# littlepure2333/GFlow

Measured on AMD Instinct MI355X. Metric: GFlow fit_video frames/sec (fwd+bwd+step) @60k Gaussians 480p, higher is better.
Workload: dtype f32

## Files before the change

gflow_amd/_lib.py:

```python
import ctypes
import os
import subprocess
import threading

import torch

_HERE = os.path.dirname(os.path.abspath(__file__))
_CSRC = os.path.join(_HERE, "csrc")
LIB_PATH = os.environ.get("GFLOW_HIP_LIB") or os.path.join(_HERE, "libgflow_hip.so")

_lock = threading.Lock()
_lib = None

c_void_p, c_int, c_float, c_size_t, c_int64 = ctypes.c_void_p, ctypes.c_int, ctypes.c_float, ctypes.c_size_t, ctypes.c_int64

MIN_VERSION = 312

_P = c_void_p
SIGNATURES = {
    "gfl_version": (c_int, []),
    "gfl_constants": (c_int, [_P]),
    "gfl_constants_n": (c_int, [_P, c_int]),
    "gfl_ewa_on_mfma": (c_int, []),
    "gfl_status_string": (ctypes.c_char_p, [c_int]),
    "gfl_last_hip_error": (c_int, []),
    "gfl_reduce_workspace_bytes": (c_size_t, [c_int]),
    "gfl_reduce_cam_workspace_bytes": (c_size_t, [c_int]),
    "gfl_project_point_fwd": (c_int, [_P, _P, _P, c_int, c_int, c_int, c_float, c_float, _P, _P, _P]),
    "gfl_project_point_bwd": (c_int, [_P, _P, _P, _P, _P, _P, c_int, _P, _P, _P, c_size_t, _P]),
    "gfl_project_point_bwd_cam": (c_int, [_P, _P, _P, _P, _P, _P, c_int, _P, _P, _P, _P, c_size_t, _P]),
    "gfl_cov3d_fwd": (c_int, [_P, _P, _P, c_int, _P, _P]),
    "gfl_cov3d_bwd": (c_int, [_P, _P, _P, _P, c_int, _P, _P, _P]),
    "gfl_ewa_fwd": (c_int, [_P, _P, _P, _P, _P, _P, c_int, c_int, c_int, _P, _P, _P, _P]),
    "gfl_ewa_bwd": (c_int, [_P, _P, _P, _P, _P, _P, c_int, c_int, c_int, _P, _P, _P, _P, c_size_t, _P]),
    "gfl_ewa_bwd_cam": (c_int, [_P, _P, _P, _P, _P, _P, c_int, c_int, c_int, _P, _P, _P, _P, _P, c_size_t, _P]),
    "gfl_bin_workspace_bytes": (c_size_t, [c_int, c_int, c_int, c_int]),
    "gfl_bin_count": (c_int, [_P, _P, _P, c_int, c_int, c_int, _P, _P]),
    "gfl_bin_sort": (c_int, [_P, _P, _P, _P, c_int, c_int, c_int, _P, c_int, _P, _P, _P, _P, c_size_t, _P]),
    "gfl_blend_fwd": (c_int, [_P, _P, _P, _P, c_int, c_int, c_int, _P, _P, c_float, c_int, c_int, _P, _P, _P, _P]),
    "gfl_blend_bwd": (c_int, [_P, _P, _P, _P, c_int, c_int, c_int, _P, _P, c_float, c_int, c_int, _P, _P, _P, c_int,
                              _P, _P, _P, _P, c_int, _P]),
    "gfl_sh_fwd": (c_int, [_P, _P, _P, c_int, c_int, _P, _P]),
    "gfl_sh_bwd": (c_int, [_P, _P, _P, _P, c_int, c_int, _P, _P, _P]),
    "gfl_colormap_nonzero": (c_int, [_P, c_int, _P, _P, _P, c_size_t, _P]),
    "gfl_loss_workspace_bytes": (c_size_t, [c_int, c_int]),
    "gfl_loss_fwd_bwd": (c_int, [_P, _P, _P, _P, _P, c_float, c_float, c_int, c_int, _P, _P, _P, _P, c_size_t, _P]),
    "gfl_loss_fwd_bwd_partials": (c_int, [_P, _P, _P, _P, _P, c_float, c_float, c_int, c_int, _P, _P, _P, c_size_t, _P, _P, _P, _P, _P]),
    "gfl_loss_prepare_gt": (c_int, [_P, _P, c_int, c_int, _P, _P]),
    "gfl_loss_fwd_bwd_partials_cached": (c_int, [_P, _P, _P, _P, _P, c_float, c_float, c_int, c_int, _P, _P, _P, c_size_t, _P, _P, _P, _P, _P, _P]),
    "gfl_adam_step": (c_int, [_P, _P, _P, _P, c_int64, c_int, _P, c_float, c_float, c_float, c_float, _P, c_float, c_int, _P]),
    "gfl_step_increment": (c_int, [_P, _P]),
    "gfl_tile_sort_only": (c_int, [_P, c_int, c_int, _P, _P, _P, _P]),
    "gfl_tile_sort_ordered": (c_int, [_P, c_int, c_int, c_int, _P, _P, _P, _P]),
    "gfl_tile_sort_reserved": (c_int, [_P, _P, _P, _P, c_int, c_int, c_int, _P, _P, _P, _P]),
    "gfl_fit_workspace_bytes": (c_size_t, [c_int, c_int, c_int, c_int]),
    "gfl_fit_workspace_layout": (c_int, [c_int, c_int, c_int, c_int, _P, _P, _P, c_int]),
    "gfl_fit_forward": (c_int, [_P, _P, _P]),
    "gfl_fit_backward_step": (c_int, [_P, _P, _P]),
    "gfl_fit_iteration": (c_int, [_P, _P, _P]),
    "gfl_fit_iterations": (c_int, [_P, _P, c_int, c_int, _P]),
    "gfl_fit_reserved_supported": (c_int, [_P, _P]),
    "gfl_fit_snapshot_stage": (c_int, [_P, _P, _P]),
    "gfl_fit_snapshot_workspace_bytes": (c_size_t, [c_int, c_int, c_int]),
    "gfl_fit_snapshot": (c_int, [_P, _P, _P, _P, _P, c_size_t, _P]),
    "gfl_fit_iteration_snapshot": (c_int, [_P, _P, _P, _P, _P]),
    "gfl_render_fwd": (c_int, [_P, _P, _P]),
    "gfl_render_bwd": (c_int, [_P, _P, _P, _P, _P, _P, _P, _P]),
    "gfl_render_bwd_cam": (c_int, [_P, _P, _P, _P, _P, _P, _P, _P, _P]),
    "gfl_render_batch_workspace_bytes": (c_size_t, [c_int, c_int, c_int, c_int, c_int]),
    "gfl_render_batch": (c_int, [_P, c_int, _P, _P, c_int, c_int, c_int, c_int, c_int, _P, _P, _P, _P, _P, c_size_t, _P]),
    "gfl_fit_prepare_targets": (c_int, [_P, _P]),
    "gfl_fit_schedule_info": (c_int, [_P, _P, _P, _P, _P]),
    "gfl_fit_schedule_info_fwd": (c_int, [_P, _P, _P, _P, _P]),
    "gfl_selftest_reduce10": (c_int, [_P, _P, _P, _P]),
    "gfl_selftest_cov2d": (c_int, [_P, _P, c_int, _P, _P, _P]),
    "gfl_selftest_block_mask": (c_int, [_P, c_int, c_int, c_int, c_int, _P, _P, _P]),
    "gfl_concave_hull": (c_int, [_P, c_int, ctypes.c_double, ctypes.c_double, _P, c_int]),
    "gfl_scan_f64_workspace_bytes": (c_size_t, [c_int]),
    "gfl_scan_f64": (c_int, [_P, c_int, _P, _P, c_size_t, _P]),
    "gfl_track_anchor_workspace_bytes": (c_size_t, [c_int, c_int]),
    "gfl_track_anchor": (c_int, [_P, c_int, c_int, _P, c_int, _P, _P, _P, c_size_t, _P]),
    "gfl_track_frame": (c_int, [_P, c_int, _P, c_int, c_int, _P, c_int, c_int, _P, _P, c_int, c_int, c_int, c_float, _P, _P,
                                _P]),
    "gfl_track_history": (c_int, [_P, c_int, _P, c_int, c_int, _P, c_int, c_int, c_float, _P, _P, _P]),
    "gfl_track_backward_workspace_bytes": (c_size_t, [c_int, c_int]),
    "gfl_track_backward": (c_int, [_P, _P, _P, c_int, _P, _P, c_int, _P, _P, _P, _P, c_size_t, _P]),
    "gfl_seg_score": (c_int, [_P, _P, _P, c_int, c_int, c_int, c_int, _P, _P]),
    "gfl_recon_workspace_bytes": (c_size_t, [c_int, c_int]),
    "gfl_recon_frame": (c_int, [_P, _P, c_int, c_int, c_int, c_int, _P, _P, c_size_t, _P]),
    "gfl_flow_workspace_bytes": (c_size_t, [c_int, c_int]),
    "gfl_flow_pair": (c_int, [_P, c_int, _P, _P, _P, c_int, _P, c_int, c_int, _P, _P, c_int, c_int, c_float, c_int, c_int, _P,
                              _P, _P, _P, c_size_t, _P]),
    "gfl_epi_workspace_bytes": (c_size_t, [c_int, c_int, c_int]),
    "gfl_epi_fundamental": (c_int, [_P, c_int, c_int, _P, c_int, _P, _P, _P, _P, _P, c_size_t, _P]),
    "gfl_epi_mask": (c_int, [_P, c_int, c_int, _P, ctypes.c_double, _P, _P, _P, _P, _P, _P, c_size_t, _P]),
    "gfl_flow_occlusion": (c_int, [_P, _P, c_int, c_int, c_int, c_float, c_float, _P, _P, _P, _P, _P]),
    "gfl_abi_sizes": (c_int, [_P, _P]),
    "gfl_profile_enable": (c_int, [ctypes.c_uint]),
    "gfl_profile_read": (c_int, [_P, _P, c_int]),
}


def build(force=False, quiet=True):
    if force:
        subprocess.run(["make", "-C", _CSRC, "clean"], check=True, capture_output=quiet)
    res = subprocess.run(["make", "-C", _CSRC, "-j8"], capture_output=True, text=True)
    if res.returncode != 0:
        raise RuntimeError("building libgflow_hip.so failed:\n" + res.stdout + res.stderr)
    return LIB_PATH


def load():
    global _lib
    with _lock:
        if _lib is not None:
            return _lib
        if not os.path.exists(LIB_PATH):
            raise RuntimeError(
                f"{LIB_PATH} is missing: run `python -c 'import __graft_entry__ as g; g.build()'` "
                "(or `make -C gflow_amd/csrc`).  gflow_amd has no CPU fallback.")
        lib = ctypes.CDLL(LIB_PATH)
        for name, (res, args) in SIGNATURES.items():
            try:
                fn = getattr(lib, name)
            except AttributeError:
                raise RuntimeError(f"{LIB_PATH} has no {name}: it was built from older sources, rebuild the library "
                                   "(make -C gflow_amd/csrc)") from None
            fn.restype = res
            fn.argtypes = args
        if lib.gfl_version() < MIN_VERSION:
            raise RuntimeError(f"{LIB_PATH} is version {lib.gfl_version()}, this binding needs >= {MIN_VERSION}: rebuild it "
                               "(make -C gflow_amd/csrc)")
        _lib = lib
        return lib


def check(rc, what=""):
    if rc != 0:
        lib = load()
        msg = lib.gfl_status_string(rc).decode()
        extra = f" (hipError {lib.gfl_last_hip_error()})" if rc == -3 else ""
        raise RuntimeError(f"libgflow_hip: {what}: {msg}{extra}")


def ptr(t):
    return None if t is None else ctypes.c_void_p(t.data_ptr())


def stream():
    return ctypes.c_void_p(torch.cuda.current_stream().cuda_stream)


def need_device(*tensors):
    for t in tensors:
        if t is not None and not t.is_cuda:
            raise RuntimeError("gflow_amd: tensors must be on a HIP (cuda) device; there is no CPU fallback")


def scratch(nbytes, device):
    return torch.empty(max(int(nbytes), 16), dtype=torch.uint8, device=device)


def scan_f64(x):
    need_device(x)
    x = x.reshape(-1).double().contiguous()
    out = torch.empty_like(x)
    n = x.numel()
    if n:
        lib = load()
        ws = scratch(lib.gfl_scan_f64_workspace_bytes(n), x.device)
        check(lib.gfl_scan_f64(ptr(x), n, ptr(out), ptr(ws), ws.numel(), stream()), "scan_f64")
    return out


def resolve_deterministic(deterministic):
    return torch.are_deterministic_algorithms_enabled() if deterministic is None else bool(deterministic)


_hip = None


def _hip_runtime():
    global _hip
    if _hip is None:
        _hip = ctypes.CDLL("libamdhip64.so")
        _hip.hipExtStreamCreateWithCUMask.restype = ctypes.c_int
        _hip.hipExtStreamCreateWithCUMask.argtypes = [ctypes.POINTER(ctypes.c_void_p), ctypes.c_uint32,
                                                      ctypes.POINTER(ctypes.c_uint32)]
    return _hip


def cu_partition(parts, device=None, cus=None):
    if cus is None:
        cus = torch.cuda.get_device_properties(device if device is not None else torch.cuda.current_device()).multi_processor_count
    xcds = 8
    per_xcd = cus // xcds
    n = per_xcd // int(parts)
    if n < 1:
        raise ValueError(f"cu_partition: {parts} shares of {per_xcd} CUs per XCD")
    out = []
    for p in range(int(parts)):
        words = [0] * ((cus + 31) // 32)
        for cu in range(p * n, (p + 1) * n):
            for x in range(xcds):
                i = cu * xcds + x
                words[i // 32] |= 1 << (i % 32)
        out.append((words, n * xcds))
    return out


def masked_stream(words, device=None):
    dev = torch.device("cuda", torch.cuda.current_device()) if device is None else torch.device(device)
    with torch.cuda.device(dev):
        arr = (ctypes.c_uint32 * len(words))(*words)
        h = ctypes.c_void_p()
        rc = _hip_runtime().hipExtStreamCreateWithCUMask(ctypes.byref(h), len(words), arr)
        if rc != 0:
            raise RuntimeError(f"hipExtStreamCreateWithCUMask failed: hipError {rc}")
    return torch.cuda.ExternalStream(h.value, device=dev)
```

gflow_amd/csrc/gfl_fit.hip:

```cpp
#include "gfl_fit.hpp"

using namespace gfl;

extern "C" {

size_t gfl_loss_workspace_bytes(int W, int H);

static inline int fit_nblk(int N) { return (N + BIN_BLOCK - 1) / BIN_BLOCK; }

static bool ewa_on_mfma() {
    static const bool on = [] { const char* e = getenv("GFL_EWA_MFMA"); return e && e[0] == '1'; }();
    return on;
}

int gfl_ewa_on_mfma(void) { return ewa_on_mfma() ? 1 : 0; }

static int fwd_split_min() {
    static const int v = [] { const char* e = getenv("GFL_FWD_SPLIT_MIN"); return e ? atoi(e) : FWD_SPLIT_MIN; }();
    return v;
}

static bool reserved_enabled() {
    static const bool on = [] { const char* e = getenv("GFL_RESERVED"); return !(e && e[0] == '0'); }();
    return on;
}

static int device_cus() {
    static const int cus = [] {
        int dev = 0, n = 0;
        const bool ok = hipGetDevice(&dev) == hipSuccess &&
                        hipDeviceGetAttribute(&n, hipDeviceAttributeMultiprocessorCount, dev) == hipSuccess && n > 0;
        return ok ? n : 256;
    }();
    return cus;
}
static int blend_queues(const gfl_fit_state* st) {
    int cus = (st && st->cu_count > 0) ? (st->cu_count / 8) * 8 : device_cus();
    if (cus <= 0) cus = 8;
    if (st && st->cu_count > 0) return cus < SCHED_MAX_QUEUES ? cus : SCHED_MAX_QUEUES;
    return cus < 64 ? 64 : (cus < SCHED_MAX_QUEUES ? cus : SCHED_MAX_QUEUES);
}

static int blend_grid(const gfl_fit_state* st, int T, int max_per_cu = BLEND_WG_PER_CU) {
    const int nq = blend_queues(st);
    int per = (T + nq - 1) / nq + 1;
    if (per > max_per_cu) per = max_per_cu;
    return nq * per;
}

struct FitCounters {
    int32_t pool_counter;   int32_t pad0[15];
    int32_t sched_valid;    int32_t pad1[15];
    int32_t regions_valid;  int32_t pad2[7];
    int32_t extent;         int32_t pad3[7];
    int32_t extent_next;    int32_t pad4[7];
    int32_t stamp;          int32_t pad5;
    int32_t snap_mm[2];     int32_t pad6[4];
};
static_assert(sizeof(FitCounters) == 256, "the counter block is one 256-byte region");
static_assert(offsetof(FitCounters, pool_counter) == 0 * 4 && offsetof(FitCounters, sched_valid) == 16 * 4 &&
              offsetof(FitCounters, regions_valid) == 32 * 4 && offsetof(FitCounters, extent) == 40 * 4 &&
              offsetof(FitCounters, extent_next) == 48 * 4 && offsetof(FitCounters, stamp) == 56 * 4 &&
              offsetof(FitCounters, snap_mm) == 58 * 4, "word offsets of the counters");

static size_t fit_regions(Arena& a, int cap_arg, int K_cap, int W, int H, FitWs& w) {
    const size_t T = tile_grid(W, H).tiles();
    const int cap = cap_arg > 0 ? cap_arg : 1;
    const size_t queue_items = (size_t)SCHED_MAX_QUEUES * sched_queue_capacity((int)T, 64);
    const size_t order_words = T * 4 + SORT_ORDER_TRAILER;
    w.hist = a.take<int32_t>("hist", (size_t)fit_nblk(cap) * T);
    w.keys = a.take<unsigned long long>("keys", (size_t)K_cap);
    w.partial = a.take<float>("partial", (size_t)reduce_rows(cap) * 12);
    w.tile_counts = a.take<int32_t>("tile_counts", T);
    w.pair_grad = a.take<float>("pair_grad", ((size_t)cap * SLOT_MAX + (size_t)K_cap) * PG);
    w.wide_base = (long long)cap * SLOT_MAX;
    w.wide_off = a.take<int32_t>("wide_off", (size_t)cap);
    if (FitCounters* c = a.take<FitCounters>("counters", 1)) {
        w.pool_counter = &c->pool_counter; w.sched_valid = &c->sched_valid; w.regions_valid = &c->regions_valid;
        w.extent = &c->extent; w.extent_next = &c->extent_next; w.stamp = &c->stamp; w.snap_mm = (unsigned*)c->snap_mm;
    }
    w.sched.work = a.take<int32_t>("sched_work", 4 * T);
    w.sched.list = a.take<int32_t>("sched_list", queue_items);
    w.sched.count = a.take<int32_t>("sched_count", 2 * SCHED_MAX_QUEUES);
    w.sched.counters = a.take<int32_t>("sched_counters", 2 * SCHED_MAX_QUEUES);
    w.ckpt = a.take<float>("ckpt", (size_t)SCHED_MAX_QUEUES * (HEAVY_PARTS - 1) * 5 * 256);
    w.sched_fwd.work = a.take<int32_t>("sched_fwd_work", 4 * T);
    w.sched_fwd.list = a.take<int32_t>("sched_fwd_list", queue_items);
    w.sched_fwd.count = a.take<int32_t>("sched_fwd_count", 2 * SCHED_MAX_QUEUES);
    w.sched_fwd.counters = w.sched.counters;
    w.sched_fwd.first_slot = nullptr;
    w.sched.first_slot = a.take<int32_t>("first_slot", T);
    w.loss_ws_bytes = up256(gfl_loss_workspace_bytes(W, H));
    w.loss_ws = a.take<char>("loss_ws", w.loss_ws_bytes);
    a.take<char>("loss_pad", 256);
    w.gt_stats = a.take<float>("gt_stats", (size_t)6 * W * H);
    w.scale_cnt = a.take<int32_t>("scale_cnt", (size_t)2 * fit_nblk(cap));
    w.sort_order = (int4*)a.take<int32_t>("sort_order", order_words);
    w.sort_order_next = (int4*)a.take<int32_t>("sort_order_next", order_words);
    w.region = a.take<int4>("region", T);
    w.fill = a.take<int32_t>("fill", T);
    w.partial_cam = a.take<float>("partial_cam", (size_t)reduce_rows(cap) * 4);
    w.d_rec_cam = a.take<float>("d_rec_cam", (size_t)cap * REC);
    return queue_items;
}

static int fit_layout(Arena& a, int cap, int K_cap, int W, int H) {
    if (cap < 0 || K_cap < 0 || W <= 0 || H <= 0) return GFL_ERR_INVALID;
    FitWs w;
    fit_regions(a, cap, K_cap, W, H, w);
    return a.n;
}

size_t gfl_fit_workspace_bytes(int cap, int K_cap, int W, int H) {
    Arena a;
    return fit_layout(a, cap, K_cap, W, H) < 0 ? 0 : a.off;
}

int gfl_fit_workspace_layout(int cap, int K_cap, int W, int H, const char** names, size_t* offsets, size_t* bytes, int max) {
    if (max < 0 || (max > 0 && (!names || !offsets || !bytes))) return GFL_ERR_INVALID;
    Arena a{nullptr, 0, names, offsets, bytes, max};
    return fit_layout(a, cap, K_cap, W, H);
}

static bool fit_ws_fits(const gfl_fit_state* st) {
    return st->workspace_bytes >= gfl_fit_workspace_bytes(st->cap, st->K_cap, st->W, st->H);
}

static FitWs carve(const gfl_fit_state* st) {
    Arena a{(char*)st->workspace};
    FitWs w;
    const size_t queue_items = fit_regions(a, st->cap, st->K_cap, st->W, st->H, w);
    for (Sched* s : {&w.sched, &w.sched_fwd}) {
        s->nq = blend_queues(st);
        s->cap_q = (int)(queue_items / s->nq);
        s->xcd = 1;
        s->det = (st->flags & GFL_FIT_DETERMINISTIC) ? 1 : 0;
    }
    w.sched.split_min = 0;
    w.sched_fwd.split_min = fwd_split_min();
    return w;
}

static bool next_sched_ok(const FitWs& w, int T) {
    return w.sched.xcd && T <= SCHED_PLAN_TILES && w.sched.nq % 8 == 0 && w.sched.nq / 8 <= 64 && w.sched.nq <= REDUCE_BLOCK;
}
static int next_sched_blocks(const FitWs& w, int T) { return next_sched_ok(w, T) ? 2 : 0; }
static size_t next_sched_lds(const FitWs& w, int T) { return next_sched_ok(w, T) ? sched_dyn_lds(T) : 0; }
static NextSched next_sched(const FitWs& w, int rows, int T) {
    NextSched ns;
    ns.rows = rows;
    ns.T = T;
    ns.tile_counts = w.tile_counts;
    ns.bwd = w.sched;
    ns.fwd = w.sched_fwd;
    ns.valid = w.sched_valid;
    ns.reserve = 0;
    ns.order_next = nullptr; ns.ro = ReserveOut{}; ns.regions_valid = nullptr; ns.pool_counter = nullptr;
    ns.pull_counters = nullptr; ns.n_pull = 0;
    return ns;
}

static bool fit_reserved_ok(const FitWs& w, int T) {
    return reserved_enabled() && next_sched_ok(w, T) && T <= 4096 && (2 * (size_t)T + 64) * sizeof(int32_t) <= 57 * 1024;
}
static NextSched next_sched_reserving(const gfl_fit_state* st, const FitWs& w, int rows, int T) {
    NextSched ns = next_sched(w, rows, T);
    if (!fit_reserved_ok(w, T)) return ns;
    ns.reserve = 1;
    ns.order_next = w.sort_order_next;
    ns.ro.region = w.region; ns.ro.fill = w.fill; ns.ro.extent_next = w.extent_next; ns.ro.total = st->tile_offsets + T;
    ns.ro.K_cap = st->K_cap;
    ns.regions_valid = w.regions_valid;
    ns.pool_counter = w.pool_counter;
    ns.pull_counters = w.sched.counters; ns.n_pull = 2 * w.sched.nq;
    return ns;
}

static int fit_check(const gfl_fit_state* st, const gfl_fit_hyper* hp) {
    if (!st || !hp) return GFL_ERR_INVALID;
    if (st->N < 0 || st->N > st->cap || st->W <= 0 || st->H <= 0 || st->K_cap < 0) return GFL_ERR_INVALID;
    if (st->flags & ~GFL_FIT_DETERMINISTIC) return GFL_ERR_INVALID;
    if (!st->params || !st->rec || !st->pose || !st->intr || !st->extr || !st->render || !st->final_T ||
        !st->n_contrib || !st->tile_offsets || !st->ids || !st->tile_range || !st->overflow || !st->workspace)
        return GFL_ERR_INVALID;
    if (!fit_ws_fits(st)) return GFL_ERR_WORKSPACE;
    return GFL_OK;
}


static PreArgs pre_args(const gfl_fit_state* st, const gfl_fit_hyper* hp, const FitWs& w, int gx, int gy, int op_mode) {
    PreArgs a;
    a.intr = st->intr; a.pose = st->pose;
    a.N = st->N; a.W = st->W; a.H = st->H;
    a.nearest = hp->nearest; a.extent = hp->extent;
    a.gx = gx; a.gy = gy;
    a.rec = st->rec; a.wide_off = w.wide_off; a.hist_g = w.hist; a.extr_out = st->extr; a.overflow = st->overflow;
    a.pool_counter = w.pool_counter; a.pool_cap = st->K_cap;
    a.op_mode = op_mode;
    a.scale_rows_mode = (!op_mode && hp->lambda_scale != 0.f) ? (hp->freeze_all_splats ? 2 : 1) : 0;
    a.scale_cnt = w.scale_cnt;
    return a;
}

static int fit_forward_impl(const gfl_fit_state* st, const gfl_fit_hyper* hp, gfl_stream_t stream, int op_mode, int reserved = 0,
                            const float* snap_lut = nullptr, uint8_t* snap_u8 = nullptr) {
    int rc = fit_check(st, hp);
    if (rc) return rc;
    hipStream_t s = (hipStream_t)stream;
    const auto [gx, gy, T] = tile_grid(st->W, st->H);
    const FitWs w = carve(st);
    const int nblk = fit_nblk(st->N > 0 ? st->N : 1);
    if ((size_t)T * sizeof(int32_t) > 57 * 1024) return GFL_ERR_INVALID;
    const PreArgs pa = pre_args(st, hp, w, gx, gy, op_mode);
    if (reserved) {
        if (op_mode || !fit_reserved_ok(w, T)) return GFL_ERR_INVALID;
        {
            StageScope p(ST_PREPROCESS, s);
            BinArgs b;
            b.region = w.region; b.fill = w.fill; b.keys = w.keys; b.K_cap = st->K_cap;
            b.regions_valid = w.regions_valid; b.extent_next = w.extent_next; b.extent = w.extent;
            b.pull_counters = w.sched.counters; b.n_pull = 2 * w.sched.nq;
            launch_preprocess_bin(st->params, pa, st->row_flags, b, nblk, ewa_on_mfma(), s);
        }
        {
            StageScope p(ST_TILE_SORT, s);
            rc = gfl_tile_sort_reserved((const int32_t*)w.sort_order_next, w.fill, w.tile_counts, st->overflow + 2, st->W, st->H,
                                        st->K_cap, w.keys, st->ids, st->tile_range, stream);
        }
        if (rc) return rc;
    } else {
        {
            StageScope p(ST_PREPROCESS, s);
            launch_preprocess_fwd(st->params, pa, st->row_flags, nblk, ewa_on_mfma(), s);
        }
        {
            StageScope p(ST_COLSCAN, s);
            launch_colscan(w, nblk, T, st->overflow, s);
        }
        const bool ordered = T <= 8 * BIN_BLOCK;
        {
            StageScope p(ST_SCATTER, s);
            launch_scatter(st, w, nblk, gx, gy, ordered, s);
        }
        {
            StageScope p(ST_TILE_SORT, s);
            if (ordered)
                rc = gfl_tile_sort_ordered((const int32_t*)w.sort_order, st->W, st->H, st->K_cap, w.keys, st->ids, st->tile_range,
                                           stream);
            else
                rc = gfl_tile_sort_only(st->tile_offsets, gx * gy, st->K_cap, w.keys, st->ids, st->tile_range, stream);
        }
        if (rc) return rc;
    }
    {
        StageScope p(ST_BLEND_FWD, s);
        const TileQueue q = {w.sched_fwd.list, w.sched_fwd.count, w.sched.counters, w.sched.nq, w.sched.cap_q};
        if (snap_u8) {
            rc = check(hipMemsetAsync(w.snap_mm, 0, 2 * sizeof(unsigned), s));
            if (rc) return rc;
            if (st->N > 0) launch_rec_depth_range(st->rec, st->N, w.snap_mm, s);
            launch_blend_fwd(st, hp->bg, gx, blend_grid(st, T, FWD_WG_PER_CU), st->render, st->final_T, st->n_contrib, q, w, 2,
                             w.snap_mm, snap_lut, fwd_split_min(), s, snap_u8);
            launch_center_blend(st, hp->bg, gx, T, nullptr, snap_u8 + (size_t)2 * st->W * st->H * 3, s);
        }
        const bool foot = st->foot_flags && !(hp->bg > 0.f) && st->N > 0;
        if (foot && !st->keep) return GFL_ERR_INVALID;
        const bool foot_inside = foot && !snap_u8;
        if (!snap_u8)
            launch_blend_fwd(st, hp->bg, gx, blend_grid(st, T, FWD_WG_PER_CU), st->render, st->final_T, st->n_contrib, q, w,
                             foot_inside ? 3 : 0, nullptr, nullptr, fwd_split_min(), s);
        if (st->foot_flags) {
            if (!st->keep) return GFL_ERR_INVALID;
            if (foot && !foot_inside) launch_footprint(st, gx, T, s);
        }
    }
    return check_launch();
}

int gfl_fit_forward(const gfl_fit_state* st, const gfl_fit_hyper* hp, gfl_stream_t stream) {
    return fit_forward_impl(st, hp, stream, 0);
}

struct SnapWs { unsigned* mm; int32_t* pull; size_t head_bytes; float *img_dc, *img_c, *fT; int32_t* nc; size_t bytes; };
static SnapWs snap_ws(void* base, int W, int H) {
    Arena a{(char*)base};
    const size_t P = (size_t)W * H;
    return {a.take<unsigned>("mm", 2), a.take<int32_t>("pull", 2 * SCHED_MAX_QUEUES), a.off,
            a.take<float>("img_dc", 4 * P), a.take<float>("img_c", 4 * P), a.take<float>("final_T", P),
            a.take<int32_t>("n_contrib", P), a.off};
}

size_t gfl_fit_snapshot_workspace_bytes(int N, int W, int H) {
    return (N < 0 || W <= 0 || H <= 0) ? 0 : snap_ws(nullptr, W, H).bytes;
}

int gfl_fit_snapshot(const gfl_fit_state* st, const gfl_fit_hyper* hp, const float* lut, uint8_t* out_u8, void* workspace,
                     size_t workspace_bytes, gfl_stream_t stream) {
    int rc = fit_check(st, hp);
    if (rc) return rc;
    if (!lut || !out_u8 || !workspace) return GFL_ERR_INVALID;
    if (workspace_bytes < gfl_fit_snapshot_workspace_bytes(st->N, st->W, st->H)) return GFL_ERR_WORKSPACE;
    hipStream_t s = (hipStream_t)stream;
    const auto [gx, gy, T] = tile_grid(st->W, st->H);
    const FitWs w = carve(st);
    const SnapWs sw = snap_ws(workspace, st->W, st->H);
    rc = check(hipMemsetAsync(workspace, 0, sw.head_bytes, s));
    if (rc) return rc;
    if (st->N > 0) launch_rec_depth_range(st->rec, st->N, sw.mm, s);
    launch_center_blend(st, hp->bg, gx, T, sw.img_c, nullptr, s);
    {
        const TileQueue q = {w.sched_fwd.list, w.sched_fwd.count, sw.pull, w.sched.nq, w.sched.cap_q};
        launch_blend_fwd(st, hp->bg, gx, blend_grid(st, T, FWD_WG_PER_CU), sw.img_dc, sw.fT, sw.nc, q, w, 1, sw.mm, lut, fwd_split_min(), s);
    }
    launch_snapshot_u8(st->render, sw.img_dc, sw.img_c, st->W * st->H, out_u8, s);
    return check_launch();
}

int gfl_fit_snapshot_stage(const gfl_fit_state* src, const gfl_fit_state* dst, gfl_stream_t stream) {
    if (!src || !dst || !src->workspace || !dst->workspace || !src->rec || !dst->rec || !src->ids || !dst->ids ||
        !src->tile_range || !dst->tile_range || !src->render || !dst->render || !src->tile_offsets)
        return GFL_ERR_INVALID;
    if (src->W != dst->W || src->H != dst->H || src->N != dst->N || dst->N > dst->cap || src->N > src->cap)
        return GFL_ERR_INVALID;
    if (!fit_ws_fits(src) || !fit_ws_fits(dst)) return GFL_ERR_WORKSPACE;
    const int T = tile_grid(src->W, src->H).T;
    const size_t P = (size_t)src->W * src->H;
    const FitWs a = carve(src), b = carve(dst);
    if (a.sched_fwd.nq != b.sched_fwd.nq || a.sched_fwd.cap_q != b.sched_fwd.cap_q) return GFL_ERR_INVALID;
    StageCopy c;
    c.k_ptr = a.extent;
    c.ids_cap = (unsigned)min(src->K_cap, dst->K_cap);
    c.seg[0] = {(const uint32_t*)src->ids, (uint32_t*)dst->ids, 0u};
    c.seg[1] = {(const uint32_t*)src->rec, (uint32_t*)dst->rec, (unsigned)((size_t)src->N * REC)};
    c.seg[2] = {(const uint32_t*)src->tile_range, (uint32_t*)dst->tile_range, (unsigned)(2 * T)};
    c.seg[3] = {(const uint32_t*)src->render, (uint32_t*)dst->render, (unsigned)(3 * P)};
    c.seg[4] = {(const uint32_t*)a.sched_fwd.list, (uint32_t*)b.sched_fwd.list,
                (unsigned)((size_t)a.sched_fwd.nq * a.sched_fwd.cap_q)};
    c.seg[5] = {(const uint32_t*)a.sched_fwd.count, (uint32_t*)b.sched_fwd.count, (unsigned)a.sched_fwd.nq};
    c.seg[6] = {(const uint32_t*)a.sched.first_slot, (uint32_t*)b.sched.first_slot, (unsigned)T};
    launch_snapshot_stage(c, (hipStream_t)stream);
    return check_launch();
}

int gfl_render_fwd(const gfl_fit_state* st, const gfl_fit_hyper* hp, gfl_stream_t stream) {
    if (st && st->foot_flags) return GFL_ERR_INVALID;
    if (st && (st->flags & GFL_FIT_DETERMINISTIC)) {
        const int rc = fit_check(st, hp);
        if (rc) return rc;
        const int T = tile_grid(st->W, st->H).T;
        const FitWs w = carve(st);
        hipStream_t s = (hipStream_t)stream;
        if (check(hipMemsetAsync(w.sched.work, 0, 4 * (size_t)T * sizeof(int32_t), s)) ||
            check(hipMemsetAsync(w.sched_fwd.work, 0, 4 * (size_t)T * sizeof(int32_t), s)) ||
            check(hipMemsetAsync(w.sched_valid, 0, sizeof(int32_t), s)))
            return GFL_ERR_HIP;
    }
    return fit_forward_impl(st, hp, stream, 1);
}

static int render_bwd_impl(const gfl_fit_state* st, const gfl_fit_hyper* hp, const float* d_render, const float* d_uv,
                           const float* d_depth, float* d_params, float* d_extr, float* d_intr, gfl_stream_t stream) {
    hipStream_t s = (hipStream_t)stream;
    const auto [gx, gy, T] = tile_grid(st->W, st->H);
    const FitWs w = carve(st);
    {
        StageScope p(ST_BLEND_BWD, s);
        const TileQueue q = {w.sched.list, w.sched.count, w.sched.counters + w.sched.nq, w.sched.nq, w.sched.cap_q};
        launch_blend_bwd(st, hp->bg, gx, gy, blend_grid(st, T), 10, d_render, q, w, LossTail{}, s);
    }
    {
        StageScope p(ST_PRE_BWD_ADAM, s);
        const NextSched ns = next_sched(w, reduce_rows(st->N > 0 ? st->N : 1), T);
        if (d_intr)
            launch_splat_bwd_op_cam(st, w, gx, gy, ns, next_sched_blocks(w, T), next_sched_lds(w, T), d_uv, d_depth, d_params, d_extr,
                                    d_intr, s);
        else
            launch_splat_bwd_op(st, w, gx, gy, ns, next_sched_blocks(w, T), next_sched_lds(w, T), d_uv, d_depth, d_params, d_extr, s);
    }
    return check_launch();
}

int gfl_render_bwd(const gfl_fit_state* st, const gfl_fit_hyper* hp, const float* d_render, const float* d_uv,
                   const float* d_depth, float* d_params, float* d_extr, gfl_stream_t stream) {
    int rc = fit_check(st, hp);
    if (rc) return rc;
    if (!d_render || !d_params || !d_extr) return GFL_ERR_INVALID;
    return render_bwd_impl(st, hp, d_render, d_uv, d_depth, d_params, d_extr, nullptr, stream);
}

int gfl_render_bwd_cam(const gfl_fit_state* st, const gfl_fit_hyper* hp, const float* d_render, const float* d_uv,
                       const float* d_depth, float* d_params, float* d_extr, float* d_intr, gfl_stream_t stream) {
    if (!d_extr || !d_intr) return GFL_ERR_INVALID;
    int rc = fit_check(st, hp);
    if (rc) return rc;
    if (!d_render || !d_params) return GFL_ERR_INVALID;
    return render_bwd_impl(st, hp, d_render, d_uv, d_depth, d_params, d_extr, d_intr, stream);
}

int gfl_fit_backward_step(const gfl_fit_state* st, const gfl_fit_hyper* hp, gfl_stream_t stream) {
    int rc = fit_check(st, hp);
    if (rc) return rc;
    if (!st->adam_m || !st->adam_v || !st->pose_m || !st->pose_v || !st->depth_ab || !st->depth_ab_m ||
        !st->depth_ab_v || !st->step || !st->gt_rgb || !st->d_render || !st->err_px || !st->sums || !st->d_extr)
        return GFL_ERR_INVALID;
    hipStream_t s = (hipStream_t)stream;
    const auto [gx, gy, T] = tile_grid(st->W, st->H);
    const FitWs w = carve(st);
    const float *p_ssim = nullptr, *p_grad = nullptr;
    int n_ssim = 0, n_grad = 0;
    {
        StageScope p(ST_LOSS, s);
        const float* gt_stats = (st->gt_cached && !st->foot_flags) ? w.gt_stats : nullptr;
        rc = gfl_loss_fwd_bwd_partials_cached(st->render, st->gt_rgb, st->gt_depth, st->keep, st->depth_ab,
                                              hp->lambda_rgb, hp->lambda_depth, st->W, st->H, st->d_render,
                                              st->err_px, w.loss_ws, w.loss_ws_bytes, gt_stats, &p_ssim, &n_ssim,
                                              &p_grad, &n_grad, stream);
    }
    if (rc) return rc;
    AdamCfg ac = {hp->lr, hp->beta1, hp->beta2, hp->eps, hp->lr_end_factor, hp->total_iters};
    AdamCfg ac_cam = ac;
    ac_cam.lr = hp->lr_camera;
    const bool frozen = hp->step_camera != 2 && (hp->step_camera == 0 || hp->lr_camera == 0.f);
    LossTail lt = {};
    if (frozen) {
        lt.enabled = 1;
        lt.p_ssim = p_ssim; lt.n_ssim = n_ssim; lt.p_grad = p_grad; lt.n_grad = n_grad;
        lt.depth_ab = st->depth_ab; lt.ab_m = st->depth_ab_m; lt.ab_v = st->depth_ab_v;
        lt.sums = st->sums; lt.ac_ab = ac; lt.step_affine = hp->step_camera != 0;
        lt.d_step = st->step; lt.d_extr_out = st->d_extr; lt.overflow = st->overflow;
    }
    {
        StageScope p(ST_BLEND_BWD, s);
        const TileQueue q = {w.sched.list, w.sched.count, w.sched.counters + w.sched.nq, w.sched.nq, w.sched.cap_q};
        const int sums = hp->freeze_all_splats ? 6 : (hp->freeze_rgb ? 7 : 10);
        launch_blend_bwd(st, hp->bg, gx, gy, blend_grid(st, T), sums, st->d_render, q, w, lt, s);
    }
    const int rows = reduce_rows(st->N > 0 ? st->N : 1);
    RegCfg rcfg;
    rcfg.lambda_scale = hp->lambda_scale;
    rcfg.scale_blocks = 2 * fit_nblk(st->N > 0 ? st->N : 1);
    rcfg.lambda_var = st->N > 0 ? hp->lambda_var / (float)st->N : 0.f;
    rcfg.lambda_flow = hp->lambda_flow;
    rcfg.lambda_still = hp->lambda_still;
    rcfg.freeze_rgb = hp->freeze_rgb;
    rcfg.freeze_all = hp->freeze_all_splats;
    rcfg.no_pose_grad = frozen ? 1 : 0;
    {
        StageScope p(ST_PRE_BWD_ADAM, s);
        const NextSched ns = next_sched_reserving(st, w, rows, T);
        launch_splat_bwd_adam(st, w, gx, gy, rcfg, ac, ns, next_sched_blocks(w, T) + ns.reserve, next_sched_lds(w, T), s);
    }
    if (!frozen) {
        StageScope p(ST_CAMERA, s);
        launch_camera_adam(st, w, rows, p_ssim, n_ssim, p_grad, n_grad, ac_cam, ac, hp->step_camera != 0, s);
    }
    return check_launch();
}

int gfl_fit_iterations(const gfl_fit_state* st, const gfl_fit_hyper* hp, int count, int flags, gfl_stream_t stream) {
    if (count < 1 || (flags & ~GFL_ITER_RESERVED)) return GFL_ERR_INVALID;
    int rc = fit_check(st, hp);
    if (rc) return rc;
    const int T = tile_grid(st->W, st->H).T;
    const FitWs w = carve(st);
    const bool res_ok = fit_reserved_ok(w, T) && st->N > 0;
    if ((flags & GFL_ITER_RESERVED) && !res_ok) return GFL_ERR_INVALID;
    for (int j = 0; j < count; ++j) {
        const int reserved = res_ok && (j > 0 || (flags & GFL_ITER_RESERVED)) ? 1 : 0;
        rc = fit_forward_impl(st, hp, stream, 0, reserved);
        if (rc) return rc;
        rc = gfl_fit_backward_step(st, hp, stream);
        if (rc) return rc;
    }
    return GFL_OK;
}

int gfl_fit_iteration_snapshot(const gfl_fit_state* st, const gfl_fit_hyper* hp, const float* lut, uint8_t* out_u8,
                               gfl_stream_t stream) {
    if (!lut || !out_u8) return GFL_ERR_INVALID;
    int rc = fit_forward_impl(st, hp, stream, 0, 0, lut, out_u8);
    if (rc) return rc;
    return gfl_fit_backward_step(st, hp, stream);
}

int gfl_fit_reserved_supported(const gfl_fit_state* st, const gfl_fit_hyper* hp) {
    if (fit_check(st, hp) || st->N <= 0) return 0;
    const int T = tile_grid(st->W, st->H).T;
    return fit_reserved_ok(carve(st), T) ? 1 : 0;
}

int gfl_fit_prepare_targets(const gfl_fit_state* st, gfl_stream_t stream) {
    if (!st || st->W <= 0 || st->H <= 0 || !st->gt_rgb || !st->workspace) return GFL_ERR_INVALID;
    if (!fit_ws_fits(st)) return GFL_ERR_WORKSPACE;
    const FitWs w = carve(st);
    return gfl_loss_prepare_gt(st->gt_rgb, st->keep, st->W, st->H, w.gt_stats, stream);
}

static int schedule_info(const gfl_fit_state* st, bool fwd, int* n_queues, int* queue_capacity, const int32_t** d_lists,
                         const int32_t** d_counts) {
    if (!st || !n_queues || !queue_capacity || !d_lists || !d_counts || !st->workspace) return GFL_ERR_INVALID;
    if (!fit_ws_fits(st)) return GFL_ERR_WORKSPACE;
    const FitWs w = carve(st);
    const Sched& sc = fwd ? w.sched_fwd : w.sched;
    *n_queues = sc.nq;
    *queue_capacity = sc.cap_q;
    *d_lists = sc.list;
    *d_counts = sc.count;
    return GFL_OK;
}

int gfl_fit_schedule_info(const gfl_fit_state* st, int* n_queues, int* queue_capacity, const int32_t** d_lists,
                          const int32_t** d_counts) {
    return schedule_info(st, false, n_queues, queue_capacity, d_lists, d_counts);
}

int gfl_fit_schedule_info_fwd(const gfl_fit_state* st, int* n_queues, int* queue_capacity, const int32_t** d_lists,
                              const int32_t** d_counts) {
    return schedule_info(st, true, n_queues, queue_capacity, d_lists, d_counts);
}

int gfl_fit_iteration(const gfl_fit_state* st, const gfl_fit_hyper* hp, gfl_stream_t stream) {
    int rc = gfl_fit_forward(st, hp, stream);
    if (rc) return rc;
    return gfl_fit_backward_step(st, hp, stream);
}

#ifdef GFL_TRACE
int gfl_debug_read_fwd_trace(long long* out, int n_tiles) { return read_fwd_trace(out, n_tiles); }
int gfl_debug_read_fwd_trace2(long long* out, int n_values) { return read_fwd_trace2(out, n_values); }
int gfl_debug_read_phase_trace(long long* out, int n_values) {
    const int rc = read_phase_trace_bin(out, n_values);
    return rc ? rc : read_phase_trace_splat(out, n_values);
}
int gfl_debug_read_bwd_trace(long long* out, int n_tiles) { return read_bwd_trace(out, n_tiles); }
#endif

}
```

gflow_amd/csrc/gfl_fit_snap.hip:

```cpp
#include "gfl_fit.hpp"

namespace gfl {

__global__ void __launch_bounds__(256) center_blend_kernel(const float* __restrict__ rec, const int32_t* __restrict__ ids,
                                                           const int32_t* __restrict__ tile_range, float bg, int W, int H, int gx,
                                                           float* __restrict__ out, uint8_t* __restrict__ out_u8) {
    __shared__ RecLDS recs[FB + 1];
    __shared__ unsigned char s_mask[FB];
    if (threadIdx.x == 0) {
        const float4 z = make_float4(0.f, 0.f, 0.f, 0.f);
        recs[FB].p0 = z; recs[FB].p1 = z; recs[FB].p2 = z;
    }
    const int tile = blockIdx.x;
    const int tx = tile % gx, ty = tile / gx;
    const int tid = threadIdx.x, wave = tid >> 6, lane = tid & 63;
    const int px = tx * GFL_TILE + (wave & 1) * 8 + (lane & 7);
    const int py = ty * GFL_TILE + (wave >> 1) * 8 + (lane >> 3);
    const bool inside = px < W && py < H;
    const float fx = pixf(px), fy = pixf(py);
    const int start = tile_range[2 * tile], end = tile_range[2 * tile + 1];
    const float blob_cutoff = alpha_cutoff(1.f, 1.f);
    float T = 1.f, Tw = inside ? 1.f : 0.f, a0 = 0.f, a1 = 0.f, a2 = 0.f;
    for (int base = start; base < end; base += FB) {
        if (__syncthreads_and(Tw == 0.f)) break;
        const int idx = base + tid;
        unsigned char m = 0;
        if (idx < end) {
            const int g = ids[idx];
            const float4* r4 = reinterpret_cast<const float4*>(rec + (size_t)g * REC);
            float4 p0 = r4[0], p1 = r4[1], p2 = r4[2];
            p0.z = 1.f; p0.w = 0.f; p1.x = 1.f; p1.y = 1.f;
            p2.z = p2.z < 0.f ? p2.z : blob_cutoff;
            recs[tid].p0 = p0; recs[tid].p1 = p1; recs[tid].p2 = p2;
            m = (unsigned char)block_mask(p0, p1, p2.z, tx * GFL_TILE, ty * GFL_TILE);
        }
        s_mask[tid] = m;
        __syncthreads();
        const int cnt = min(FB, end - base);
        for (int c0 = 0; c0 < cnt && !__all(Tw == 0.f); c0 += 64) {
            const int slot = c0 + lane;
            unsigned long long bits = __ballot(slot < cnt && ((s_mask[slot] >> wave) & 1));
            while (bits) {
                int j[4];
#pragma unroll
                for (int u = 0; u < 4; ++u) {
                    j[u] = bits ? c0 + (int)__builtin_ctzll(bits) : FB;
                    bits &= bits - 1;
                }
                float4 q0[4], q1[4];
                float cb[4], al[4];
                bool val[4];
#pragma unroll
                for (int u = 0; u < 4; ++u) { q0[u] = recs[j[u]].p0; q1[u] = recs[j[u]].p1; cb[u] = recs[j[u]].p2.x; }
#pragma unroll
                for (int u = 0; u < 4; ++u) {
                    float G;
                    val[u] = splat_alpha2(q0[u], q1[u], fx, fy, al[u], G);
                }
#pragma unroll
                for (int u = 0; u < 4; ++u) {
                    const float a = val[u] ? al[u] : 0.f;
                    const float test_T = Tw * (1.f - a);
                    const bool stop = test_T < GFL_T_MIN;
                    const float w = stop ? 0.f : a * Tw;
                    a0 = fmaf(q1[u].z, w, a0); a1 = fmaf(q1[u].w, w, a1); a2 = fmaf(cb[u], w, a2);
                    T = stop ? T : test_T;
                    Tw = stop ? 0.f : test_T;
                }
                if (__all(Tw == 0.f)) break;
            }
        }
    }
    if (inside) {
        const size_t pix = (size_t)py * W + px, plane = (size_t)H * W;
        const float o0 = fmaf(T, bg, a0), o1 = fmaf(T, bg, a1), o2 = fmaf(T, bg, a2);
        if (out_u8) {
            uint8_t* u = out_u8 + pix * 3;
            u[0] = img_u8(o0); u[1] = img_u8(o1); u[2] = img_u8(o2);
        } else {
            out[pix] = o0; out[plane + pix] = o1; out[2 * plane + pix] = o2;
        }
    }
}

__global__ void __launch_bounds__(256) rec_depth_range_kernel(const float* __restrict__ rec, int N, unsigned* __restrict__ mm) {
    unsigned lo = 0xffffffffu, hi = 0u;
    for (int i = blockIdx.x * blockDim.x + threadIdx.x; i < N; i += gridDim.x * blockDim.x) {
        const float x = rec[(size_t)i * REC + 9];
        const unsigned b = __float_as_uint(x);
        const unsigned k = (b & 0x80000000u) ? ~b : (b | 0x80000000u);
        if (x != 0.f) lo = min(lo, k);
        hi = max(hi, k);
    }
#pragma unroll
    for (int off = 32; off >= 1; off >>= 1) {
        lo = min(lo, (unsigned)__shfl_xor((int)lo, off));
        hi = max(hi, (unsigned)__shfl_xor((int)hi, off));
    }
    if ((threadIdx.x & 63) == 0) {
        atomicMax(&mm[0], ~lo);
        atomicMax(&mm[1], hi);
    }
}

__global__ void __launch_bounds__(256) snapshot_u8_kernel(const float* __restrict__ a, const float* __restrict__ b,
                                                          const float* __restrict__ c, int P, uint8_t* __restrict__ out) {
    const int i = blockIdx.x * blockDim.x + threadIdx.x;
    if (i >= P) return;
    const float* src[3] = {a, b, c};
#pragma unroll
    for (int k = 0; k < 3; ++k) {
#pragma unroll
        for (int ch = 0; ch < 3; ++ch) {
            out[((size_t)k * P + i) * 3 + ch] = img_u8(src[k][(size_t)ch * P + i]);
        }
    }
}

__global__ void __launch_bounds__(256) snapshot_stage_kernel(StageCopy c) {
    const unsigned tid = blockIdx.x * blockDim.x + threadIdx.x, stride = gridDim.x * blockDim.x;
#pragma unroll
    for (int sgi = 0; sgi < 7; ++sgi) {
        const StageSeg sg = c.seg[sgi];
        unsigned n = sg.n;
        if (sgi == 0) n = min((unsigned)max(*c.k_ptr, 0), c.ids_cap);
        const unsigned n4 = n >> 2;
        const uint4* s4 = reinterpret_cast<const uint4*>(sg.src);
        uint4* d4 = reinterpret_cast<uint4*>(sg.dst);
        for (unsigned i = tid; i < n4; i += stride) d4[i] = s4[i];
        for (unsigned i = (n4 << 2) + tid; i < n; i += stride) sg.dst[i] = sg.src[i];
    }
}

void launch_center_blend(const gfl_fit_state* st, float bg, int gx, int T, float* out, uint8_t* out_u8, hipStream_t s) {
    center_blend_kernel<<<T, 256, 0, s>>>(st->rec, st->ids, st->tile_range, bg, st->W, st->H, gx, out, out_u8);
}

void launch_rec_depth_range(const float* rec, int N, unsigned* mm, hipStream_t s) {
    rec_depth_range_kernel<<<min((N + 255) / 256, 32), 256, 0, s>>>(rec, N, mm);
}

void launch_snapshot_u8(const float* a, const float* b, const float* c, int P, uint8_t* out, hipStream_t s) {
    snapshot_u8_kernel<<<(P + 255) / 256, 256, 0, s>>>(a, b, c, P, out);
}

void launch_snapshot_stage(const StageCopy& c, hipStream_t s) { snapshot_stage_kernel<<<1024, 256, 0, s>>>(c); }

}
```

gflow_amd/fit_video.py:

```python
import argparse
import json
import math
import os
import sys
import time

import torch

from . import camera as CM
from . import flow as FL
from . import quality as QL
from . import segmentation as SG
from . import tracking as TK

SCRIPT_OVERRIDES = dict(num_points=50000, lr_after=4e-3, lr_camera_after=1e-3, densify_times_after=2,
                        densify_occ_percent=0.5, lambda_depth=0.1, lambda_var=50.0, lambda_still=0.0)
DEFAULTS = dict(num_points=60000, lr=4e-3, lr_camera=0.0, iterations_first=500, lr_after=1e-3, iterations_after=300,
                camera_first=True, lr_camera_after=5e-4, iterations_camera=150, densify_interval=150, densify_times=2,
                densify_interval_after=100, densify_times_after=1, densify_occ_percent=1.0, densify_err_thre=1e-2,
                densify_err_percent=1.0, lambda_rgb=1.0, lambda_depth=1e-4, lambda_var=10.0, lambda_still=10.0,
                lambda_flow=0.01, lambda_scale=0.0, background="black",
                traj_num=0, traj_offset=0)

METRIC_NAMES = ("psnr_sum", "frames", "iterations", "rasterisations", "clips", "splats_final")


def shard(n_items, rank, world, lengths=None):
    lengths = [1] * n_items if lengths is None else [int(v) for v in lengths]
    if len(lengths) != n_items:
        raise ValueError("shard: one length per clip")
    load = [0] * world
    mine = []
    for i in sorted(range(n_items), key=lambda j: (-lengths[j], j)):
        r = min(range(world), key=lambda q: (load[q], q))
        load[r] += lengths[i]
        if r == rank:
            mine.append(i)
    return sorted(mine)


def reduce_metrics(local, wall_seconds, dist=None, device="cpu", rank=0, world=1):
    own = [0.0] * world
    own[rank] = float(wall_seconds)
    vec = torch.tensor([float(local.get(k, 0.0)) for k in METRIC_NAMES] + own, dtype=torch.float64, device=device)
    wall = torch.tensor([float(wall_seconds)], dtype=torch.float64, device=device)
    if dist is not None and dist.is_initialized():
        dist.all_reduce(vec, op=dist.ReduceOp.SUM)
        dist.all_reduce(wall, op=dist.ReduceOp.MAX)
    vals = vec.tolist()
    out = {k: float(v) for k, v in zip(METRIC_NAMES, vals)}
    out["wall_s"] = float(wall.item())
    out["rank_wall_s"] = [float(v) for v in vals[len(METRIC_NAMES):]]
    return out


TAPVID_KEYS = ("occlusion_accuracy", "average_jaccard", "average_pts_within_thresh")
DAVIS_KEYS = ("J", "F", "J&F")
RECON_KEYS = ("PSNR", "SSIM")
CAMERA_KEYS = CM.SCORE_KEYS
FLOW_KEYS = FL.EVAL_KEYS


def _mean_over_clips(keys, scores, totals, dist=None, device="cpu", none=float("nan")):
    n = len(keys)
    sums, counts = [0.0] * n, [0.0] * n
    for m in scores:
        for j, k in enumerate(keys):
            if m[k] is not None and not math.isnan(m[k]):
                sums[j] += float(m[k])
                counts[j] += 1.0
    vec = torch.tensor(sums + counts + [float(t) for t in totals.values()], dtype=torch.float64, device=device)
    if dist is not None and dist.is_initialized():
        dist.all_reduce(vec, op=dist.ReduceOp.SUM)
    v = vec.tolist()
    out = {k: v[j] / v[n + j] if v[n + j] else none for j, k in enumerate(keys)}
    out.update(zip(totals, (int(t) for t in v[2 * n:])))
    return out


def reduce_tapvid(preds, gts, n_frames, dropped, dist=None, device="cpu"):
    ms = [TK.evaluate(p, *gts[ci][:4], n_frames[ci], *gts[ci][4:]) for ci, p in preds.items()]
    return _mean_over_clips(TAPVID_KEYS, ms, dict(clips=len(ms), queries_dropped=dropped), dist, device)


def reduce_davis(segs, dist=None, device="cpu"):
    ms = [SG.evaluate(seg) for seg in segs.values()]
    totals = dict(frames_scored=sum(m["frames_scored"] for m in ms), clips=sum(1 for m in ms if m["frames_scored"]))
    return _mean_over_clips(DAVIS_KEYS, ms, totals, dist, device)


def reduce_recon(recons, dist=None, device="cpu"):
    ms = [QL.evaluate(rec) for rec in recons.values()]
    totals = dict(frames=sum(m["frames"] for m in ms), clips=sum(1 for m in ms if m["frames"]))
    return _mean_over_clips(RECON_KEYS, ms, totals, dist, device)


def reduce_camera(cams, dist=None, device="cpu"):
    scored = [cam for cam in cams.values() if not any(cam[k] is None for k in CAMERA_KEYS)]
    totals = dict(clips=len(scored), clips_unscored=len(cams) - len(scored))
    return _mean_over_clips(CAMERA_KEYS, scored, totals, dist, device, none=None)


def reduce_flow(flows, dist=None, device="cpu"):
    ms = [FL.evaluate(fl) for fl in flows.values()]
    totals = dict(pairs=sum(m["pairs"] for m in ms), clips=sum(1 for m in ms if m["pairs"]))
    return _mean_over_clips(FLOW_KEYS, ms, totals, dist, device, none=None)


def csv_metrics(out):
    m = {}
    if "recon" in out:
        m.update({"PSNR": out["recon"]["PSNR"], "SSIM": out["recon"]["SSIM"]})
    if "tapvid" in out:
        m.update({"Occlusion_Accuracy": out["tapvid"]["occlusion_accuracy"], "Average_Jaccard": out["tapvid"]["average_jaccard"],
                  "Average_PTS_within_threshold": out["tapvid"]["average_pts_within_thresh"]})
    if "davis" in out:
        m.update({"J_zero": out["davis"]["J"], "F_zero": out["davis"]["F"], "J&F_zero": out["davis"]["J&F"]})
    if "camera" in out:
        m.update({k: out["camera"][k] for k in CAMERA_KEYS})
    return m


_FIT_STREAMS = {}


def upload_clip(frames, device):
    out = []
    for fr in frames:
        d = dict(fr)
        occ = fr.get("occ_mask")
        if occ is not None and "occ_count" not in d:
            m = torch.as_tensor(occ).squeeze()
            if m.dim() == 3:
                m = m[..., 0] if m.shape[-1] in (1, 3) else m[0]
            d["occ_count"] = int((m > 0).sum())
        for k, v in fr.items():
            if isinstance(v, torch.Tensor) and k != "extr":
                d[k] = v.to(device, non_blocking=True)
        out.append(d)
    return out


def select_traj_seeds(tr, traj_num, traj_offset):
    import numpy as np
    from scipy.ndimage import minimum_filter
    n = tr.current_pts_num()
    interval = max(int(n / traj_num), 1)
    plain = list(range(n))[traj_offset::interval]
    move_seg = getattr(tr, "move_seg", None)
    if move_seg is None:
        return plain, None
    H, W = tr.H, tr.W
    erode = lambda m: minimum_filter(m, size=10, mode="constant", cval=255)
    move_er = erode(np.asarray(move_seg, dtype=np.uint8))
    still_er = erode((255 - np.asarray(move_seg, dtype=np.int32)).astype(np.uint8))
    s_still, s_move = 50, 15
    grid = lambda lo_i, hi_i, lo_j, hi_j, s: [(j, i) for i in range(lo_i, hi_i, s) for j in range(lo_j, hi_j, s)]
    sparse = [(j, i) for (j, i) in grid(s_still, H, s_still, W, s_still) if still_er[i, j]]
    if len(sparse) == 0:
        sparse = grid(s_still, H, s_still, W, s_still)
    dense = [(j, i) for (j, i) in grid(s_move, H - s_move, s_move, W - s_move, s_move) if move_er[i, j]]
    if len(sparse) == 0:
        dense = grid(s_move, H - s_move, s_move, W - s_move, s_move)
    uv = tr.last_uv.detach().double()
    still = tr.still_mask.detach()

    def closest(points):
        q = torch.tensor(points, dtype=torch.float64, device=uv.device)
        out = []
        for a in range(0, q.shape[0], 256):
            d = ((uv[:, None, :] - q[None, a:a + 256, :]) ** 2).sum(-1)
            out.append(d.argmin(dim=0))
        return torch.cat(out)

    if len(sparse) == 0:
        return plain, None
    sp = closest(sparse)
    sp_still = sp[still[sp]]
    if len(dense):
        de = closest(dense)
        de_move = de[~still[de]]
        return torch.cat([sp_still, de_move]).tolist(), int(sp_still.shape[0])
    return sp_still.tolist(), None


def begin_frame(tr, frames, i, load_extr=True):
    fr = frames[i]
    tr.set_gt_image(fr["image"])
    tr.set_gt_depth(fr["depth"])
    tr.set_gt_flow(frames[i - 1]["flow"])
    if load_extr and fr.get("extr") is not None:
        tr.load_camera(extr=fr["extr"])


def stage_kwargs(c, frames, i, stage):
    fr = frames[i]
    if stage == "camera":
        return dict(iterations=c["iterations_camera"], lr_camera=c["lr_camera_after"], lambda_var=0.0, lambda_still=0.0,
                    lambda_flow=c["lambda_flow"], densify_interval=c["densify_interval"], densify_times=c["densify_times"],
                    camera_only=True, move_mask=fr["move_mask"])
    if stage == "joint":
        return dict(iterations=c["iterations_after"], lr=c["lr_after"], lr_camera=0.0, lambda_var=c["lambda_var"],
                    lambda_still=c["lambda_still"], lambda_flow=c["lambda_flow"], densify_interval=c["densify_interval_after"],
                    densify_times=c["densify_times_after"], mask=fr.get("occ_mask"), mask_count=fr.get("occ_count"),
                    move_mask=fr["move_mask"])
    raise ValueError(stage)


def fit_clip(frames, device, cfg=None, fused=True, deterministic=None, **options):
    if deterministic and not fused:
        raise ValueError("fit_clip(deterministic=True) needs fused=True: the operator path's alpha_blending backward has no "
                         "deterministic implementation")
    from .trainer import run_to_end
    dev_ = torch.device(device)
    g = fit_clip_steps(frames, device, cfg, fused=fused, deterministic=deterministic, chunk=None, cu_count=0, **options)

    drive = lambda: run_to_end(g)
    if dev_.type == "cuda" and torch.cuda.current_stream(dev_) == torch.cuda.default_stream(dev_):
        key = dev_.index
        if key not in _FIT_STREAMS:
            _FIT_STREAMS[key] = torch.cuda.Stream(device=dev_)
        fs = _FIT_STREAMS[key]
        fs.wait_stream(torch.cuda.current_stream(dev_))
        with torch.cuda.stream(fs):
            out = drive()
        torch.cuda.current_stream(dev_).wait_stream(fs)
        return out
    return drive()


def fit_clip_steps(frames, device, cfg=None, seed=0, snapshot_interval=0, fused=True, log=None, load_extr=True, chunk=None,
                   async_snapshots=True, keep=None, cu_count=0, deterministic=None, track_queries=None, segment=False,
                   recon=False, camera=False, flow=False, track_backward=False):
    if track_backward and track_queries is None:
        raise ValueError("fit_clip(track_backward=True) needs track_queries")
    from .trainer import SimpleGaussian
    c = dict(DEFAULTS)
    c.update(cfg or {})
    if any(isinstance(v, torch.Tensor) and not v.is_cuda for k, v in frames[0].items() if k != "extr"):
        frames = upload_clip(frames, device)
    f0 = frames[0]
    tracker = None
    if track_queries is not None:
        tracker = TK.Tracker(track_queries, len(frames), device, backward=bool(track_backward))
    cam_rec = None
    if camera:
        cam_gt = [fr["extr_gt"] if fr.get("extr_gt") is not None else fr.get("extr") for fr in frames]
        missing = [t for t, e in enumerate(cam_gt) if e is None]
        if missing:
            raise ValueError(f"fit_clip(camera=True): frames {missing} carry neither extr_gt nor extr")
        cam_rec = CM.CameraRecorder(len(frames))
    tr = SimpleGaussian(f0["image"], f0["depth"], num_points=c["num_points"], background=c["background"],
                        device=device, seed=seed, fused=fused, deterministic=deterministic)
    tr.async_snapshots = bool(async_snapshots)
    tr.cu_count = int(cu_count)
    if segment:
        tr.seg_recorder = SG.MoveSegRecorder(len(frames), tr.H, tr.W, tr.device)
    recon_rec = None
    if recon:
        recon_rec = QL.ReconRecorder(len(frames), tr.H, tr.W, tr.device)
    flow_rec = None
    if flow:
        flow_rec = FL.FlowRecorder(len(frames), tr.H, tr.W, tr.device, keep_maps=flow == "maps")
        if keep is not None and keep.get("record_flow_inputs"):
            flow_rec.inputs = keep.setdefault("flow_inputs", [])
    tr.load_camera(focal=f0["focal"], pp=f0["pp"])
    if load_extr and f0.get("extr") is not None:
        tr.load_camera(extr=f0["extr"])
    tr.init_gaussians_from_image(f0["image"], f0["depth"], num_points=c["num_points"])
    common = dict(lambda_rgb=c["lambda_rgb"], lambda_depth=c["lambda_depth"], lambda_scale=c["lambda_scale"],
                  densify_occ_percent=c["densify_occ_percent"], densify_err_thre=c["densify_err_thre"],
                  densify_err_percent=c["densify_err_percent"], snapshot_interval=snapshot_interval,
                  lazy_images=True,
                  chunk=chunk)
    traj = int(c["traj_num"]) > 0
    yield from tr.train_steps(iterations=c["iterations_first"], lr=c["lr"], lr_camera=c["lr_camera"],
                              lambda_var=c["lambda_var"], densify_interval=c["densify_interval"],
                              densify_times=c["densify_times"], move_mask=f0["move_mask"],
                              move_seg=traj,
                              **common)
    traj_rec = []
    final = []

    def final_forward():
        if not final:
            final.append(tr._aux_forward())
            final[0].watch_overflow()
            tr.rasterisations_done += 1
        return final[0]

    def record_trajectories():
        with torch.no_grad():
            xyz_now = tr.get_attribute("xyz")[traj_index_t].detach().float().clone()
            extr_now = tr.get_extr().detach().clone()
            if tr.engine_current:
                rgb_u8 = tr._render_scene_fused()[0].clone()
                final.append(tr._aux)
            else:
                from . import render as render_mod
                rgb_u8 = render_mod.render2img_device(render_mod.render_multiple(tr._input_group(detach=True), ["rgb"])["rgb"])
            tr.rasterisations_done += 1
        traj_rec.append((xyz_now, extr_now, rgb_u8))

    def record_tracks(i):
        with torch.no_grad():
            if tr.engine_current:
                from .fused import REC
                aux = final_forward()
                n = aux.N
                uv, uv_stride, depth, depth_stride, dm = aux.rec[:n, 0:2], REC, aux.rec[:n, 9], REC, aux.render[3]
            else:
                from . import render as render_mod
                o = render_mod.render_multiple(tr._input_group(detach=True), ["uv", "depth", "depth_map"])
                uv, depth = o["uv"].float().contiguous(), o["depth"].float().reshape(-1).contiguous()
                dm = o["depth_map"].float().reshape(tr.H, tr.W).contiguous()
                uv_stride, depth_stride = 2, 1
                tr.rasterisations_done += 1
            tracker.frame(i, uv, uv_stride, depth, depth_stride, dm)
            if keep is not None and keep.get("record_track_inputs"):
                keep.setdefault("track_inputs", []).append((uv.clone(), depth.clone(), dm.clone()))

    def record_flow(i):
        with torch.no_grad():
            if tr.engine_current:
                aux = final_forward()
                rec, n, ids, tile_range = aux.rec, aux.N, aux.ids, aux.tile_range
            else:
                rec, n, ids, tile_range = FL.operator_state(tr._input_group(detach=True))
                tr.rasterisations_done += 1
            prev = frames[i - 1] if i else None
            flow_rec.frame(i, rec, n, ids, tile_range, prev["flow"] if prev else None, prev["move_mask"] if prev else None)

    def record_scores(i):
        with torch.no_grad():
            if recon_rec is not None:
                recon_rec.frame(i, tr.last_render, tr.gt_image)
                if keep is not None and keep.get("record_recon_inputs"):
                    keep.setdefault("recon_inputs", []).append(tr.last_render[:3].clone())
            if cam_rec is not None:
                cam_rec.frame(i, tr.get_extr())

    def draw_trajectories():
        from . import msplat
        from . import render as render_mod
        imgs, uvs = [], []
        with torch.no_grad():
            for xyz_now, extr_now, rgb_u8 in traj_rec:
                overlay = tr.eval_trajectories(xyz_now, extr_now, line_scale=0.5, point_scale=2.0, alpha=0.8,
                                               split_interval=split_interval)
                img_traj = render_mod.render2img_device(overlay)
                upon = 1.0 - (1.0 - rgb_u8.double() / 255.0) * (1.0 - img_traj.double() / 255.0)
                imgs.append(torch.stack([img_traj, (upon * 255.0).to(torch.uint8)]))
                uvs.append(msplat.project_point(xyz_now, tr.intr, extr_now, tr.W, tr.H)[0])
                if keep is not None:
                    keep.setdefault("traj_groups", []).append([x.clone() if isinstance(x, torch.Tensor) else x
                                                               for x in tr.last_traj_group])
        return torch.stack(imgs), torch.stack(uvs)

    psnr_sum = None

    def end_of_frame(i):
        nonlocal psnr_sum
        final.clear()
        if traj:
            record_trajectories()
        if tracker is not None:
            record_tracks(i)
        if flow_rec is not None:
            record_flow(i)
        p = tr.psnr()
        psnr_sum = p.double() if psnr_sum is None else psnr_sum + p.double()
        if recon_rec is not None or cam_rec is not None:
            record_scores(i)
        if keep is not None:
            keep["psnr"].append(p)
        if log:
            log(f"frame {i}: psnr {float(p):.2f} dB, splats {tr.current_pts_num()}")

    if traj:
        traj_index, split_interval = select_traj_seeds(tr, int(c["traj_num"]), int(c["traj_offset"]))
        traj_index_t = torch.as_tensor(traj_index, device=tr.device).long()
    if keep is not None:
        keep["trainer"], keep["psnr"] = tr, []
    end_of_frame(0)
    for i in range(1, len(frames)):
        begin_frame(tr, frames, i, load_extr)
        if segment:
            tr.seg_recorder.frame = i
        if c["camera_first"]:
            yield from tr.train_steps(**stage_kwargs(c, frames, i, "camera"), **common)
        if c["iterations_after"] > 0:
            yield from tr.train_steps(**stage_kwargs(c, frames, i, "joint"), **common)
        end_of_frame(i)
    if tr.engine is not None:
        tr.engine.check_overflow()
    if traj:
        imgs_d, uvs_d = draw_trajectories()
        if imgs_d.is_cuda:
            from .pinned import PINNED
            block = PINNED.take(imgs_d.numel())
            imgs_h = block[0][:imgs_d.numel()].view(imgs_d.shape)
            imgs_h.copy_(imgs_d, non_blocking=True)
            uvs_h = uvs_d.cpu()
            traj_out = dict(images=PINNED.hand_out(block, [imgs_h])[0], uv=uvs_h.numpy(), index=list(traj_index),
                            split_interval=split_interval)
            PINNED.release(block)
        else:
            traj_out = dict(images=imgs_d.numpy(), uv=uvs_d.numpy(), index=list(traj_index), split_interval=split_interval)
        if keep is not None:
            keep["traj"] = traj_out
    out = dict(psnr_sum=float(psnr_sum), frames=len(frames), iterations=tr.iterations_done,
               rasterisations=tr.rasterisations_done, clips=1, splats_final=tr.current_pts_num(),
               void_iterations=tr.engine.regions_outgrown if tr.engine is not None else 0)
    if traj:
        out["traj"] = traj_out
    if tracker is not None:
        out["tracks"] = tracker.result()
    if segment:
        rec = tr.seg_recorder
        if keep is not None and keep.get("record_seg_inputs"):
            keep["seg_inputs"] = [None if x is None else (x[0].clone(), x[1].clone()) for x in rec.inputs]
        out["segmentation"] = rec.result([fr["move_mask"] for fr in frames])
    if recon_rec is not None:
        out["recon"] = recon_rec.result()
    if cam_rec is not None:
        import numpy as np
        extr = cam_rec.result()
        gt = np.stack([torch.as_tensor(e).detach().cpu().double().numpy().reshape(3, 4) for e in cam_gt])
        out["camera"] = dict(extr=extr, **CM.evaluate(extr, gt))
    if flow_rec is not None:
        out["flow"] = flow_rec.result()
    return out


NUMERIC_KEYS = ("psnr_sum", "frames", "iterations", "rasterisations", "clips", "splats_final", "void_iterations")


def fit_clips_concurrent(clips, device, cfg=None, seeds=None, chunk=32, partition=False, deterministic=None,
                         track_queries=None, track_backward=False, **options):
    n = len(clips)
    if track_queries is not None and len(track_queries) != n:
        raise ValueError("fit_clips_concurrent: track_queries needs one entry per clip")
    if track_backward and track_queries is None:
        raise ValueError("fit_clips_concurrent(track_backward=True) needs track_queries")
    seeds = list(range(n)) if seeds is None else seeds
    dev = torch.device(device)
    if dev.index is None:
        dev = torch.device("cuda", torch.cuda.current_device())
    cur = torch.cuda.current_stream(dev)
    shares = None
    if partition and n > 1:
        from . import _lib
        shares = _lib.cu_partition(n, dev)
        streams = [_lib.masked_stream(words, dev) for words, _ in shares]
    else:
        streams = [torch.cuda.Stream(device=dev) for _ in range(n)]
    for s in streams:
        s.wait_stream(cur)
    gens = [fit_clip_steps(clips[i], dev, cfg, seed=seeds[i], chunk=chunk, async_snapshots=n == 1,
                           cu_count=shares[i][1] if shares else 0, deterministic=deterministic,
                           track_queries=None if track_queries is None else track_queries[i],
                           track_backward=bool(track_backward) and track_queries[i] is not None, **options)
            for i in range(n)]
    results = [None] * n
    live = list(range(n))
    while live:
        for i in list(live):
            with torch.cuda.stream(streams[i]):
                try:
                    next(gens[i])
                except StopIteration as e:
                    results[i] = e.value
                    live.remove(i)
    for s in streams:
        cur.wait_stream(s)
    return results


def main(argv=None):
    ap = argparse.ArgumentParser(description="fit synthetic clips, one process per GPU")
    ap.add_argument("--clips", type=int, default=1)
    ap.add_argument("--frames", type=int, default=4)
    ap.add_argument("--height", type=int, default=480)
    ap.add_argument("--width", type=int, default=854)
    ap.add_argument("--num_points", type=int, default=60000)
    ap.add_argument("--iterations_first", type=int, default=500)
    ap.add_argument("--iterations_after", type=int, default=300)
    ap.add_argument("--iterations_camera", type=int, default=150)
    ap.add_argument("--frames-list", default=None, help="comma-separated frame counts, one per synthetic clip (clips of "
                                                        "unequal length: the shard balances them)")
    ap.add_argument("--clips-per-gpu", type=int, default=1,
                    help="clips a rank fits at the same time on its GPU (fit_clips_concurrent)")
    ap.add_argument("--verbose", action="store_true")
    ap.add_argument("--sequence", action="append", default=None,
                    help="path of a prepared sequence folder (images + the reference's sibling folders, "
                         "gflow_amd/io.py); may be given several times, one clip each; default: synthetic clips")
    ap.add_argument("--resize", type=int, default=None, help="shorter image side after loading a --sequence")
    ap.add_argument("--deterministic", action="store_true",
                    help="bit-identical results for identical inputs (the library's deterministic mode, INTEGRATION.md)")
    ap.add_argument("--track", action="store_true",
                    help="track the first-visible query points of each clip's tracking.pkl (synthetic clips: their "
                         "make_clip_tracks) through the fit and score them with TAP-Vid (a \"tapvid\" block in the line)")
    ap.add_argument("--track-backward", action="store_true",
                    help="with --track: also track every query through the frames before its own (the \"tapvid\" block "
                         "then carries \"backward\": true)")
    ap.add_argument("--track-queries", choices=("first", "strided"), default="first",
                    help="with --track: the query protocol -- each track's first visible frame, or TAP-Vid's strided one "
                         "(every fifth frame where the track is visible; wants --track-backward)")
    ap.add_argument("--track-out", default=None, help="with --track: write each clip's predicted tracks to DIR/clip_<i>.npz")
    ap.add_argument("--seg", action="store_true",
                    help="keep every frame's moving-region mask and score it against the frame's move_mask with DAVIS J, F "
                         "and J&F (a \"davis\" block in the line)")
    ap.add_argument("--seg-out", default=None,
                    help="with --seg: write each clip's masks to DIR/clip_<i>/move_mask_<frame>.png")
    ap.add_argument("--recon", action="store_true",
                    help="score every frame's render with PSNR and SSIM on the device (a \"recon\" block in the line)")
    ap.add_argument("--camera", action="store_true",
                    help="keep every frame's camera and score the path against the clip's own (extr_gt, else extr) with "
                         "ATE and RPE (a \"camera\" block in the line)")
    ap.add_argument("--flow", action="store_true",
                    help="the dense optical flow the fitted splats imply between consecutive frames, scored against the flow "
                         "the clip came with: end-point error, still / moving, accuracies, coverage (a \"flow\" block in the "
                         "line)")
    ap.add_argument("--flow-out", default=None,
                    help="with --flow: write each clip's flow maps to DIR/clip_<i>/flow_<frame>.flo (frame -> frame + 1 on "
                         "the frame's grid; pixels without a flow are 1e10, Middlebury's mark)")
    ap.add_argument("--no-load-extr", action="store_true",
                    help="do not load the frames' camera poses (extr): the camera-only stages estimate them, as the "
                         "reference's scripts/fit_video.sh runs")
    ap.add_argument("--make-move-masks", action="store_true",
                    help="with --sequence: compute every frame's move_mask from its forward flow on the device "
                         "(gflow_amd.move_seg, before the clock starts) instead of reading <seq>_epipolar")
    ap.add_argument("--make-occ-masks", action="store_true",
                    help="with --sequence: compute every frame's occ_mask from its forward and backward flows "
                         "(<seq>_flow_unimatch/*pred.flo, *pred_bwd.flo) on the device (gflow_amd.occlusion, before the clock "
                         "starts) instead of reading *occ_bwd.png")
    ap.add_argument("--metrics-csv", default=None,
                    help="rank 0 writes the blocks that were asked for as key,value lines under the reference's "
                         "metrics.csv keys")
    args = ap.parse_args(argv)
    if args.track_backward and not args.track:
        ap.error("--track-backward needs --track")
    if args.track and args.track_queries == "strided" and not args.track_backward:
        print("warning: --track-queries strided without --track-backward: every frame before a query is a miss",
              file=sys.stderr)
    det = True if args.deterministic else None
    from . import synthetic as S
    rank = int(os.environ.get("RANK", "0"))
    local_rank = int(os.environ.get("LOCAL_RANK", "0"))
    world = int(os.environ.get("WORLD_SIZE", "1"))
    n_dev = torch.cuda.device_count()
    if n_dev < 1:
        raise RuntimeError("gflow_amd.fit_video needs a HIP device (there is no CPU rasteriser)")
    shared = world > n_dev
    torch.cuda.set_device(local_rank % n_dev)
    dev = torch.device("cuda", local_rank % n_dev)
    dist = None
    if world > 1:
        import torch.distributed as dist
        if shared:
            dist.init_process_group(backend="gloo")
        else:
            dist.init_process_group(backend="nccl", device_id=dev)
    cfg = dict(num_points=args.num_points, iterations_first=args.iterations_first,
               iterations_after=args.iterations_after, iterations_camera=args.iterations_camera)
    local = {k: 0.0 for k in METRIC_NAMES}
    n_clips = len(args.sequence) if args.sequence else args.clips
    if args.sequence:
        from . import io as gio
        lengths = [len(gio.sequence_paths(p)["img"]) for p in args.sequence]
    elif args.frames_list:
        lengths = [int(v) for v in args.frames_list.split(",")]
        if len(lengths) != n_clips:
            raise SystemExit("--frames-list needs one length per clip")
    else:
        lengths = [args.frames] * n_clips
    mine = shard(n_clips, rank, world, lengths)
    t_load = time.perf_counter()
    clips = {}
    for ci in mine:
        if args.sequence:
            clips[ci] = gio.load_sequence(args.sequence[ci], resize=args.resize,
                                          move_masks="epipolar" if args.make_move_masks else "files",
                                          occ_masks="flow" if args.make_occ_masks else "files")
        else:
            clips[ci] = upload_clip(S.make_clip(lengths[ci], args.height, args.width, seed=ci, device=dev), dev)
    gts, queries, dropped = {}, {}, 0
    if args.track:
        for ci in mine:
            h, w = clips[ci][0]["image"].shape[:2]
            if args.sequence:
                pts, occ = TK.read_tapvid_pickle(os.path.join(args.sequence[ci], "tracking.pkl"))
            else:
                g = S.make_clip_tracks(lengths[ci], args.height, args.width, seed=ci)
                pts, occ = g["points"].astype("float32"), g["occluded"]
            if args.track_queries == "strided":
                q, src = TK.strided_queries(pts, occ, h, w)
                keep = q[:, 0] < len(clips[ci])
                gts[ci] = (pts, occ, h, w, q[keep], src[keep])
            else:
                q = TK.first_visible_queries(pts, occ, h, w)
                keep = q[:, 0] < len(clips[ci])
                gts[ci] = (pts[keep], occ[keep], h, w)
            dropped += int((~keep).sum())
            queries[ci] = q[keep]
    t_load = time.perf_counter() - t_load
    torch.cuda.synchronize()
    t0 = time.perf_counter()
    c = max(1, args.clips_per_gpu)
    order = sorted(clips, key=lambda j: (-lengths[j], j))
    options = dict(track_backward=args.track_backward, deterministic=det, segment=args.seg, recon=args.recon, camera=args.camera,
                   flow=("maps" if args.flow_out else True) if args.flow else False, load_extr=not args.no_load_extr)
    results = {}
    for g0 in range(0, len(order), c):
        group = order[g0:g0 + c]
        if len(group) == 1:
            ci = group[0]
            res = [fit_clip(clips[ci], dev, cfg, seed=ci, track_queries=queries.get(ci), **options,
                            log=(lambda s, ci=ci: print(f"[rank {rank} clip {ci}] {s}")) if args.verbose else None)]
        else:
            res = fit_clips_concurrent([clips[ci] for ci in group], dev, cfg, seeds=group,
                                       track_queries=[queries.get(ci) for ci in group] if args.track else None, **options)
        for ci, m in zip(group, res):
            for k in METRIC_NAMES:
                local[k] += m[k]
            results[ci] = m
    torch.cuda.synchronize()
    wall = time.perf_counter() - t0
    of = lambda key: {ci: m[key] for ci, m in results.items()}
    over_ranks = (dist, torch.device("cpu") if (world > 1 and shared) else dev)
    out = reduce_metrics(local, wall, *over_ranks, rank=rank, world=world)
    if args.track:
        preds = of("tracks")
        out["tapvid"] = reduce_tapvid(preds, gts, {ci: len(clips[ci]) for ci in clips}, dropped, *over_ranks)
        if args.track_backward:
            out["tapvid"]["backward"] = True
        if args.track_out:
            import numpy as np
            os.makedirs(args.track_out, exist_ok=True)
            for ci, p in preds.items():
                np.savez(os.path.join(args.track_out, f"clip_{ci}.npz"), queries=queries[ci], **p)
    if args.seg:
        out["davis"] = reduce_davis(of("segmentation"), *over_ranks)
        if args.seg_out:
            from PIL import Image
            for ci, seg in of("segmentation").items():
                d = os.path.join(args.seg_out, f"clip_{ci}")
                os.makedirs(d, exist_ok=True)
                for t in range(len(seg["masks"])):
                    if seg["valid"][t]:
                        Image.fromarray(seg["masks"][t]).save(os.path.join(d, f"move_mask_{t:05d}.png"))
    if args.recon:
        out["recon"] = reduce_recon(of("recon"), *over_ranks)
    if args.camera:
        out["camera"] = reduce_camera(of("camera"), *over_ranks)
    if args.flow:
        out["flow"] = reduce_flow(of("flow"), *over_ranks)
        if args.flow_out:
            for ci, fl in of("flow").items():
                FL.write_flo_maps(os.path.join(args.flow_out, f"clip_{ci}"), fl)
    if rank == 0 and args.metrics_csv:
        QL.write_metrics_csv(args.metrics_csv, csv_metrics(out))
    if rank == 0:
        out["frames_per_s"] = out["frames"] / out["wall_s"]
        out["iterations_per_s"] = out["iterations"] / out["wall_s"]
        out["psnr_mean_db"] = out["psnr_sum"] / max(out["frames"], 1.0)
        out["n_gpus"] = world
        out["clips_per_gpu"] = c
        out["load_s_rank0"] = t_load
        print(json.dumps(out))
    if dist is not None:
        dist.destroy_process_group()
    return out if rank == 0 else None


if __name__ == "__main__":
    main()
```

gflow_amd/fused.py:

```python
import ctypes

import torch

from . import _lib as L

ROW = 16
REC = 12
COLS = {"xyz": (0, 3), "scale": (3, 6), "rotate": (6, 10), "opacity": (10, 11), "rgb": (11, 14)}

_P = ctypes.c_void_p
_I = ctypes.c_int32


class FitState(ctypes.Structure):
    _fields_ = [("N", _I), ("cap", _I), ("W", _I), ("H", _I), ("K_cap", _I), ("gt_cached", _I),
                ("params", _P), ("adam_m", _P), ("adam_v", _P), ("rec", _P), ("d_rec", _P),
                ("flow_target", _P), ("flow_w", _P), ("still_target", _P), ("still_w", _P), ("row_flags", _P),
                ("pose", _P), ("pose_m", _P), ("pose_v", _P),
                ("depth_ab", _P), ("depth_ab_m", _P), ("depth_ab_v", _P),
                ("intr", _P), ("extr", _P), ("d_extr", _P), ("step", _P),
                ("gt_rgb", _P), ("gt_depth", _P), ("keep", _P), ("move_mask", _P), ("foot_flags", _P),
                ("render", _P), ("final_T", _P), ("n_contrib", _P),
                ("d_render", _P), ("err_px", _P), ("sums", _P),
                ("tile_offsets", _P), ("ids", _P), ("tile_range", _P), ("overflow", _P),
                ("workspace", _P), ("workspace_bytes", ctypes.c_size_t), ("cu_count", _I), ("flags", _I)]

GFL_FIT_DETERMINISTIC = 1


class FitHyper(ctypes.Structure):
    _fields_ = [("bg", ctypes.c_float), ("nearest", ctypes.c_float), ("extent", ctypes.c_float),
                ("lambda_rgb", ctypes.c_float), ("lambda_depth", ctypes.c_float), ("lambda_var", ctypes.c_float),
                ("lambda_flow", ctypes.c_float), ("lambda_still", ctypes.c_float), ("lambda_scale", ctypes.c_float),
                ("lr", ctypes.c_float), ("lr_camera", ctypes.c_float), ("beta1", ctypes.c_float),
                ("beta2", ctypes.c_float), ("eps", ctypes.c_float), ("lr_end_factor", ctypes.c_float),
                ("total_iters", _I), ("freeze_rgb", _I), ("freeze_all_splats", _I), ("step_camera", _I)]


def _declare(lib):
    if getattr(lib, "_fit_declared", False):
        return
    lib.gfl_fit_workspace_bytes.restype = ctypes.c_size_t
    lib.gfl_fit_workspace_bytes.argtypes = [ctypes.c_int] * 4
    for name in ("gfl_fit_forward", "gfl_fit_backward_step", "gfl_fit_iteration", "gfl_render_fwd"):
        fn = getattr(lib, name)
        fn.restype = ctypes.c_int
        fn.argtypes = [ctypes.POINTER(FitState), ctypes.POINTER(FitHyper), _P]
    lib.gfl_fit_iterations.restype = ctypes.c_int
    lib.gfl_fit_iterations.argtypes = [ctypes.POINTER(FitState), ctypes.POINTER(FitHyper), ctypes.c_int, ctypes.c_int, _P]
    lib.gfl_fit_snapshot.restype = ctypes.c_int
    lib.gfl_fit_snapshot.argtypes = [ctypes.POINTER(FitState), ctypes.POINTER(FitHyper), _P, _P, _P, ctypes.c_size_t, _P]
    lib.gfl_fit_iteration_snapshot.restype = ctypes.c_int
    lib.gfl_fit_iteration_snapshot.argtypes = [ctypes.POINTER(FitState), ctypes.POINTER(FitHyper), _P, _P, _P]
    lib.gfl_render_bwd.restype = ctypes.c_int
    lib.gfl_render_bwd.argtypes = [ctypes.POINTER(FitState), ctypes.POINTER(FitHyper), _P, _P, _P, _P, _P, _P]
    lib.gfl_render_bwd_cam.restype = ctypes.c_int
    lib.gfl_render_bwd_cam.argtypes = [ctypes.POINTER(FitState), ctypes.POINTER(FitHyper), _P, _P, _P, _P, _P, _P, _P]
    lib._fit_declared = True


PROFILE = {"mask": 0}

import gc as _gc
import threading as _threading

_GRAPH_LOCK = _threading.RLock()


def set_profile(mask):
    PROFILE["mask"] = int(mask)
    L.check(L.load().gfl_profile_enable(int(mask)), "profile")


class FitEngine:
    def __init__(self, W, H, capacity, device, K_cap=None, bg=0.0, cu_count=0, deterministic=False):
        self.lib = L.load()
        self.cu_count = int(cu_count)
        self._deterministic = bool(deterministic)
        _declare(self.lib)
        self.dev = torch.device(device)
        if self.dev.type != "cuda":
            raise RuntimeError("FitEngine needs a HIP device (there is no CPU path)")
        self.W, self.H = int(W), int(H)
        self.gx, self.gy = (self.W + 15) // 16, (self.H + 15) // 16
        self.T = self.gx * self.gy
        self.N = 0
        self.hp = FitHyper(bg=bg, nearest=0.2, extent=1.3, lambda_rgb=1.0, lambda_depth=0.0, lambda_var=0.0,
                           lambda_flow=0.0, lambda_still=0.0, lambda_scale=0.0, lr=1e-2, lr_camera=0.0, beta1=0.9, beta2=0.999,
                           eps=1e-8, lr_end_factor=0.1, total_iters=0, freeze_rgb=0, freeze_all_splats=0,
                           step_camera=1)
        f32 = dict(dtype=torch.float32, device=self.dev)
        i32 = dict(dtype=torch.int32, device=self.dev)
        H_, W_ = self.H, self.W
        self.pose = torch.zeros(7, **f32)
        self.pose[3:4].fill_(1.0)
        self.pose_m, self.pose_v = torch.zeros(7, **f32), torch.zeros(7, **f32)
        self.depth_ab = torch.zeros(2, **f32)
        self.depth_ab[0:1].fill_(1.0)
        self.ab_m, self.ab_v = torch.zeros(2, **f32), torch.zeros(2, **f32)
        self.intr = torch.zeros(4, **f32)
        self.extr = torch.zeros(12, **f32)
        self.d_extr = torch.zeros(12, **f32)
        self.step = torch.zeros(1, **i32)
        self.render = torch.zeros(4, H_, W_, **f32)
        self.final_T = torch.zeros(H_, W_, **f32)
        self.n_contrib = torch.zeros(H_, W_, **i32)
        self.d_render = torch.zeros(4, H_, W_, **f32)
        self.err_px = torch.zeros(H_, W_, **f32)
        self.sums = torch.zeros(8, **f32)
        self._offsets_and_flags = torch.zeros(self.T + 1 + 4, **i32)
        self.tile_offsets = self._offsets_and_flags[:self.T + 1]
        self.tile_range = torch.zeros(self.T, 2, **i32)
        self.overflow = self._offsets_and_flags[self.T + 1:]
        self.gt_rgb = self.gt_depth = self.keep = None
        self.move_mask = self.foot_flags = None
        self.flow_target = self.flow_w = self.still_target = self.still_w = self.row_flags = None
        self.cap = self.K_cap = 0
        self.K_cap_req = K_cap
        self._K_grown = False
        self.params = self.d_rec = self._state = None
        self.want_d_rec = False
        self._graphs, self._graph_key, self._graph_trash = {}, None, []
        self._reserved_sup = (None, 0)
        self.regions_outgrown = self.pairs_grown = 0
        self._pend_event = self._pend_host = self._ovf_event = self._ovf_host = None
        self._snap_ring = self._snap_ring_done = None
        self._snap_out = self._snap_ws = self._capture_stream = None
        self._launched = False
        self._reserved_N = -1
        self.busy = False
        self._alloc(int(capacity))

    def __del__(self):
        try:
            with _GRAPH_LOCK:
                self._graphs.clear()
                for gs in getattr(self, "_graph_trash", []):
                    gs.clear()
        except Exception:
            pass

    def _retire_graphs(self):
        if self._graphs:
            self._graph_trash.append(self._graphs)
            self._graphs = {}
        if len(self._graph_trash) > 256:
            self.reap_graphs()

    def reap_graphs(self):
        if self._graph_trash:
            with _GRAPH_LOCK:
                for gs in self._graph_trash:
                    gs.clear()
            self._graph_trash = []

    def _alloc(self, cap):
        f32 = dict(dtype=torch.float32, device=self.dev)
        old = self.params
        n = self.N
        self.cap = cap
        self.params = torch.zeros(cap, ROW, **f32)
        self.adam_m = torch.zeros(cap, ROW, **f32)
        self.adam_v = torch.zeros(cap, ROW, **f32)
        self.rec = torch.zeros(cap, REC, **f32)
        self.d_rec = torch.zeros(cap, REC, **f32) if self.want_d_rec else None
        if old is not None and n:
            self.params[:n] = old[:n]
        k_min = self.K_cap if self._K_grown else 0
        self._alloc_pairs(max(int(self.K_cap_req) if self.K_cap_req else max(4_000_000, 8 * cap), k_min))

    def _alloc_pairs(self, K_cap):
        self.K_cap = int(K_cap)
        self.ids = torch.zeros(self.K_cap, dtype=torch.int32, device=self.dev)
        nbytes = self.lib.gfl_fit_workspace_bytes(self.cap, self.K_cap, self.W, self.H)
        self.workspace = torch.zeros(nbytes, dtype=torch.uint8, device=self.dev)
        self._state = None
        self._reserved_N = -1

    def ensure_capacity(self, n):
        if n > self.cap:
            regs = (self.flow_target, self.flow_w, self.still_target, self.still_w, self.row_flags, self.foot_flags)
            m, v = self.adam_m, self.adam_v
            old_n = self.N
            self._alloc(max(n, 2 * self.cap))
            self.adam_m[:old_n], self.adam_v[:old_n] = m[:old_n], v[:old_n]
            grown = []
            for t in regs:
                if t is None:
                    grown.append(None)
                    continue
                g = torch.zeros((self.cap,) + tuple(t.shape[1:]), dtype=t.dtype, device=self.dev)
                g[:t.shape[0]] = t
                grown.append(g)
            self.flow_target, self.flow_w, self.still_target, self.still_w, self.row_flags, self.foot_flags = grown

    def set_count(self, n):
        if n > self.cap:
            raise RuntimeError("FitEngine.set_count beyond the capacity; call ensure_capacity first")
        self.N = int(n)
        if self._state is not None:
            self._state.N = self.N
        self._reserved_N = -1

    def invalidate_regions(self):
        self._reserved_N = -1

    def set_splats(self, attrs):
        n = attrs["xyz"].shape[0]
        self.ensure_capacity(n)
        self.N = n
        for k, (a, b) in COLS.items():
            self.params[:n, a:b] = attrs[k].detach().reshape(n, b - a).to(self.dev)
        self.params[:n, 14:] = 0
        self._state = None
        self._reserved_N = -1

    def views(self):
        return {k: self.params[:self.N, a:b] for k, (a, b) in COLS.items()}

    def reset_optimizer(self, splats=True, camera=True):
        if splats:
            self.adam_m.zero_()
            self.adam_v.zero_()
        if camera:
            self.pose_m.zero_(); self.pose_v.zero_(); self.ab_m.zero_(); self.ab_v.zero_()
        self.step.zero_()

    def set_targets(self, gt_image, gt_depth=None, keep=None):
        self.gt_rgb = gt_image.to(self.dev).float().contiguous()
        self.gt_depth = None if gt_depth is None else gt_depth.to(self.dev).float().reshape(self.H, self.W).contiguous()
        self.keep = None if keep is None else keep.to(self.dev).reshape(self.H, self.W).to(torch.uint8).contiguous()
        self.move_mask = self.foot_flags = None
        self._state = None

    def set_footprint_mask(self, move_mask, moving_rows):
        self.move_mask = move_mask.to(self.dev).reshape(self.H, self.W).to(torch.uint8).contiguous()
        flags = torch.zeros(self.cap, dtype=torch.uint8, device=self.dev)
        flags[:moving_rows.shape[0]] = moving_rows.to(self.dev).to(torch.uint8)
        self.foot_flags = flags
        if self.hp.bg > 0.0:
            self.keep = torch.zeros(self.H, self.W, dtype=torch.uint8, device=self.dev)
        else:
            self.keep = (self.move_mask == 0).to(torch.uint8).contiguous()
        self._state = None

    def set_regularisers(self, flow_target=None, flow_w=None, still_target=None, still_w=None, row_flags=None):
        def pad(t, width, dtype):
            if t is None:
                return None
            out = torch.zeros((self.cap, width) if width else (self.cap,), dtype=dtype, device=self.dev)
            out[:t.shape[0]] = t.to(self.dev).reshape((t.shape[0], width) if width else (t.shape[0],))
            return out
        self.flow_target, self.flow_w = pad(flow_target, 2, torch.float32), pad(flow_w, 0, torch.float32)
        self.still_target, self.still_w = pad(still_target, 3, torch.float32), pad(still_w, 0, torch.float32)
        self.row_flags = pad(row_flags, 0, torch.uint8)
        self._state = None

    def state(self):
        if self._state is None:
            s = FitState()
            s.N, s.cap, s.W, s.H, s.K_cap = self.N, self.cap, self.W, self.H, self.K_cap
            for name, ctype in FitState._fields_:
                if ctype is _P:
                    t = getattr(self, {"depth_ab_m": "ab_m", "depth_ab_v": "ab_v"}.get(name, name))
                    setattr(s, name, None if t is None else t.data_ptr())
            s.workspace_bytes = self.workspace.numel()
            s.cu_count = self.cu_count
            s.flags = GFL_FIT_DETERMINISTIC if self._deterministic else 0
            if self.gt_rgb is not None and self.foot_flags is None:
                L.check(self.lib.gfl_fit_prepare_targets(ctypes.byref(s), L.stream()), "fit prepare targets")
                s.gt_cached = 1
            self._state = s
        return self._state

    @property
    def deterministic(self):
        return self._deterministic

    @deterministic.setter
    def deterministic(self, on):
        self._deterministic = bool(on)
        if self._state is not None:
            self._state.flags = GFL_FIT_DETERMINISTIC if self._deterministic else 0

    def snapshot_ring(self, rows):
        ring = self._snap_ring
        if ring is None or ring.shape[0] < rows:
            ring = torch.empty(int(rows), 3, self.H, self.W, 3, dtype=torch.uint8, device=self.dev)
            self._snap_ring = ring
        if self._snap_ring_done is not None:
            torch.cuda.current_stream().wait_event(self._snap_ring_done)
        return ring[:rows]

    def snapshot_ring_copied(self):
        self._snap_ring_done = torch.cuda.Event()
        self._snap_ring_done.record()

    def forward(self):
        L.check(self.lib.gfl_fit_forward(ctypes.byref(self.state()), ctypes.byref(self.hp), L.stream()), "fit forward")

    def backward_step(self):
        L.check(self.lib.gfl_fit_backward_step(ctypes.byref(self.state()), ctypes.byref(self.hp), L.stream()),
                "fit backward/step")
        self._reserved_N = self.N

    GFL_ITER_RESERVED = 8

    def _reserved_flag(self):
        if self._reserved_N != self.N or self.N <= 0:
            return 0
        key = (self.W, self.H, self.K_cap)
        if self._reserved_sup[0] != key:
            self._reserved_sup = (key, int(self.lib.gfl_fit_reserved_supported(ctypes.byref(self.state()),
                                                                                ctypes.byref(self.hp))))
        return self.GFL_ITER_RESERVED if self._reserved_sup[1] else 0

    def iteration(self, use_graph=False, count=1, snapshot=False, flags=0, reserved=None):
        if snapshot:
            from .color import lut
            assert count == 1
            if self._snap_out is None:
                self._snap_out = torch.empty(3, self.H, self.W, 3, dtype=torch.uint8, device=self.dev)
            snap_args = (L.ptr(lut("turbo", self.dev)), L.ptr(self._snap_out))
        reserved = 0 if (flags or reserved is False or snapshot) else self._reserved_flag()
        gkey = ("snap", count, reserved) if snapshot else (count, reserved)
        if use_graph and not PROFILE["mask"] and self._launched and not flags:
            key = bytes(self.state()) + bytes(self.hp)
            if self._graph_key != key:
                self._retire_graphs()
                self._graph_key = key
            g = self._graphs.get(gkey)
            if g is None:
                if self._capture_stream is None:
                    self._capture_stream = torch.cuda.Stream(device=self.dev)
                side = self._capture_stream
                cur = torch.cuda.current_stream()
                st, hp = self.state(), self.hp
                with _GRAPH_LOCK:
                    gc_on = _gc.isenabled()
                    _gc.disable()
                    try:
                        g = torch.cuda.CUDAGraph()
                        side.wait_stream(cur)
                        with torch.cuda.stream(side):
                            g.capture_begin(capture_error_mode="thread_local")
                            try:
                                if snapshot:
                                    L.check(self.lib.gfl_fit_iteration_snapshot(ctypes.byref(st), ctypes.byref(hp), *snap_args,
                                                                                L.stream()), "snapshot iteration (capture)")
                                else:
                                    L.check(self.lib.gfl_fit_iterations(ctypes.byref(st), ctypes.byref(hp), count, reserved,
                                                                        L.stream()), "fit iterations (capture)")
                            finally:
                                g.capture_end()
                        cur.wait_stream(side)
                    finally:
                        if gc_on:
                            _gc.enable()
                self._graphs[gkey] = g
            g.replay()
            self._reserved_N = self.N
            return self._snap_out if snapshot else None
        if snapshot:
            L.check(self.lib.gfl_fit_iteration_snapshot(ctypes.byref(self.state()), ctypes.byref(self.hp), *snap_args, L.stream()),
                    "snapshot iteration")
        else:
            L.check(self.lib.gfl_fit_iterations(ctypes.byref(self.state()), ctypes.byref(self.hp), count, int(flags) | reserved,
                                                L.stream()), "fit iterations")
        self._reserved_N = self.N
        self._launched = True
        return self._snap_out if snapshot else None

    def snapshot(self, out=None):
        from .color import lut
        need = self.lib.gfl_fit_snapshot_workspace_bytes(self.N, self.W, self.H)
        if self._snap_ws is None or self._snap_ws.numel() < need:
            self._snap_ws = torch.empty(int(need * 1.5), dtype=torch.uint8, device=self.dev)
        if out is None:
            out = torch.empty(3, self.H, self.W, 3, dtype=torch.uint8, device=self.dev)
        L.check(self.lib.gfl_fit_snapshot(ctypes.byref(self.state()), ctypes.byref(self.hp), L.ptr(lut("turbo", self.dev)),
                                          L.ptr(out), L.ptr(self._snap_ws), self._snap_ws.numel(), L.stream()), "snapshot")
        return out

    _STATE_TENSORS = ("step", "pose", "pose_m", "pose_v", "depth_ab", "ab_m", "ab_v")

    def save_state(self):
        n = self.N
        out = {"N": n, "rows": [t[:n].clone() for t in (self.params, self.adam_m, self.adam_v)]}
        for k in self._STATE_TENSORS:
            out[k] = getattr(self, k).clone()
        return out

    def restore_state(self, saved):
        n = saved["N"]
        if n != self.N:
            raise RuntimeError("FitEngine.restore_state: the splat count has changed since save_state")
        self._reserved_N = -1
        for dst, src in zip((self.params, self.adam_m, self.adam_v), saved["rows"]):
            torch.bitwise_or(src.view(torch.int32), 0, out=dst[:n].view(torch.int32))
        for k in self._STATE_TENSORS:
            t = getattr(self, k)
            torch.bitwise_or(saved[k].view(torch.int32), 0, out=t.view(torch.int32))

    @property
    def uv(self):
        return self.rec[:self.N, 0:2]

    @property
    def depth(self):
        return self.rec[:self.N, 9:10]

    @property
    def K(self):
        return int(self.tile_offsets[self.T].item())

    def schedule(self, forward=False):
        nq, cap = ctypes.c_int(), ctypes.c_int()
        lists, counts = ctypes.c_void_p(), ctypes.c_void_p()
        fn = self.lib.gfl_fit_schedule_info_fwd if forward else self.lib.gfl_fit_schedule_info
        L.check(fn(ctypes.byref(self.state()), ctypes.byref(nq), ctypes.byref(cap),
                   ctypes.byref(lists), ctypes.byref(counts)), "fit schedule info")
        off_l = lists.value - self.workspace.data_ptr()
        off_c = counts.value - self.workspace.data_ptr()
        torch.cuda.synchronize(self.dev)
        lst = self.workspace[off_l:off_l + 4 * nq.value * cap.value].view(torch.int32).reshape(nq.value, cap.value).cpu()
        cnt = self.workspace[off_c:off_c + 4 * nq.value].view(torch.int32).cpu()
        return [(lst[c, :int(cnt[c])] & 0xffff).long() for c in range(nq.value)]

    def check_overflow(self):
        self._ovf_event = None
        code = int(self.overflow[0].item())
        self.reap_graphs()
        if code:
            self.overflow.zero_()
            raise RuntimeError(self._overflow_message(code))

    def settle_overflow(self):
        self._ovf_event = None
        self._pend_event = None
        code, skipped = (int(v) for v in self.overflow[:2].tolist())
        self.reap_graphs()
        if code == 0:
            if skipped > 0:
                self._count_void(skipped)
            return max(skipped, 0)
        if code != 1:
            self.overflow.zero_()
            raise RuntimeError(self._overflow_message(code))
        self._double_pairs()
        self.overflow.zero_()
        return max(skipped, 0)

    def _count_void(self, skipped):
        self.overflow[1:2].zero_()
        self.regions_outgrown += skipped

    def _double_pairs(self):
        self._K_grown = True
        self._alloc_pairs(2 * self.K_cap)
        with _GRAPH_LOCK:
            self._graphs.clear()
        self._graph_key = None
        self.pairs_grown += 1

    def grow_pairs(self):
        self._pend_event = None
        self._double_pairs()

    def _overflow_message(self, code):
        if code == 2:
            return ("FitEngine: an iteration was told that the previous one had run its preprocess / reserved its tile regions, "
                    "and it had not")
        return f"FitEngine: more than K_cap={self.K_cap} splat-tile pairs; raise K_cap"

    def watch_pending(self):
        if self._pend_host is None:
            self._pend_host = torch.zeros(8, dtype=torch.int32, pin_memory=True)
        self._pend_host[0:5].copy_(self._offsets_and_flags[self.T:self.T + 5], non_blocking=True)
        self._pend_event = torch.cuda.Event()
        self._pend_event.record()

    def pending_ready(self):
        return self._pend_event is None or self._pend_event.query()

    def read_pending(self):
        if self._pend_event is None:
            return None
        self._pend_event.synchronize()
        self._pend_event = None
        v = self._pend_host.tolist()
        return v[1], v[2], v[0]

    def drop_pending(self):
        self._pend_event = None

    def take_pending(self):
        got = self.read_pending()
        if got is None:
            return None
        code, skipped, pairs = got
        if code != 0 or 2 * pairs > self.K_cap:
            if code == 0:
                torch.cuda.current_stream().synchronize()
                self.grow_pairs()
            return -1
        if skipped > 0:
            self._count_void(skipped)
        return max(skipped, 0)

    def watch_overflow(self):
        self.poll_overflow()
        if self._ovf_host is None:
            self._ovf_host = torch.zeros(1, dtype=torch.int32, pin_memory=True)
        self._ovf_host.copy_(self.overflow[0:1], non_blocking=True)
        self._ovf_event = torch.cuda.Event()
        self._ovf_event.record()

    def poll_overflow(self):
        ev = self._ovf_event
        if ev is not None and ev.query():
            self._ovf_event = None
            if int(self._ovf_host[0]):
                self.overflow.zero_()
                raise RuntimeError(self._overflow_message(int(self._ovf_host[0])))

    def loss_terms(self):
        hw = float(self.H * self.W)
        return self.sums[0] / hw + (1.0 - self.sums[1] / (3.0 * hw)), self.sums[2] / hw
```

gflow_amd/stage.py:

```python
from types import SimpleNamespace

import torch

from . import geometry, losses
from . import render as render_mod
from .optim import LinearLR
from .pinned import PINNED, copy_stream


class StagePlan(SimpleNamespace):

    def snapshot(self, i):
        return bool(self.snapshot_interval) and i % self.snapshot_interval == 0

    def log(self, i):
        return bool(self.log_interval) and i % self.log_interval == 0

    def occ_densify(self, i):
        return bool(self.occlusion) and i == 0

    def err_densify(self, i):
        return bool(not self.camera_only and self.densify_interval and (i + 1) % self.densify_interval == 0
                    and (i + 1) // self.densify_interval <= self.densify_times)

    def plain(self, i):
        return not (self.snapshot(i) or self.log(i) or self.occ_densify(i) or self.err_densify(i))


class ListSink:
    copy_stream = snap_stream = None

    def __init__(self):
        self.lists = ([], [], [])

    def put(self, *images):
        for lst, img in zip(self.lists, images):
            lst.append(img)

    def flush(self, lazy=False):
        pass

    def images(self):
        return [[f for f in torch.stack(lst).cpu().numpy()] if lst else [] for lst in self.lists]


class RingSink(ListSink):

    def __init__(self, eng, plan, H, W, dev):
        super().__init__()
        self.eng, self.plan, self.H, self.W, self.dev = eng, plan, H, W, dev
        self.pin = self.pin_block = self.pin_hold = self.ring = None
        self.copy_stream = None
        self.snap_stream = None

    def slot(self, k):
        if self.pin is None or k >= self.pin.shape[0]:
            self._grow(k)
        self.put(*self.pin[k])
        return self.ring[k]

    def _grow(self, k):
        H, W, p = self.H, self.W, self.plan
        n_snaps = max((p.iterations + p.snapshot_interval - 1) // p.snapshot_interval, 2 * k, 1)
        block = PINNED.take(n_snaps * 3 * H * W * 3)
        pin = block[0][:n_snaps * 3 * H * W * 3].view(n_snaps, 3, H, W, 3)
        hold = PINNED.hold(block, self)
        PINNED.release(block)
        ring = self.eng.snapshot_ring(n_snaps)
        if self.pin is not None:
            if self.snap_stream is not None:
                torch.cuda.current_stream().wait_stream(self.snap_stream)
            ring[:k].copy_(self.ring[:k])
            self.lists = tuple([pin[j, c] for j in range(k)] for c in range(3))
            self.pin_hold()
        self.pin_block, self.pin, self.pin_hold, self.ring = block, pin, hold, ring
        self.copy_stream = copy_stream(self.dev)

    def copy_out(self, t):
        block = PINNED.take(t.numel())
        pin = block[0][:t.numel()].view(t.shape)
        cs = copy_stream(self.dev)
        cs.wait_stream(torch.cuda.current_stream())
        with torch.cuda.stream(cs):
            pin.copy_(t, non_blocking=True)
        PINNED.copied(block, cs)
        t.record_stream(cs)
        if self.copy_stream is None:
            self.copy_stream = cs
        return block, pin

    def flush(self, lazy=False):
        k = len(self.lists[0])
        if self.pin is not None and k:
            self.copy_stream.wait_stream(torch.cuda.current_stream())
            if self.snap_stream is not None:
                self.copy_stream.wait_stream(self.snap_stream)
            with torch.cuda.stream(self.copy_stream):
                self.pin[:k].copy_(self.ring[:k], non_blocking=True)
                self.eng.snapshot_ring_copied()
            PINNED.copied(self.pin_block, self.copy_stream)
            self.ring.record_stream(self.copy_stream)
        if self.copy_stream is not None and not lazy:
            self.copy_stream.synchronize()

    def images(self):
        out = [PINNED.hand_out(self.pin_block, lst) if lst else [] for lst in self.lists]
        if self.pin_hold is not None:
            self.lists, self.pin = ([], [], []), None
            self.pin_hold()
        return out


class _Stage:

    def __init__(self, tr, p, sink):
        self.tr, self.plan, self.sink = tr, p, sink
        self.log = []
        self.iteration = 0
        self.move_mask, self.camera_only = p.move_mask, p.camera_only
        self.uv = self.depth = self.last_render = None
        self.yielding = False

    @property
    def frames(self):
        return self.sink.lists[0]

    def __call__(self):
        self.one_iteration()

    def run(self, n):
        for _ in range(n):
            self.one_iteration()


class OperatorStage(_Stage):

    def __init__(self, tr, p):
        super().__init__(tr, p, ListSink())
        tr.add_optimizer(p.lr, p.lr_camera, depth_invariant=True)
        tr.scheduler = LinearLR(tr.optimizer, start_factor=1.0, end_factor=0.1, total_iters=p.iterations)
        self.later_frame = tr.later_frame

    def one_iteration(self):
        tr, p, iteration, camera_only = self.tr, self.plan, self.iteration, self.camera_only
        snap = p.snapshot(iteration)
        uv, depth, render4, extras = tr._render_rgbd(want_extras=snap)
        within = geometry.within(uv.detach(), tr.W, tr.H)
        tr.within_index = within
        mm = p.move_mask
        if tr.still_mask_tentative is not None and camera_only:
            with torch.no_grad():
                grp = tr._input_group(sel=~tr.still_mask_tentative, detach=True)
                mrgb = render_mod.render_multiple(grp, ["rgb"])["rgb"]
                tr.rasterisations_done += 1
                grey = 0.299 * mrgb[0] + 0.587 * mrgb[1] + 0.114 * mrgb[2]
                mm = (grey > 0.0) | self.move_mask
            self.move_mask = mm
        loss, loss_rgb_pixel, l_rgb, l_depth = losses.image_loss(
            render4, tr.gt_image, tr.gt_depth if p.lambda_depth > 0 else None, tr.depth_ab,
            p.lambda_rgb if p.lambda_rgb > 0 else 0.0, p.lambda_depth if p.lambda_depth > 0 else 0.0,
            mm if camera_only else None)
        terms = {"rgb": l_rgb, "depth": l_depth}

        valid = tr._stage_rows(within, camera_only)
        if p.lambda_var:
            l_var = losses.var_loss(tr.get_attribute("scale"))
            loss = loss + p.lambda_var * l_var
            terms["var"] = l_var
        if p.lambda_scale:
            l_scale = losses.scale_loss(tr.get_attribute("scale"), valid, depth[valid])
            loss = loss + p.lambda_scale * l_scale
            terms["scale"] = l_scale
        still = tr._still_selection(p.lambda_still)
        if still is not None:
            m, last_xyz = still
            diff = torch.norm(tr.get_attribute("xyz")[:m.shape[0]] - last_xyz, dim=1)
            l_still = (diff * m).sum() / m.sum().clamp(min=1)
            loss = loss + p.lambda_still * l_still
            terms["still"] = l_still
        flow = tr._flow_selection(p.lambda_flow, camera_only)
        if flow is not None:
            and_mask, gt_f = flow
            d = (uv[:tr.last_num] - tr.last_uv - gt_f) ** 2
            l_flow = (d * and_mask.unsqueeze(1)).sum() / (2.0 * and_mask.sum().clamp(min=1))
            loss = loss + p.lambda_flow * l_flow
            terms["flow"] = l_flow

        tr.optimizer.zero_grad()
        loss.backward()
        if self.later_frame and tr._attributes["rgb"].grad is not None:
            tr._attributes["rgb"].grad.zero_()
        if tr.has_still and tr._attributes["xyz"].grad is not None:
            tr._attributes["xyz"].grad[:tr.still_mask.shape[0]] *= (~tr.still_mask).unsqueeze(1)
        if camera_only:
            for q in tr._attributes.values():
                if q.grad is not None:
                    q.grad.zero_()
        tr.optimizer.step()
        tr.scheduler.step()
        tr.iterations_done += 1
        if p.log(iteration):
            self.log.append({k: float(v.detach()) for k, v in terms.items()}
                            | {"total": float(loss.detach()), "it": iteration})

        if p.occ_densify(iteration):
            if p.mask.sum() > 0:
                tr.densify_by_pixels(torch.ones_like(loss_rgb_pixel), error_threshold=0.0,
                                     percent=p.densify_occ_percent, mask=p.mask)
        if p.err_densify(iteration):
            tr.densify_by_pixels(loss_rgb_pixel, error_threshold=p.densify_err_thre, percent=p.densify_err_percent,
                                 mask=None)
        if snap:
            self.sink.put(render_mod.render2img_device(render4[:3]), render_mod.render2img_device(extras[0]),
                          render_mod.render2img_device(extras[1]))
        self.uv, self.depth, self.last_render = uv.detach(), depth.detach(), render4.detach()
        self.iteration += 1


class FusedStage(_Stage):

    def __init__(self, tr, p):
        tr.lr, tr.lr_camera = p.lr, p.lr_camera
        eng = self.eng = tr._pack_to_engine()
        super().__init__(tr, p, RingSink(eng, p, tr.H, tr.W, tr.device))
        eng.drop_pending()
        eng.pose.copy_(tr.pose.detach())
        eng.invalidate_regions()
        tr.pose = eng.pose
        eng.depth_ab.zero_()
        eng.depth_ab[0:1].fill_(1.0)
        tr.depth_ab = eng.depth_ab
        eng.intr.copy_(tr.intr)
        eng.reset_optimizer()
        hp = eng.hp
        hp.bg = tr.bg
        hp.lambda_rgb = p.lambda_rgb if p.lambda_rgb > 0 else 0.0
        hp.lambda_depth = p.lambda_depth if p.lambda_depth > 0 else 0.0
        hp.lambda_var, hp.lr, hp.lr_camera = p.lambda_var, p.lr, p.lr_camera
        hp.lambda_scale = float(p.lambda_scale or 0.0)
        hp.lr_end_factor, hp.total_iters = 0.1, p.iterations
        hp.freeze_rgb = 1 if tr.later_frame else 0
        hp.freeze_all_splats = 1 if p.camera_only else 0
        hp.step_camera = 1
        hp.lambda_flow = hp.lambda_still = 0.0
        self._set_regularisers()
        move_mask, camera_only = p.move_mask, p.camera_only
        eng.set_targets(tr.gt_image, tr.gt_depth if p.lambda_depth > 0 else None,
                        (~move_mask) if (camera_only and move_mask is not None) else None)
        self.tentative = tr.still_mask_tentative is not None and camera_only
        if self.tentative:
            eng.set_footprint_mask(move_mask if move_mask is not None else torch.zeros(tr.H, tr.W, dtype=torch.bool),
                                   ~tr.still_mask_tentative)
        self.unchecked = 0

    def _set_regularisers(self):
        tr, p, eng, dev = self.tr, self.plan, self.eng, self.tr.device
        n, hp = eng.N, eng.hp
        flow_target = flow_w = still_target = still_w = row_flags = None
        if tr.has_still:
            row_flags = torch.zeros(n, dtype=torch.uint8, device=dev)
            row_flags[:tr.still_mask.shape[0]] = tr.still_mask.to(torch.uint8) | 2
        still = tr._still_selection(p.lambda_still)
        if still is not None:
            m, last_xyz = still
            still_target = torch.zeros(n, 3, device=dev)
            still_target[:m.shape[0]] = last_xyz
            still_w = torch.zeros(n, device=dev)
            still_w[:m.shape[0]] = m.float() / m.sum().clamp(min=1)
            hp.lambda_still = p.lambda_still
        flow = tr._flow_selection(p.lambda_flow, p.camera_only)
        if flow is not None:
            and_mask, gt_f = flow
            flow_target = torch.zeros(n, 2, device=dev)
            flow_target[:tr.last_num] = tr.last_uv + gt_f
            flow_w = torch.zeros(n, device=dev)
            flow_w[:tr.last_num] = and_mask.float() / (2.0 * and_mask.sum().clamp(min=1))
            hp.lambda_flow = p.lambda_flow
        eng.set_regularisers(flow_target, flow_w, still_target, still_w, row_flags)

    def note_forward(self, n_rendered, rec=None):
        rec = self.eng.rec if rec is None else rec
        self.uv, self.depth, self.last_render = rec[:n_rendered, 0:2], rec[:n_rendered, 9:10], self.eng.render

    def settle(self, last=None):
        while True:
            k = self.eng.settle_overflow()
            if not k:
                return
            for _ in range(k - 1 if last else k):
                self.eng.iteration(use_graph=False)
            if last:
                last()

    def account(self):
        k = self.eng.take_pending()
        if k is None:
            if self.unchecked:
                self.settle()
        elif k < 0:
            self.settle()
        else:
            for _ in range(k):
                self.eng.iteration(use_graph=False, reserved=False)

    def _launch(self, dst, n_rendered, looked_at):
        tr, eng = self.tr, self.eng
        if dst is not None and not tr.async_snapshots:
            imgs = eng.iteration(use_graph=tr.use_graph, snapshot=True, reserved=False)
            torch.bitwise_or(imgs, 0, out=dst)
        else:
            eng.iteration(use_graph=tr.use_graph, reserved=None if not looked_at else False)
            if dst is not None:
                tr._snapshot_async(dst, n_rendered)
                self.sink.snap_stream = tr._snap_stream

    def one_iteration(self):
        tr, eng, p, iteration = self.tr, self.eng, self.plan, self.iteration
        n_rendered = eng.N
        looked_at = not p.plain(iteration)
        if looked_at and tr.exact_snapshots:
            self.account()
        if self.tentative:
            tr.rasterisations_done += 1
        dst = None
        if p.snapshot(iteration):
            dst = self.sink.slot(len(self.frames))
        launch = lambda: self._launch(dst, n_rendered, looked_at)
        launch()
        if looked_at and tr.exact_snapshots == "blocking":
            self.settle(last=launch)
        self.unchecked = 0 if looked_at else self.unchecked + 1
        tr.rasterisations_done += 1
        tr.iterations_done += 1
        rec_now = eng.rec
        if p.log(iteration):
            self.log.append(self._log_entry(iteration))
        densified = self._densify(iteration, launch)
        self.note_forward(n_rendered, rec_now)
        if densified:
            self.uv, self.depth = self.uv.clone(), self.depth.clone()
            eng.reset_optimizer(splats=True, camera=False)
            eng.hp.total_iters = 0
            eng.hp.step_camera = 0
        self.iteration += 1

    def _log_entry(self, iteration):
        eng, hp, lambda_var = self.eng, self.eng.hp, self.plan.lambda_var
        l_rgb, l_depth = eng.loss_terms()
        total = hp.lambda_rgb * l_rgb + hp.lambda_depth * l_depth
        entry = {"rgb": float(l_rgb), "depth": float(l_depth), "it": iteration}
        if lambda_var:
            entry["var"] = float(losses.var_loss(torch.abs(eng.views()["scale"])))
            total = total + lambda_var * entry["var"]
        entry["total"] = float(total)
        return entry

    def _densify(self, iteration, launch):
        tr, eng, p = self.tr, self.eng, self.plan
        densified = False
        if not tr.exact_snapshots and p.err_densify(iteration):
            self.settle(last=launch)
        if p.occ_densify(iteration):
            b, n = tr.densify_by_pixels(torch.ones_like(eng.err_px), error_threshold=0.0,
                                        percent=p.densify_occ_percent, mask=p.mask, n_masked=p.mask_count)
            densified |= n > b
        if p.err_densify(iteration):
            b, n = tr.densify_by_pixels(eng.err_px, error_threshold=p.densify_err_thre,
                                        percent=p.densify_err_percent, mask=None)
            densified |= n > b
        return densified

    def _plain(self, b, **how):
        n_rendered = self.eng.N
        self.eng.iteration(count=b, **how)
        self.note_forward(n_rendered)
        self.tr.rasterisations_done += (2 * b) if self.tentative else b
        self.tr.iterations_done += b
        self.iteration += b

    def run(self, n):
        tr, eng, plain, iterations = self.tr, self.eng, self.plan.plain, self.plan.iterations
        end = self.iteration + n
        while self.iteration < end:
            i = self.iteration
            if self.yielding and not plain(i) and tr.exact_snapshots and not eng.pending_ready():
                return
            if plain(i) and not plain(i + 1) and i + 1 < iterations and tr.exact_snapshots:
                if self.unchecked:
                    eng.watch_pending()
                    self.unchecked = 0
                self._plain(1, use_graph=tr.use_graph, reserved=False)
                continue
            k = 0
            while (k < 4 and i + k < end and plain(i + k)
                   and (plain(i + k + 1) or i + k + 1 >= iterations or not tr.exact_snapshots)):
                k += 1
            if k < 2 or not tr.use_graph:
                self.one_iteration()
                continue
            self._plain(4 if k == 4 else 2, use_graph=True)
            self.unchecked += 4 if k == 4 else 2
```

gflow_amd/trainer.py:

```python
import math
import os

import numpy as np
import torch
import torch.nn as nn
import torch.nn.functional as F

from . import _lib as L
from . import geometry, msplat
from . import render as render_mod
from .geometry import device_constant, pose_to_extr, rotmat_to_unitquat_xyzw
from .optim import Adam
from .pinned import PINNED
from .sampling import complex_texture_sampling
from .stage import FusedStage, OperatorStage, StagePlan


def run_to_end(g):
    try:
        while True:
            next(g)
    except StopIteration as e:
        return e.value


class SimpleGaussian:
    def __init__(self, gt_image, gt_depth=None, gt_flow=None, num_points=100000, background="black",
                 device=None, log_dir=None, seed=None, fused=True, deterministic=None):
        self.fused = bool(fused)
        self.deterministic = L.resolve_deterministic(deterministic)
        if self.deterministic and not self.fused and deterministic is not None:
            raise ValueError("SimpleGaussian(deterministic=True) needs fused=True: the operator path's alpha_blending "
                             "backward has no deterministic implementation")
        self.async_snapshots = True
        self.exact_snapshots = True
        self.cu_count = 0
        self.use_graph = True
        self.engine = None
        self.device = torch.device(device if device is not None else "cuda")
        if self.device.type != "cuda":
            raise RuntimeError("gflow_amd.trainer needs a HIP device (there is no CPU rasteriser)")
        self.gt_image = gt_image.to(self.device)
        self.gt_depth = gt_depth.to(self.device) if gt_depth is not None else None
        self.gt_flow = gt_flow.to(self.device) if gt_flow is not None else None
        self.num_points = num_points
        H, W, _ = gt_image.shape
        self.H, self.W = H, W
        self.bg = {"black": 0.0, "white": 1.0, "cyan": 0.33}.get(background, 0.0)
        fov = math.pi / 2.0
        fx = 0.5 * float(W) / math.tan(0.5 * fov)
        fy = 0.5 * float(H) / math.tan(0.5 * fov)
        self.intr = device_constant([fx, fy, W / 2.0, H / 2.0], self.device)
        self.pose = device_constant([0.0, 0.0, 0.0, 1.0, 0.0, 0.0, 0.0], self.device)
        self.rng = np.random.default_rng(seed)
        self.gen = torch.Generator(device=self.device)
        self.gen.manual_seed(0 if seed is None else int(seed))
        N = int(num_points)
        self._activations = {
            "scale": torch.abs,
            "rotate": F.normalize,
            "opacity": lambda x: torch.sigmoid(x * 10.0),
            "rgb": torch.sigmoid,
        }
        self._activations_inv = {
            "scale": torch.abs,
            "rotate": F.normalize,
            "opacity": lambda x: torch.logit(x) / 10.0,
            "rgb": torch.logit,
        }
        rand = lambda *s: torch.rand(*s, device=self.device, generator=self.gen)
        self._attributes = {
            "xyz": rand(N, 3) * 2 - 1,
            "scale": rand(N, 3),
            "rotate": F.normalize(rand(N, 4)),
            "opacity": self._activations_inv["opacity"](0.99 * torch.ones(N, 1, device=self.device)),
            "rgb": rand(N, 3),
        }
        self.dir = log_dir
        if log_dir is not None:
            os.makedirs(log_dir, exist_ok=True)
        self.move_seg = None
        self.seg_recorder = None
        self.iterations_done = 0
        self.rasterisations_done = 0
        self.lr = self.lr_camera = None
        self.train_log = self.last_render = None
        self.still_mask = self.still_mask_tentative = self.last_still_mask = self.last_uv = self.last_depth = None
        self.last_xyz = self.last_num = self.move_seg_erode = self.mask_prompt_pts = self.propagate_seg = None
        self.traj_xyz = self.traj_scale = self.traj_rotate = self.traj_opacity = self.traj_rgb = self.last_traj_group = None
        self._engine_live = False
        self._aux = self._snap_aux = self._snap_stream = self._snap_done = None

    @property
    def later_frame(self):
        return self.last_xyz is not None

    @property
    def has_still(self):
        return self.still_mask is not None

    @property
    def engine_current(self):
        return self.fused and self.engine is not None and self.engine.N == self.current_pts_num()

    @property
    def engine_live(self):
        return (self.engine_current and self._engine_live
                and self._attributes["xyz"].data_ptr() == self.engine.params.data_ptr())

    def set_gt_image(self, gt_image):
        self.gt_image = gt_image.to(self.device)

    def set_gt_depth(self, gt_depth):
        self.gt_depth = gt_depth.to(self.device)

    def set_gt_flow(self, gt_flow):
        self.gt_flow = gt_flow.to(self.device)

    def get_extr(self):
        return pose_to_extr(self.pose)

    def load_camera(self, focal=None, pp=None, extr=None, scale=None, show=False):
        if focal is not None:
            self.intr[:2].fill_(float(focal))
        if pp is not None:
            self.intr[2:3].fill_(float(pp[0]))
            self.intr[3:4].fill_(float(pp[1]))
        if extr is not None:
            extr = torch.as_tensor(extr, dtype=torch.float32, device=self.device)
            T = extr[:3, 3] * (scale if scale is not None else 1.0)
            pose = self.pose.detach().clone()
            pose[0:4] = rotmat_to_unitquat_xyzw(extr[:3, :3])
            pose[4:7] = T
            self.pose = pose
        if show:
            print("[camera] intr:", self.intr, "\n[camera] extr:\n", self.get_extr())

    def current_pts_num(self):
        return self._attributes["xyz"].shape[0]

    def get_attribute(self, name):
        if name not in self._attributes:
            raise ValueError(f"Attribute or activation for {name} is not VALID!")
        act = self._activations.get(name)
        return act(self._attributes[name]) if act is not None else self._attributes[name]

    def init_gaussians_from_image(self, gt_image, gt_depth=None, num_points=None, mask=None, drop_to=None):
        num_points = self.num_points if num_points is None else num_points
        self._engine_live = False
        if mask is None and drop_to is None:
            from .sampling import complex_texture_sampling_device
            img = gt_image.to(self.device)
            self.gt_depth = gt_depth.float().to(self.device)
            xys, depths, scales, rgbs = complex_texture_sampling_device(img, self.gt_depth, num_points, generator=self.gen,
                                                                        deterministic=self.deterministic)
            n = xys.shape[0]
            xys, depths = xys.float(), depths.float()
            scales = (scales * (depths / depths.min()).squeeze(1).double()).float()
            rgbs = rgbs.float()
        else:
            xys, depths, scales, rgbs, gt_depth = complex_texture_sampling(
                gt_image, gt_depth.cpu(), num_points=num_points, mask=mask, drop_to=drop_to, rng=self.rng)
            n = xys.shape[0]
            xys = torch.from_numpy(xys).float().to(self.device)
            depths = depths.float().to(self.device)
            self.gt_depth = gt_depth.float().to(self.device)
            scales = torch.from_numpy(scales * (depths / depths.min()).squeeze().cpu().numpy()).float().to(self.device)
            rgbs = torch.from_numpy(rgbs).float().contiguous().to(self.device)
        self._attributes["xyz"] = geometry.pix2world(xys, depths, self.intr, self.get_extr().detach())
        scales = scales.unsqueeze(1).repeat(1, 3)
        self._attributes["scale"] = self._activations_inv["scale"](torch.clamp(scales, max=1e-3))
        rgbs = torch.clamp(rgbs.contiguous(), 1e-15, 1 - 1e-15)
        self._attributes["rgb"] = self._activations_inv["rgb"](rgbs)
        self._attributes["opacity"] = self._activations_inv["opacity"](0.99 * torch.ones(n, 1, device=self.device))
        self._attributes["rotate"] = F.normalize(torch.rand(n, 4, device=self.device, generator=self.gen))

    def add_optimizer(self, lr=1e-2, lr_camera=0.0, depth_invariant=True):
        self.lr, self.lr_camera = lr, lr_camera
        self._engine_live = False
        for k in self._attributes:
            self._attributes[k] = nn.Parameter(self._attributes[k].detach().contiguous()).requires_grad_(True)
        self.pose = nn.Parameter(self.pose.detach().clone()).requires_grad_(True)
        self.depth_ab = nn.Parameter(device_constant([1.0, 0.0], self.device)).requires_grad_(depth_invariant)
        groups = [{"params": list(self._attributes.values()), "lr": lr, "name": "attributes"},
                  {"params": [self.pose], "lr": lr_camera, "name": "extr"}]
        if depth_invariant:
            groups.append({"params": [self.depth_ab], "lr": lr, "name": "depth_ab"})
        self.optimizer = Adam(groups)

    def _input_group(self, sel=None, detach=False):
        g = []
        for k in ("xyz", "scale", "rotate", "opacity", "rgb"):
            a = self.get_attribute(k)
            if detach:
                a = a.detach()
            if sel is not None:
                a = a[:sel.shape[0]][sel]
            g.append(a)
        return g + [self.intr, self.get_extr(), self.bg, self.W, self.H]

    def _render_rgbd(self, want_extras):
        xyz, scale, rotate, opacity, rgb, intr, extr, bg, W, H = self._input_group()
        uv, depth = msplat.project_point(xyz, intr, extr, W, H)
        visible = depth != 0
        cov3d = msplat.compute_cov3d(scale, rotate, visible)
        conic, radius, tiles = msplat.ewa_project(xyz, cov3d, intr, extr, uv, W, H, visible)
        ids, tile_range = msplat.sort_gaussian(uv, depth, W, H, radius, tiles)
        self.last_K = ids.numel()
        render4 = msplat.alpha_blending(uv, conic, opacity, torch.cat([rgb, depth], dim=1), ids, tile_range, bg, W, H)
        extras = None
        if want_extras:
            with torch.no_grad():
                dc = render_mod.apply_float_colormap(depth.detach(), "turbo", non_zero=True)
                depth_color = msplat.alpha_blending(uv.detach(), conic.detach(), opacity.detach(), dc, ids,
                                                    tile_range, bg, W, H)
                unit = device_constant([1.0, 0.0, 1.0], self.device)
                center = msplat.alpha_blending(uv.detach(), torch.ones_like(conic) * unit,
                                               torch.ones_like(opacity.detach()), rgb.detach(), ids, tile_range, bg,
                                               W, H)
            extras = (depth_color, center)
        self.rasterisations_done += 1
        return uv, depth, render4, extras

    def init_mask_prompt_pts(self, mask_prompt, ckpt_name=None):
        with torch.no_grad():
            uv = render_mod.render_multiple(self._input_group(detach=True), ["uv", "center"])["uv"].detach()
        self.rasterisations_done += 1
        mask_prompt = torch.as_tensor(mask_prompt).to(self.device)
        within = geometry.within(uv, self.W, self.H)
        yx = uv.long()
        under = mask_prompt[yx[:, 1].clamp(0, self.H - 1), yx[:, 0].clamp(0, self.W - 1)].bool()
        self.mask_prompt_pts = within & under
        if self.dir is not None and ckpt_name is not None:
            from PIL import Image
            os.makedirs(os.path.join(self.dir, "images_seg"), exist_ok=True)
            Image.fromarray((mask_prompt.detach().cpu().numpy() * 255).astype(np.uint8)).save(
                os.path.join(self.dir, "images_seg", f"propagate_mask_{ckpt_name}.png"))
        return self.mask_prompt_pts

    def make_stepper(self, iterations=500, lr=1e-2, lr_camera=0.0, lambda_rgb=1.0, lambda_depth=0.0,
                     lambda_flow=0.0, lambda_var=0.0, lambda_still=0.0, lambda_scale=0.0, move_mask=None,
                     densify_interval=500, densify_times=1, mask=None, camera_only=False, densify_occ_percent=0.1,
                     densify_err_thre=1e-2, densify_err_percent=0.2, snapshot_interval=10, log_interval=0,
                     mask_count=None):
        if move_mask is not None:
            move_mask = move_mask.to(self.device).bool()
        if not camera_only and self.has_still:
            self._warp_moving()
        plan = StagePlan(iterations=iterations, lr=lr, lr_camera=lr_camera, lambda_rgb=lambda_rgb, lambda_depth=lambda_depth,
                         lambda_flow=lambda_flow, lambda_var=lambda_var, lambda_still=lambda_still, lambda_scale=lambda_scale,
                         move_mask=move_mask, densify_interval=densify_interval, densify_times=densify_times, mask=mask,
                         camera_only=camera_only, densify_occ_percent=densify_occ_percent, densify_err_thre=densify_err_thre,
                         densify_err_percent=densify_err_percent, snapshot_interval=snapshot_interval,
                         log_interval=log_interval, mask_count=mask_count,
                         occlusion=not camera_only and self.later_frame and mask is not None)
        return (FusedStage if self.fused else OperatorStage)(self, plan)

    def _warp_moving(self):
        W, H = self.W, self.H
        n_last = self.last_still_mask.shape[0]
        moving = ~self.last_still_mask
        uv_last = self.last_uv[:n_last]
        inside = geometry.within(uv_last, W, H) & moving
        yx = uv_last.long()
        flow_at = self.gt_flow[yx[:, 1].clamp(0, H - 1), yx[:, 0].clamp(0, W - 1)]
        uv_new = uv_last + flow_at
        yn = uv_new[:, 1].long().clamp(0, H - 1)
        xn = uv_new[:, 0].long().clamp(0, W - 1)
        depth_new = self.gt_depth[yn, xn]
        xyz_new = geometry.pix2world(uv_new, depth_new.reshape(-1, 1), self.intr, self.get_extr().detach())
        xyz = self._attributes["xyz"].detach().clone()
        xyz[:n_last] = torch.where(inside.unsqueeze(1), xyz_new, xyz[:n_last])
        self._attributes["xyz"] = xyz

    def _stage_rows(self, inside, camera_only):
        if not self.has_still:
            return inside
        n = self.still_mask.shape[0]
        out = inside.clone()
        out[:n] = (self.still_mask if camera_only else ~self.still_mask) & out[:n]
        return out

    def _still_selection(self, lambda_still):
        if not (lambda_still and self.has_still):
            return None
        m = self.last_still_mask
        return m, self.last_xyz[:m.shape[0]]

    def _flow_selection(self, lambda_flow, camera_only):
        if not (lambda_flow and self.gt_flow is not None and self.last_uv is not None):
            return None
        W, H = self.W, self.H
        and_mask = self._stage_rows(geometry.within(self.last_uv, W, H), camera_only)
        yx = self.last_uv.long()
        return and_mask, self.gt_flow[yx[:, 1].clamp(0, H - 1), yx[:, 0].clamp(0, W - 1)]

    def _new_engine(self, capacity, K_cap=None):
        from .fused import FitEngine
        return FitEngine(self.W, self.H, capacity, self.device, K_cap=K_cap, bg=self.bg, cu_count=self.cu_count,
                         deterministic=self.deterministic)

    def _engine_for(self, n):
        if self.engine is None:
            self.engine = self._new_engine(max(8 * int(self.num_points), 2 * n, 65536))
        self.engine.ensure_capacity(n)
        return self.engine

    def _pack_to_engine(self):
        eng = self._engine_for(self.current_pts_num())
        if not self.engine_live:
            eng.set_splats(self._attributes)
        self._attributes = eng.views()
        self._engine_live = True
        return eng

    def train(self, *a, **kw):
        return run_to_end(self.train_steps(*a, **kw))

    def train_steps(self, iterations=500, save_ckpt=False, ckpt_name="ckpt", snapshot_interval=10, render_parts=True,
                    lazy_images=False, chunk=None, move_seg=False, **kw):
        st = self.make_stepper(iterations=iterations, snapshot_interval=snapshot_interval, **kw)
        if chunk:
            st.yielding = True
            while st.iteration < iterations:
                st.run(min(int(chunk), iterations - st.iteration))
                yield
        else:
            st.run(iterations)
        self.train_log = st.log
        if self.fused and self.engine is not None:
            st.settle()
            if st.sink.snap_stream is not None:
                with torch.cuda.stream(st.sink.snap_stream):
                    self._snap_aux.watch_overflow()
        move_mask = kw.get("move_mask")
        if move_mask is not None:
            move_mask = move_mask.to(self.device).bool()

        self._project_appended(st)
        uv_d, depth_d = st.uv.clone(), st.depth.clone()
        if not st.camera_only:
            self._relabel_after_stage(uv_d, depth_d, move_mask, move_seg)
        parts, parts_block = (None, None, None, None), None
        if self.has_still and render_parts:
            parts, parts_block = self._render_parts(st.sink)
            self.rasterisations_done += 2
        self.last_render = st.last_render.clone()
        if save_ckpt:
            self.save_checkpoint(ckpt_name=ckpt_name)
        st.sink.flush(lazy_images)
        if parts_block is not None:
            parts = PINNED.hand_out(parts_block, [parts[0, 0], parts[0, 2], parts[1, 0], parts[1, 2]])
            PINNED.release(parts_block)
        frames, frames_depth, frames_center = st.sink.images()
        return (frames, frames_center, frames_depth, *parts, self.move_seg)

    def _project_appended(self, st):
        if st.uv.shape[0] == self.current_pts_num():
            return
        with torch.no_grad():
            if self.fused and self.engine is not None:
                self.engine.forward()
                st.uv, st.depth, st.last_render = self.engine.uv, self.engine.depth, self.engine.render
            else:
                st.uv, st.depth, st.last_render, _ = self._render_rgbd(want_extras=False)
            self.rasterisations_done += 1

    def _relabel_after_stage(self, uv_d, depth_d, move_mask, move_seg):
        W, H, dev = self.W, self.H, self.device
        within = geometry.within(uv_d, W, H)
        yx = uv_d.long()
        labels = ~move_mask[yx[:, 1].clamp(0, H - 1), yx[:, 0].clamp(0, W - 1)]
        n_now = self.current_pts_num()
        still = torch.ones(n_now, dtype=torch.bool, device=dev)
        still[:uv_d.shape[0]] = torch.where(within, labels, still[:uv_d.shape[0]])
        self.still_mask = still
        self.still_mask_tentative = still.clone()
        if self.last_still_mask is not None:
            self.still_mask[:self.last_still_mask.shape[0]] = self.last_still_mask
        if move_seg:
            from .hull import FastConcaveHull2D
            from scipy.ndimage import minimum_filter
            sel = within & ~self.still_mask[:uv_d.shape[0]]
            pts = uv_d[sel].cpu().numpy()
            if pts.shape[0] > 5:
                self.move_seg = (FastConcaveHull2D(pts).mask(W, H) * 255).astype(np.uint8)
                self.move_seg_erode = minimum_filter(self.move_seg, size=20, mode="constant", cval=255)
        if self.seg_recorder is not None:
            self.seg_recorder.record(uv_d, within & ~self.still_mask[:uv_d.shape[0]])
        if self.mask_prompt_pts is not None:
            from .hull import FastConcaveHull2D
            m = self.mask_prompt_pts
            p_uv = uv_d[:m.shape[0]][m]
            p_uv = p_uv[geometry.within(p_uv, W, H)]
            if p_uv.shape[0] > 4:
                self.propagate_seg = (FastConcaveHull2D(p_uv.cpu().numpy()).mask(W, H) * 255).astype(np.uint8)
        self.last_still_mask = self.still_mask.detach()
        self.last_uv = uv_d
        self.last_depth = depth_d
        self.last_xyz = self.get_attribute("xyz").detach()
        self.last_num = self.last_xyz.shape[0]

    def _render_parts(self, sink):
        if self.fused and self.engine is not None and self.engine.N == self.still_mask.shape[0]:
            block, pin = sink.copy_out(self._render_parts_fused())
            return pin, block
        with torch.no_grad():
            o = render_mod.render_multiple(self._input_group(sel=self.still_mask, detach=True), ["rgb", "center"])
            still_rgb, still_center = render_mod.render2img(o["rgb"]), render_mod.render2img(o["center"])
            o = render_mod.render_multiple(self._input_group(sel=~self.still_mask, detach=True), ["rgb", "center"])
            move_rgb, move_center = render_mod.render2img(o["rgb"]), render_mod.render2img(o["center"])
        return (still_rgb, still_center, move_rgb, move_center), None

    def _snapshot_async(self, out, n):
        import ctypes
        eng = self.engine
        cur = torch.cuda.current_stream()
        if not self._fits(self._snap_aux, n, eng.K_cap):
            if self._snap_aux is not None:
                self._snap_stream.synchronize()
            else:
                self._snap_stream = torch.cuda.Stream(device=self.device)
            self._snap_aux = self._new_engine(max(eng.cap, n), eng.K_cap)
            self._snap_done = None
        aux, side = self._snap_aux, self._snap_stream
        if self._snap_done is not None:
            cur.wait_event(self._snap_done)
        aux.set_count(n)
        aux.hp.bg, aux.hp.nearest, aux.hp.extent = eng.hp.bg, eng.hp.nearest, eng.hp.extent
        L.check(eng.lib.gfl_fit_snapshot_stage(ctypes.byref(eng.state()), ctypes.byref(aux.state()), L.stream()),
                "snapshot stage")
        ready = torch.cuda.Event()
        ready.record(cur)
        with torch.cuda.stream(side):
            side.wait_event(ready)
            aux.snapshot(out=out)
            self._snap_done = torch.cuda.Event()
            self._snap_done.record(side)

    @staticmethod
    def _fits(aux, n, K_cap=None):
        return aux is not None and aux.cap >= n and (K_cap is None or aux.K_cap >= K_cap)

    def _aux_engine(self):
        eng = self.engine
        if not self._fits(self._aux, eng.N):
            self._aux = self._new_engine(max(eng.cap, eng.N))
        aux = self._aux
        aux.set_count(eng.N)
        aux.pose.copy_(eng.pose)
        aux.intr.copy_(eng.intr)
        aux.hp.bg = self.bg
        return aux

    def _render_scene_fused(self):
        aux = self._aux_forward()
        out = aux.snapshot()
        aux.watch_overflow()
        return out

    def _aux_forward(self):
        aux, n = self._aux_engine(), self.engine.N
        aux.params[:n].copy_(self.engine.params[:n])
        aux.forward()
        return aux

    def _render_parts_fused(self):
        eng, aux, n = self.engine, self._aux_engine(), self.engine.N
        out = []
        hidden = torch.full((), -1000.0, device=self.device)
        for sel in (self.still_mask, ~self.still_mask):
            aux.params[:n].copy_(eng.params[:n])
            aux.params[:n, 10] = torch.where(sel, eng.params[:n, 10], hidden)
            aux.forward()
            out.append(aux.snapshot())
        aux.watch_overflow()
        return torch.stack(out)

    def densify_weights(self, error_map, error_threshold=1e-3, mask=None):
        dev = self.device
        err = error_map.detach().float()
        inf = torch.full_like(err, float("inf"))
        pos_min = torch.where(err > 0, err, inf).min()
        err = err + torch.where(torch.isinf(pos_min), torch.ones_like(pos_min), pos_min)
        if mask is None:
            m = err > error_threshold
        else:
            m = mask.detach().to(dev).squeeze()
            if m.dim() == 3:
                m = m[..., 0] if m.shape[-1] in (1, 3) else m[0]
            m = m > 0
        m = m[:, :err.shape[1]]
        return err * m, m

    def new_splats_at(self, ys, xs):
        dev = self.device
        k = ys.shape[0]
        xys = torch.stack([xs, ys], dim=1).float()
        depths = self.gt_depth[ys, xs].reshape(-1, 1).float()
        scales = (depths / depths.min()).squeeze(1) * (1.0 / self.num_points)
        new_xyz = geometry.pix2world(xys, depths, self.intr, self.get_extr().detach())
        new_scale = torch.abs(scales.unsqueeze(1).repeat(1, 3))
        new_rgb = torch.logit(torch.clamp(self.gt_image[ys, xs].contiguous(), 1e-15, 1 - 1e-15))
        new_rot = torch.zeros(k, 4, device=dev)
        new_rot[:, 0] = 1.0
        new_op = torch.logit(0.99 * torch.ones(k, 1, device=dev)) / 10.0
        return new_xyz, new_scale, new_rot, new_op, new_rgb

    def densify_by_pixels(self, error_map, error_threshold=1e-3, percent=0.1, mask=None, n_masked=None):
        W = self.W
        if n_masked == 0:
            return self.current_pts_num(), self.current_pts_num()
        err, m = self.densify_weights(error_map, error_threshold, mask)
        if n_masked is None:
            n_masked = int(m.sum())
            if self.fused and self.engine is not None:
                self.engine.reap_graphs()
        densify_num = int(self.num_points * (n_masked / m.numel()) * percent)
        num_before = self.current_pts_num()
        if densify_num > 0:
            idx = self.sample_pixels(err, densify_num)
            self.last_densify_idx = idx
            self.densification_postfix(*self.new_splats_at(idx // W, idx % W))
        return num_before, self.current_pts_num()

    def sample_pixels(self, weights, count):
        from .sampling import cdf_device
        cdf = cdf_device(weights, self.deterministic)
        u = torch.rand(count, generator=self.gen, device=self.device, dtype=torch.float64) * cdf[-1]
        return torch.searchsorted(cdf, u, right=True).clamp_(max=cdf.numel() - 1)

    def densification_postfix(self, new_xyz, new_scale, new_rotate, new_opacity, new_rgb):
        new = {"xyz": new_xyz, "scale": new_scale, "rotate": new_rotate, "opacity": new_opacity, "rgb": new_rgb}
        eng = self.engine
        if self.engine_live:
            from .fused import COLS
            n0, k = eng.N, new_xyz.shape[0]
            eng.ensure_capacity(n0 + k)
            rows = eng.params[n0:n0 + k]
            for name, (a, b) in COLS.items():
                rows[:, a:b] = new[name].detach().reshape(k, b - a)
            rows[:, 14:] = 0
            eng.set_count(n0 + k)
            self._attributes = eng.views()
            return
        for k in self._attributes:
            cat = torch.cat((self._attributes[k].detach(), new[k]), dim=0).contiguous()
            self._attributes[k] = nn.Parameter(cat).requires_grad_(True)
        self.optimizer = Adam(list(self._attributes.values()), lr=self.lr)

    def save_checkpoint(self, ckpt_name=None):
        if self.dir is None:
            raise RuntimeError("save_checkpoint: this trainer was built without log_dir")
        ckpt = {
            "attributes": {k: v.detach().clone().contiguous() for k, v in self._attributes.items()},
            "intr": self.intr,
            "extr": self.get_extr().detach().clone(),
            "still_mask": self.still_mask,
            "move_seg": self.move_seg,
            "last_uv": self.last_uv,
            "width": self.W,
            "height": self.H,
        }
        os.makedirs(os.path.join(self.dir, "ckpt"), exist_ok=True)
        self.checkpoint_path = os.path.join(self.dir, "ckpt", f"{ckpt_name or 'ckpt'}.tar")
        torch.save(ckpt, self.checkpoint_path)

    def load_checkpoint(self, checkpoint_path):
        ckpt = torch.load(checkpoint_path, map_location=self.device, weights_only=False)
        self._engine_live = False
        self._attributes = {k: v.to(self.device) for k, v in ckpt["attributes"].items()}
        self.intr = ckpt["intr"].to(self.device)
        self.load_camera(extr=ckpt["extr"])
        for k in ("still_mask", "move_seg", "last_uv"):
            if ckpt.get(k) is not None:
                setattr(self, k, ckpt[k])

    def eval(self, traj_index=None, line_scale=0.1, point_scale=0.3, alpha=0.5, split_interval=None):
        traj_index = torch.as_tensor(traj_index, device=self.device).long()
        current_xyz = self.get_attribute("xyz")[traj_index].detach().float()
        with torch.no_grad():
            out_traj = self.eval_trajectories(current_xyz, self.get_extr().detach(), line_scale, point_scale, alpha, split_interval)
            out = render_mod.render_multiple(self._input_group(detach=True), ["rgb", "center", "depth_map_color"])
            self.rasterisations_done += 1
        out_img = render_mod.render2img(out["rgb"])
        out_img_center = render_mod.render2img(out["center"])
        out_img_depth = render_mod.render2img(out["depth_map_color"])
        out_img_traj = render_mod.render2img(out_traj)
        result = 1 - (1 - np.array(out_img) / 255.0) * (1 - np.array(out_img_traj) / 255.0)
        return out_img, out_img_center, out_img_depth, out_img_traj, (result * 255).astype(np.uint8)

    def eval_trajectories(self, current_xyz, extr, line_scale=0.1, point_scale=0.3, alpha=0.5, split_interval=None):
        from .color import apply_float_colormap
        from .trajectory import gen_line_set
        dev = self.device
        num_traj = current_xyz.shape[0]
        op_inv = self._activations_inv["opacity"]
        if self.traj_xyz is None:
            self.traj_xyz = current_xyz
            self.traj_scale = torch.ones((num_traj, 3), device=dev)
            self.traj_rotate = torch.tensor([1.0, 0.0, 0.0, 0.0], device=dev).repeat(num_traj, 1)
            self.traj_opacity = op_inv(0.99 * torch.ones((num_traj, 1), device=dev))
            if split_interval is None or num_traj == split_interval:
                traj_rgb = torch.arange(0, 1, 1 / num_traj, device=dev).float().unsqueeze(1)
            else:
                still = torch.arange(0, 1, 1 / split_interval, device=dev).float().unsqueeze(1)
                move = torch.arange(0, 1, 1 / (num_traj - split_interval), device=dev).float().unsqueeze(1)
                traj_rgb = torch.cat([still, move], dim=0)
            traj_rgb = apply_float_colormap(traj_rgb, colormap="gist_rainbow")
            self.traj_rgb = torch.nan_to_num(self._activations_inv["rgb"](traj_rgb), posinf=1e6, neginf=-1e6)
            self.last_traj_xyz = self.traj_xyz
            self.last_traj_rgb = self.traj_rgb
        else:
            line_xyz, line_rgb = gen_line_set(self.last_traj_xyz, current_xyz, self.last_traj_rgb, device=dev)
            num_in_line = line_xyz.shape[0]
            self.traj_xyz = torch.cat([self.traj_xyz, line_xyz], dim=0)
            num_total = self.traj_xyz.shape[0]
            self.traj_scale = torch.ones((num_total, 3), device=dev) * 1e-6
            self.traj_rotate = torch.tensor([1.0, 0.0, 0.0, 0.0], device=dev).repeat(num_total, 1)
            self.traj_opacity = torch.cat([self.traj_opacity * alpha,
                                           op_inv(0.99 * torch.ones((num_in_line, 1), device=dev))], dim=0)
            self.traj_rgb = torch.cat([self.traj_rgb, line_rgb], dim=0)
            self.last_traj_xyz = current_xyz
        traj_group = [self.traj_xyz, self.traj_scale, self.traj_rotate, self.traj_opacity, self.traj_rgb, self.intr, extr,
                      self.bg, self.W, self.H]
        self.last_traj_group = traj_group
        self.rasterisations_done += 1
        return render_mod.render_traj(traj_group, num_traj, line_scale, point_scale)

    def project_points(self, points):
        return msplat.project_point(points, self.intr, self.get_extr(), self.W, self.H)

    def psnr(self):
        return self.psnr_of(self.last_render)

    def psnr_of(self, render4):
        img = torch.floor(torch.clamp(render4[:3].permute(1, 2, 0), 0.0, 1.0) * 255.0) / 255.0
        mse = ((img - self.gt_image) ** 2).mean()
        return -10.0 * torch.log10(mse)
```

include/gflow_hip.h:

```cpp
#ifndef GFLOW_HIP_H
#define GFLOW_HIP_H

#include <stddef.h>
#include <stdint.h>

#ifdef __cplusplus
extern "C" {
#endif

typedef void* gfl_stream_t;

typedef enum gfl_status {
    GFL_OK = 0,
    GFL_ERR_INVALID = -1,
    GFL_ERR_WORKSPACE = -2,
    GFL_ERR_HIP = -3
} gfl_status;

#define GFL_TILE 16
#ifndef GFL_NEAREST
#define GFL_NEAREST 0.2f
#endif
#ifndef GFL_EXTENT
#define GFL_EXTENT 1.3f
#endif
#ifndef GFL_FOV_CLAMP
#define GFL_FOV_CLAMP 1.3f
#endif
#ifndef GFL_LOWPASS
#define GFL_LOWPASS 0.3f
#endif
#ifndef GFL_EIG_FLOOR
#define GFL_EIG_FLOOR 0.1f
#endif
#ifndef GFL_RADIUS_SIGMA
#define GFL_RADIUS_SIGMA 3.0f
#endif
#ifndef GFL_ALPHA_MIN
#define GFL_ALPHA_MIN (1.0f / 255.0f)
#endif
#ifndef GFL_ALPHA_MAX
#define GFL_ALPHA_MAX 0.99f
#endif
#ifndef GFL_T_MIN
#define GFL_T_MIN 1e-4f
#endif
#ifndef GFL_PIXEL_CENTER
#define GFL_PIXEL_CENTER 0.0f
#endif
#define GFL_MAX_BLEND_CHANNELS 4

#define GFL_VERSION 312
int gfl_version(void);
int gfl_constants(float* out10);
#define GFL_N_CONSTANTS 11
int gfl_constants_n(float* out, int n);
int gfl_ewa_on_mfma(void);
const char* gfl_status_string(int status);
int gfl_last_hip_error(void);
size_t gfl_reduce_workspace_bytes(int N);
size_t gfl_reduce_cam_workspace_bytes(int N);

int gfl_project_point_fwd(const float* xyz, const float* intr, const float* extr, int N, int W, int H,
                          float nearest, float extent, float* uv, float* depth, gfl_stream_t stream);
int gfl_project_point_bwd(const float* xyz, const float* intr, const float* extr, const float* depth,
                          const float* d_uv, const float* d_depth, int N, float* d_xyz, float* d_extr,
                          void* workspace, size_t workspace_bytes, gfl_stream_t stream);
int gfl_project_point_bwd_cam(const float* xyz, const float* intr, const float* extr, const float* depth,
                              const float* d_uv, const float* d_depth, int N, float* d_xyz, float* d_extr,
                              float* d_intr, void* workspace, size_t workspace_bytes, gfl_stream_t stream);

int gfl_cov3d_fwd(const float* scale, const float* rotate, const uint8_t* visible, int N, float* cov3d,
                  gfl_stream_t stream);
int gfl_cov3d_bwd(const float* scale, const float* rotate, const uint8_t* visible, const float* d_cov3d,
                  int N, float* d_scale, float* d_rotate, gfl_stream_t stream);

int gfl_ewa_fwd(const float* xyz, const float* cov3d, const float* intr, const float* extr, const float* uv,
                const uint8_t* visible, int N, int W, int H, float* conic, int32_t* radius,
                int32_t* tiles_touched, gfl_stream_t stream);
int gfl_ewa_bwd(const float* xyz, const float* cov3d, const float* intr, const float* extr,
                const int32_t* radius, const float* d_conic, int N, int W, int H, float* d_xyz,
                float* d_cov3d, float* d_extr, void* workspace, size_t workspace_bytes, gfl_stream_t stream);
int gfl_ewa_bwd_cam(const float* xyz, const float* cov3d, const float* intr, const float* extr,
                    const int32_t* radius, const float* d_conic, int N, int W, int H, float* d_xyz,
                    float* d_cov3d, float* d_extr, float* d_intr, void* workspace, size_t workspace_bytes,
                    gfl_stream_t stream);

size_t gfl_bin_workspace_bytes(int N, int K_cap, int W, int H);
int gfl_bin_count(const float* uv, const int32_t* radius, const float* cutoff, int N, int W, int H,
                  int32_t* tile_offsets, gfl_stream_t stream);
int gfl_bin_sort(const float* uv, const float* depth, const int32_t* radius, const float* cutoff, int N, int W,
                 int H, const int32_t* tile_offsets, int K_cap, int32_t* ids, int32_t* tile_range,
                 int32_t* overflow, void* workspace, size_t workspace_bytes, gfl_stream_t stream);

int gfl_blend_fwd(const float* uv, const float* conic, const float* opacity, const float* feature,
                  int C_total, int c0, int C, const int32_t* ids, const int32_t* tile_range, float bg, int W,
                  int H, float* out, float* final_T, int32_t* n_contrib, gfl_stream_t stream);
int gfl_blend_bwd(const float* uv, const float* conic, const float* opacity, const float* feature,
                  int C_total, int c0, int C, const int32_t* ids, const int32_t* tile_range, float bg, int W,
                  int H, const float* final_T, const int32_t* n_contrib, const float* d_out, int N,
                  float* d_uv, float* d_conic, float* d_opacity, float* d_feature, int zero_first,
                  gfl_stream_t stream);

int gfl_sh_fwd(const float* shs, const float* dirs, const uint8_t* visible, int N, int K, float* out,
               gfl_stream_t stream);
int gfl_sh_bwd(const float* shs, const float* dirs, const uint8_t* visible, const float* d_out, int N, int K,
               float* d_shs, float* d_dirs, gfl_stream_t stream);

int gfl_colormap_nonzero(const float* value, int N, const float* lut, float* out, void* workspace,
                         size_t workspace_bytes, gfl_stream_t stream);

size_t gfl_loss_workspace_bytes(int W, int H);
int gfl_loss_fwd_bwd_partials(const float* render, const float* gt_rgb, const float* gt_depth, const uint8_t* keep,
                              const float* depth_ab, float lambda_rgb, float lambda_depth, int W, int H,
                              float* d_render, float* err_px, void* workspace, size_t workspace_bytes,
                              const float** p_ssim, int* n_ssim, const float** p_grad, int* n_grad,
                              gfl_stream_t stream);
int gfl_loss_prepare_gt(const float* gt_rgb, const uint8_t* keep, int W, int H, float* gt_stats, gfl_stream_t stream);
int gfl_loss_fwd_bwd_partials_cached(const float* render, const float* gt_rgb, const float* gt_depth,
                                     const uint8_t* keep, const float* depth_ab, float lambda_rgb, float lambda_depth,
                                     int W, int H, float* d_render, float* err_px, void* workspace,
                                     size_t workspace_bytes, const float* gt_stats, const float** p_ssim, int* n_ssim,
                                     const float** p_grad, int* n_grad, gfl_stream_t stream);
int gfl_loss_fwd_bwd(const float* render, const float* gt_rgb, const float* gt_depth, const uint8_t* keep,
                     const float* depth_ab, float lambda_rgb, float lambda_depth, int W, int H,
                     float* d_render, float* err_px, float* sums, void* workspace, size_t workspace_bytes,
                     gfl_stream_t stream);

int gfl_adam_step(float* param, const float* grad, float* m, float* v, int64_t n, int row_len,
                  const uint8_t* row_zero_grad, float lr, float beta1, float beta2, float eps,
                  const int32_t* d_step, float lr_end_factor, int total_iters, gfl_stream_t stream);
int gfl_step_increment(int32_t* d_step, gfl_stream_t stream);

typedef struct gfl_fit_state {
    int32_t N, cap, W, H, K_cap;
    int32_t gt_cached;
    float *params, *adam_m, *adam_v;
    float *rec, *d_rec;
    const float *flow_target, *flow_w, *still_target, *still_w;
    const uint8_t* row_flags;
    float *pose, *pose_m, *pose_v;
    float *depth_ab, *depth_ab_m, *depth_ab_v;
    const float* intr;
    float* extr;
    float* d_extr;
    int32_t* step;
    const float* gt_rgb;
    const float* gt_depth;
    uint8_t* keep;
    const uint8_t* move_mask;
    const uint8_t* foot_flags;
    float *render, *final_T;
    int32_t* n_contrib;
    float *d_render, *err_px, *sums;
    int32_t *tile_offsets, *ids, *tile_range, *overflow;
    void* workspace;
    size_t workspace_bytes;
    int32_t cu_count;
    int32_t flags;
} gfl_fit_state;

#define GFL_FIT_DETERMINISTIC 1

typedef struct gfl_fit_hyper {
    float bg, nearest, extent;
    float lambda_rgb, lambda_depth, lambda_var, lambda_flow, lambda_still;
    float lambda_scale;
    float lr, lr_camera, beta1, beta2, eps, lr_end_factor;
    int32_t total_iters;
    int32_t freeze_rgb;
    int32_t freeze_all_splats;
    int32_t step_camera;
} gfl_fit_hyper;

size_t gfl_fit_workspace_bytes(int cap, int K_cap, int W, int H);
int gfl_fit_workspace_layout(int cap, int K_cap, int W, int H,
                             const char** names, size_t* offsets, size_t* bytes, int max);
int gfl_fit_forward(const gfl_fit_state* st, const gfl_fit_hyper* hp, gfl_stream_t stream);
int gfl_fit_backward_step(const gfl_fit_state* st, const gfl_fit_hyper* hp, gfl_stream_t stream);
int gfl_fit_iteration(const gfl_fit_state* st, const gfl_fit_hyper* hp, gfl_stream_t stream);
#define GFL_ITER_RESERVED 8
int gfl_fit_iterations(const gfl_fit_state* st, const gfl_fit_hyper* hp, int count, int flags, gfl_stream_t stream);
int gfl_fit_reserved_supported(const gfl_fit_state* st, const gfl_fit_hyper* hp);
int gfl_render_fwd(const gfl_fit_state* st, const gfl_fit_hyper* hp, gfl_stream_t stream);
int gfl_render_bwd(const gfl_fit_state* st, const gfl_fit_hyper* hp, const float* d_render, const float* d_uv,
                   const float* d_depth, float* d_params, float* d_extr, gfl_stream_t stream);
int gfl_render_bwd_cam(const gfl_fit_state* st, const gfl_fit_hyper* hp, const float* d_render, const float* d_uv,
                       const float* d_depth, float* d_params, float* d_extr, float* d_intr, gfl_stream_t stream);
size_t gfl_render_batch_workspace_bytes(int J, int rows_total, int K_cap, int W, int H);
int gfl_render_batch(const float* params, int R, const int32_t* job_rows, const float* job_cam, int J, int rows_total, int W,
                     int H, int K_cap, float* out_f32, uint8_t* out_u8, float* out_rec, int32_t* overflow, void* workspace,
                     size_t workspace_bytes, gfl_stream_t stream);
size_t gfl_fit_snapshot_workspace_bytes(int N, int W, int H);
int gfl_fit_snapshot(const gfl_fit_state* st, const gfl_fit_hyper* hp, const float* lut, uint8_t* out_u8, void* workspace,
                     size_t workspace_bytes, gfl_stream_t stream);
int gfl_fit_iteration_snapshot(const gfl_fit_state* st, const gfl_fit_hyper* hp, const float* lut, uint8_t* out_u8,
                               gfl_stream_t stream);
int gfl_fit_snapshot_stage(const gfl_fit_state* src, const gfl_fit_state* dst, gfl_stream_t stream);
int gfl_fit_prepare_targets(const gfl_fit_state* st, gfl_stream_t stream);
int gfl_fit_schedule_info(const gfl_fit_state* st, int* n_queues, int* queue_capacity, const int32_t** d_lists,
                          const int32_t** d_counts);
int gfl_fit_schedule_info_fwd(const gfl_fit_state* st, int* n_queues, int* queue_capacity, const int32_t** d_lists,
                              const int32_t** d_counts);
int gfl_tile_sort_only(const int32_t* tile_offsets, int T, int K_cap, void* keys, int32_t* ids,
                       int32_t* tile_range, gfl_stream_t stream);
#define GFL_SORT_MAX_SPLIT 64
#define GFL_SORT_ORDER_TRAILER (GFL_SORT_MAX_SPLIT + 4)
int gfl_tile_sort_ordered(const int32_t* order, int W, int H, int K_cap, void* keys, int32_t* ids, int32_t* tile_range,
                          gfl_stream_t stream);
int gfl_tile_sort_reserved(const int32_t* order, const int32_t* fill, int32_t* tile_counts, int32_t* void_words, int W, int H,
                           int K_cap, void* keys, int32_t* ids, int32_t* tile_range, gfl_stream_t stream);

int gfl_selftest_reduce10(const float* in, float* out_scatter, float* out_dpp, gfl_stream_t stream);
int gfl_selftest_cov2d(const float* m, const float* cov, int n, float* out_valu, float* out_mfma, gfl_stream_t stream);
int gfl_selftest_block_mask(const float* rec, int n, int x0, int y0, int box, int32_t* mask, int32_t* truth, gfl_stream_t stream);

int gfl_concave_hull(const double* points_xy, int n, double concavity, double length_threshold, double* ring_xy,
                     int cap_vertices);

#define GFL_SCAN_CHUNK 2048
size_t gfl_scan_f64_workspace_bytes(int n);
int gfl_scan_f64(const double* in, int n, double* out, void* workspace, size_t workspace_bytes, gfl_stream_t stream);

size_t gfl_track_anchor_workspace_bytes(int n_new, int N);
int gfl_track_anchor(const float* uv, int uv_stride, int N, const double* query_xy, int n_new, int32_t* anchor,
                     double* shift_xy, void* workspace, size_t workspace_bytes, gfl_stream_t stream);
int gfl_track_frame(const float* uv, int uv_stride, const float* depth, int depth_stride, int N, const float* depth_map,
                    int W, int H, const int32_t* anchor, const double* shift_xy, int n_anchored, int frame, int T,
                    float occ_threshold, float* tracks, uint8_t* occluded, gfl_stream_t stream);

int gfl_track_history(const float* uv, int uv_stride, const float* depth, int depth_stride, int N, const float* depth_map,
                      int W, int H, float occ_threshold, float* hist_uv, uint8_t* hist_occ, gfl_stream_t stream);
size_t gfl_track_backward_workspace_bytes(int Q, int T);
int gfl_track_backward(const float* hist_uv, const uint8_t* hist_occ, const int64_t* row_start, int T,
                       const double* query_xy, const int32_t* query_frame, int Q, float* tracks, uint8_t* occluded,
                       int32_t* back_anchor, void* workspace, size_t workspace_bytes, gfl_stream_t stream);

int gfl_seg_score(const uint8_t* pred, const uint8_t* gt, const uint8_t* valid, int T, int H, int W, int radius,
                  uint32_t* counts, gfl_stream_t stream);

size_t gfl_recon_workspace_bytes(int W, int H);
int gfl_recon_frame(const float* render, const float* gt_rgb, int W, int H, int frame, int T, double* sums, void* workspace,
                    size_t workspace_bytes, gfl_stream_t stream);

size_t gfl_flow_workspace_bytes(int W, int H);
int gfl_flow_pair(const float* rec_a, int n_a, const int32_t* ids, const int32_t* tile_range, const float* uv_b,
                  int uv_b_stride, const float* depth_b, int depth_b_stride, int n_b, const float* gt_flow,
                  const uint8_t* move_mask, int W, int H, float min_weight, int pair, int n_pairs, double* sums,
                  float* flow_out, uint8_t* valid_out, void* workspace, size_t workspace_bytes, gfl_stream_t stream);

size_t gfl_epi_workspace_bytes(int W, int H, int K);
int gfl_epi_fundamental(const float* flow, int W, int H, const int32_t* samples, int K, double* F_all, double* medians,
                        double* F_best, int32_t* best, void* workspace, size_t workspace_bytes, gfl_stream_t stream);
int gfl_epi_mask(const float* flow, int W, int H, const double* F, double threshold, float* err_norm, uint8_t* mask,
                 uint8_t* open, uint8_t* erode, uint8_t* dilate, void* workspace, size_t workspace_bytes, gfl_stream_t stream);

int gfl_flow_occlusion(const float* fwd, const float* bwd, int n_pairs, int W, int H, float alpha, float beta,
                       float* diff_fwd, float* diff_bwd, uint8_t* occ_fwd, uint8_t* occ_bwd, gfl_stream_t stream);

int gfl_abi_sizes(int* sizeof_fit_state, int* sizeof_fit_hyper);

#define GFL_PROFILE_STAGES 9
int gfl_profile_enable(unsigned stage_mask);
int gfl_profile_read(double* total_ms, int* counts, int n_stages);

#ifdef __cplusplus
}
#endif
#endif
```

Baseline: 10.26.

## Fuse stage begin/end bookkeeping and densify append into HIP kernels

Adds HIP kernels for the per-stage relabel step (stage_end), the stage-begin target and Adam-state reset (stage_begin), and densification row append. These replace chains of small PyTorch ops and host round-trips, with the fused engine writing new splats directly into its parameter and optimizer buffers. Snapshots can now render only the requested images (RGB, depth, center), so the parts render skips the depth blend and the final stack copy. This adds new code paths that must match the original PyTorch semantics exactly.

```diff
diff --git a/gflow_amd/_lib.py b/gflow_amd/_lib.py
--- a/gflow_amd/_lib.py
+++ b/gflow_amd/_lib.py
@@ -63,6 +63,7 @@
     "gfl_fit_snapshot_stage": (c_int, [_P, _P, _P]),
     "gfl_fit_snapshot_workspace_bytes": (c_size_t, [c_int, c_int, c_int]),
     "gfl_fit_snapshot": (c_int, [_P, _P, _P, _P, _P, c_size_t, _P]),
+    "gfl_fit_snapshot_images": (c_int, [_P, _P, _P, _P, _P, c_size_t, c_int, _P]),
     "gfl_fit_iteration_snapshot": (c_int, [_P, _P, _P, _P, _P]),
     "gfl_render_fwd": (c_int, [_P, _P, _P]),
     "gfl_render_bwd": (c_int, [_P, _P, _P, _P, _P, _P, _P, _P]),
@@ -95,6 +96,10 @@
     "gfl_epi_fundamental": (c_int, [_P, c_int, c_int, _P, c_int, _P, _P, _P, _P, _P, c_size_t, _P]),
     "gfl_epi_mask": (c_int, [_P, c_int, c_int, _P, ctypes.c_double, _P, _P, _P, _P, _P, _P, c_size_t, _P]),
     "gfl_flow_occlusion": (c_int, [_P, _P, c_int, c_int, c_int, c_float, c_float, _P, _P, _P, _P, _P]),
+    "gfl_stage_end": (c_int, [_P, c_int, _P, c_int, c_int, _P, c_int, c_int, _P, _P, _P, _P, _P, _P]),
+    "gfl_stage_begin_workspace_bytes": (c_size_t, []),
+    "gfl_stage_begin": (c_int, [_P, _P, c_int, _P, _P, c_int, _P, c_int, _P, c_int, c_int, _P, _P, c_size_t, _P]),
+    "gfl_densify_append": (c_int, [_P, _P, _P, c_int, c_int, _P, c_int, _P, _P, c_int, c_int, _P, _P, _P, c_float, _P, _P]),
     "gfl_abi_sizes": (c_int, [_P, _P]),
     "gfl_profile_enable": (c_int, [ctypes.c_uint]),
     "gfl_profile_read": (c_int, [_P, _P, c_int]),
@@ -173,6 +178,31 @@
     return out
 
 
+def mask_u8(t):
+    if t.dtype == torch.bool:
+        return t.contiguous().view(torch.uint8)
+    return (t != 0).contiguous().view(torch.uint8)
+
+
+def stage_end(rec, n_rendered, move_mask, last_still, n_now):
+    need_device(rec, move_mask, last_still)
+    if rec.dtype != torch.float32 or rec.dim() != 2 or rec.shape[1] != 12 or not rec.is_contiguous() or rec.shape[0] < n_rendered:
+        raise ValueError("stage_end: rec must be a contiguous (rows >= n_rendered, 12) float32 tensor")
+    H, W = move_mask.shape
+    dev = rec.device
+    mm = mask_u8(move_mask)
+    ls = None if last_still is None else mask_u8(last_still)
+    n_last = 0 if ls is None else ls.shape[0]
+    still = torch.empty(n_now, dtype=torch.bool, device=dev)
+    tentative = torch.empty(n_now, dtype=torch.bool, device=dev)
+    uv = torch.empty(n_rendered, 2, dtype=torch.float32, device=dev)
+    depth = torch.empty(n_rendered, 1, dtype=torch.float32, device=dev)
+    sel = torch.empty(n_rendered, dtype=torch.bool, device=dev)
+    check(load().gfl_stage_end(ptr(rec), int(n_rendered), ptr(mm), int(W), int(H), ptr(ls), int(n_last), int(n_now),
+                               ptr(still), ptr(tentative), ptr(uv), ptr(depth), ptr(sel), stream()), "stage end")
+    return still, tentative, uv, depth, sel
+
+
 def resolve_deterministic(deterministic):
     return torch.are_deterministic_algorithms_enabled() if deterministic is None else bool(deterministic)
 
diff --git a/gflow_amd/csrc/gfl_fit.hip b/gflow_amd/csrc/gfl_fit.hip
--- a/gflow_amd/csrc/gfl_fit.hip
+++ b/gflow_amd/csrc/gfl_fit.hip
@@ -296,23 +296,37 @@
 
 int gfl_fit_snapshot(const gfl_fit_state* st, const gfl_fit_hyper* hp, const float* lut, uint8_t* out_u8, void* workspace,
                      size_t workspace_bytes, gfl_stream_t stream) {
+    return gfl_fit_snapshot_images(st, hp, lut, out_u8, workspace, workspace_bytes, GFL_SNAP_ALL, stream);
+}
+
+int gfl_fit_snapshot_images(const gfl_fit_state* st, const gfl_fit_hyper* hp, const float* lut, uint8_t* out_u8, void* workspace,
+                            size_t workspace_bytes, int images, gfl_stream_t stream) {
     int rc = fit_check(st, hp);
     if (rc) return rc;
-    if (!lut || !out_u8 || !workspace) return GFL_ERR_INVALID;
-    if (workspace_bytes < gfl_fit_snapshot_workspace_bytes(st->N, st->W, st->H)) return GFL_ERR_WORKSPACE;
+    if (!out_u8 || (images & ~GFL_SNAP_ALL)) return GFL_ERR_INVALID;
+    const bool want_dc = images & GFL_SNAP_DEPTH, want_c = images & GFL_SNAP_CENTER;
+    if (want_dc && !lut) return GFL_ERR_INVALID;
+    if (want_dc || want_c) {
+        if (!workspace) return GFL_ERR_INVALID;
+        if (workspace_bytes < gfl_fit_snapshot_workspace_bytes(st->N, st->W, st->H)) return GFL_ERR_WORKSPACE;
+    }
+    if (!images) return GFL_OK;
     hipStream_t s = (hipStream_t)stream;
     const auto [gx, gy, T] = tile_grid(st->W, st->H);
     const FitWs w = carve(st);
     const SnapWs sw = snap_ws(workspace, st->W, st->H);
-    rc = check(hipMemsetAsync(workspace, 0, sw.head_bytes, s));
-    if (rc) return rc;
-    if (st->N > 0) launch_rec_depth_range(st->rec, st->N, sw.mm, s);
-    launch_center_blend(st, hp->bg, gx, T, sw.img_c, nullptr, s);
-    {
+    if (want_dc) {
+        rc = check(hipMemsetAsync(workspace, 0, sw.head_bytes, s));
+        if (rc) return rc;
+        if (st->N > 0) launch_rec_depth_range(st->rec, st->N, sw.mm, s);
+    }
+    if (want_c) launch_center_blend(st, hp->bg, gx, T, sw.img_c, nullptr, s);
+    if (want_dc) {
         const TileQueue q = {w.sched_fwd.list, w.sched_fwd.count, sw.pull, w.sched.nq, w.sched.cap_q};
         launch_blend_fwd(st, hp->bg, gx, blend_grid(st, T, FWD_WG_PER_CU), sw.img_dc, sw.fT, sw.nc, q, w, 1, sw.mm, lut, fwd_split_min(), s);
     }
-    launch_snapshot_u8(st->render, sw.img_dc, sw.img_c, st->W * st->H, out_u8, s);
+    launch_snapshot_u8((images & GFL_SNAP_RGB) ? st->render : nullptr, want_dc ? sw.img_dc : nullptr, want_c ? sw.img_c : nullptr,
+                       st->W * st->H, out_u8, s);
     return check_launch();
 }
 
diff --git a/gflow_amd/csrc/gfl_fit_snap.hip b/gflow_amd/csrc/gfl_fit_snap.hip
--- a/gflow_amd/csrc/gfl_fit_snap.hip
+++ b/gflow_amd/csrc/gfl_fit_snap.hip
@@ -110,6 +110,7 @@
     const float* src[3] = {a, b, c};
 #pragma unroll
     for (int k = 0; k < 3; ++k) {
+        if (!src[k]) continue;
 #pragma unroll
         for (int ch = 0; ch < 3; ++ch) {
             out[((size_t)k * P + i) * 3 + ch] = img_u8(src[k][(size_t)ch * P + i]);
diff --git a/gflow_amd/csrc/gfl_stage.hip b/gflow_amd/csrc/gfl_stage.hip
--- /dev/null
+++ b/gflow_amd/csrc/gfl_stage.hip
@@ -0,0 +1,307 @@
+#include "gfl_fit.hpp"
+
+namespace gfl {
+
+constexpr int STAGE_BLOCK = 256;
+constexpr int STAGE_COUNT_BLOCKS = 256;
+constexpr int MIN_BLOCK = 1024;
+
+__device__ __forceinline__ bool uv_within(float u, float v, int W, int H) {
+    return u > 0.f && u < (float)(W - 1) && v > 0.f && v < (float)(H - 1);
+}
+
+__device__ __forceinline__ int trunc_clamp(float x, int n) {
+    const float t = truncf(x);
+    if (!(t > 0.f)) return 0;
+    return t >= (float)(n - 1) ? n - 1 : (int)t;
+}
+
+__device__ __forceinline__ void pix2world(const Cam& c, float u, float v, float d, float (&out)[3]) {
+#pragma clang fp contract(off)
+    const float r0 = d * (u - c.cx) / c.fx, r1 = d * (v - c.cy) / c.fx, r2 = d;
+    const float b0 = -(c.r00 * c.t0 + c.r10 * c.t1 + c.r20 * c.t2);
+    const float b1 = -(c.r01 * c.t0 + c.r11 * c.t1 + c.r21 * c.t2);
+    const float b2 = -(c.r02 * c.t0 + c.r12 * c.t1 + c.r22 * c.t2);
+    out[0] = (r0 * c.r00 + r1 * c.r10 + r2 * c.r20) + b0;
+    out[1] = (r0 * c.r01 + r1 * c.r11 + r2 * c.r21) + b1;
+    out[2] = (r0 * c.r02 + r1 * c.r12 + r2 * c.r22) + b2;
+}
+
+__device__ __forceinline__ int block_sum_int(int v, int* s_part) {
+#pragma unroll
+    for (int off = 32; off >= 1; off >>= 1) v += __shfl_xor(v, off);
+    const int wave = threadIdx.x >> 6, nw = blockDim.x >> 6;
+    if ((threadIdx.x & 63) == 0) s_part[wave] = v;
+    __syncthreads();
+    int t = 0;
+    for (int w = 0; w < nw; ++w) t += s_part[w];
+    __syncthreads();
+    return t;
+}
+
+__global__ void __launch_bounds__(STAGE_BLOCK)
+    stage_end_kernel(const float* __restrict__ rec, int n_rendered, const uint8_t* __restrict__ move_mask, int W, int H,
+                     const uint8_t* __restrict__ last_still, int n_last, int n_now, uint8_t* __restrict__ still,
+                     uint8_t* __restrict__ tentative, float* __restrict__ uv_out, float* __restrict__ depth_out,
+                     uint8_t* __restrict__ sel_out) {
+    const int i = blockIdx.x * STAGE_BLOCK + threadIdx.x;
+    if (i >= n_now) return;
+    bool inside = false, label = true;
+    if (i < n_rendered) {
+        const float* r = rec + (size_t)i * REC;
+        const float u = r[0], v = r[1];
+        reinterpret_cast<float2*>(uv_out)[i] = make_float2(u, v);
+        depth_out[i] = r[9];
+        inside = uv_within(u, v, W, H);
+        if (inside) label = move_mask[(size_t)(int)v * W + (int)u] == 0;
+    }
+    const bool own = inside ? label : true;
+    const bool keep = i < n_last ? last_still[i] != 0 : own;
+    tentative[i] = own;
+    still[i] = keep;
+    if (i < n_rendered) sel_out[i] = inside && !keep;
+}
+
+struct BeginArgs {
+    const float* last_uv; int n_flow;
+    const float* gt_flow;
+    const uint8_t* still_mask; int n_lab;
+    const uint8_t* last_still; int n_still;
+    const float* last_xyz; int xyz_stride;
+    const float* warp_depth;
+    int camera_only, W, H, N, cap;
+    float *params, *adam_m, *adam_v;
+    const float *intr, *pose;
+    float *pose_m, *pose_v, *depth_ab, *depth_ab_m, *depth_ab_v;
+    int32_t* step;
+    float *flow_target, *flow_w, *still_target, *still_w;
+    uint8_t* row_flags;
+    int32_t* partial;
+    int count_blocks;
+};
+
+__device__ __forceinline__ bool flow_selected(const BeginArgs& a, int i, float u, float v) {
+    bool s = uv_within(u, v, a.W, a.H);
+    if (i < a.n_lab) s = s && ((a.still_mask[i] != 0) == (a.camera_only != 0));
+    return s;
+}
+
+__global__ void __launch_bounds__(STAGE_BLOCK) stage_count_warp_kernel(BeginArgs a) {
+    __shared__ int s_part[STAGE_BLOCK / 64];
+    const bool flow = a.flow_w != nullptr, still = a.still_w != nullptr, warp = a.warp_depth != nullptr;
+    const int n = max(a.n_flow, a.n_still);
+    Cam c{};
+    if (warp) c = cam_from_pose(a.intr, a.pose);
+    int c_flow = 0, c_still = 0;
+    for (int i = blockIdx.x * STAGE_BLOCK + threadIdx.x; i < n; i += gridDim.x * STAGE_BLOCK) {
+        float u = 0.f, v = 0.f;
+        if (i < a.n_flow) {
+            const float2 p = reinterpret_cast<const float2*>(a.last_uv)[i];
+            u = p.x; v = p.y;
+            if (flow && flow_selected(a, i, u, v)) ++c_flow;
+        }
+        if (i < a.n_still) {
+            const bool m = a.last_still[i] != 0;
+            if (still && m) ++c_still;
+            if (warp && !m && uv_within(u, v, a.W, a.H)) {
+                const float2 f = reinterpret_cast<const float2*>(a.gt_flow)[(size_t)trunc_clamp(v, a.H) * a.W + trunc_clamp(u, a.W)];
+                const float un = u + f.x, vn = v + f.y;
+                const float d = a.warp_depth[(size_t)trunc_clamp(vn, a.H) * a.W + trunc_clamp(un, a.W)];
+                float x[3];
+                pix2world(c, un, vn, d, x);
+                float* row = a.params + (size_t)i * ROW;
+                row[0] = x[0]; row[1] = x[1]; row[2] = x[2];
+            }
+        }
+    }
+    const int t_flow = block_sum_int(c_flow, s_part), t_still = block_sum_int(c_still, s_part);
+    if (threadIdx.x == 0) {
+        a.partial[blockIdx.x] = t_flow;
+        a.partial[STAGE_COUNT_BLOCKS + blockIdx.x] = t_still;
+    }
+}
+
+__global__ void __launch_bounds__(STAGE_BLOCK) stage_tables_kernel(BeginArgs a) {
+    __shared__ int s_part[STAGE_BLOCK / 64];
+    const bool flow = a.flow_w != nullptr, still = a.still_w != nullptr;
+    int n_sel_flow = 0, n_sel_still = 0;
+    if (flow || still) {
+        const int t = threadIdx.x;
+        n_sel_flow = block_sum_int(t < a.count_blocks ? a.partial[t] : 0, s_part);
+        n_sel_still = block_sum_int(t < a.count_blocks ? a.partial[STAGE_COUNT_BLOCKS + t] : 0, s_part);
+    }
+    const int i = blockIdx.x * STAGE_BLOCK + threadIdx.x;
+    if (i < a.cap) {
+        if (a.row_flags) a.row_flags[i] = i < a.n_lab ? (uint8_t)((a.still_mask[i] != 0 ? 1 : 0) | 2) : (uint8_t)0;
+        if (flow) {
+            float2 tgt = make_float2(0.f, 0.f);
+            float w = 0.f;
+            if (i < a.n_flow) {
+                const float2 p = reinterpret_cast<const float2*>(a.last_uv)[i];
+                const float2 f = reinterpret_cast<const float2*>(a.gt_flow)[(size_t)trunc_clamp(p.y, a.H) * a.W + trunc_clamp(p.x, a.W)];
+                tgt = make_float2(p.x + f.x, p.y + f.y);
+                w = (flow_selected(a, i, p.x, p.y) ? 1.f : 0.f) / (2.0f * (float)max(n_sel_flow, 1));
+            }
+            reinterpret_cast<float2*>(a.flow_target)[i] = tgt;
+            a.flow_w[i] = w;
+        }
+        if (still) {
+            float x = 0.f, y = 0.f, z = 0.f, w = 0.f;
+            if (i < a.n_still) {
+                const float* p = a.last_xyz + (size_t)i * a.xyz_stride;
+                x = p[0]; y = p[1]; z = p[2];
+                w = (a.last_still[i] != 0 ? 1.f : 0.f) / (float)max(n_sel_still, 1);
+            }
+            float* tg = a.still_target + (size_t)i * 3;
+            tg[0] = x; tg[1] = y; tg[2] = z;
+            a.still_w[i] = w;
+        }
+    }
+    const float4 z4 = make_float4(0.f, 0.f, 0.f, 0.f);
+    float4* m4 = reinterpret_cast<float4*>(a.adam_m);
+    float4* v4 = reinterpret_cast<float4*>(a.adam_v);
+    const size_t quads = (size_t)a.N * (ROW / 4), stride = (size_t)gridDim.x * STAGE_BLOCK;
+    for (size_t j = (size_t)i; j < quads; j += stride) { m4[j] = z4; v4[j] = z4; }
+    if (i < 7) { a.pose_m[i] = 0.f; a.pose_v[i] = 0.f; }
+    if (i < 2) { a.depth_ab_m[i] = 0.f; a.depth_ab_v[i] = 0.f; a.depth_ab[i] = i == 0 ? 1.f : 0.f; }
+    if (i == 0) *a.step = 0;
+}
+
+__global__ void __launch_bounds__(MIN_BLOCK)
+    densify_min_kernel(const int64_t* __restrict__ idx, int k, const float* __restrict__ gt_depth, int P, float* __restrict__ out) {
+    __shared__ float s_min[MIN_BLOCK / 64];
+    float m = INFINITY;
+    for (int j = threadIdx.x; j < k; j += MIN_BLOCK) {
+        const int64_t p = idx[j];
+        m = fminf(m, gt_depth[p < 0 ? 0 : (p >= P ? P - 1 : p)]);
+    }
+#pragma unroll
+    for (int off = 32; off >= 1; off >>= 1) m = fminf(m, __shfl_xor(m, off));
+    if ((threadIdx.x & 63) == 0) s_min[threadIdx.x >> 6] = m;
+    __syncthreads();
+    if (threadIdx.x == 0) {
+        for (int w = 1; w < MIN_BLOCK / 64; ++w) m = fminf(m, s_min[w]);
+        *out = m;
+    }
+}
+
+__global__ void __launch_bounds__(STAGE_BLOCK)
+    densify_rows_kernel(float* __restrict__ params, float* __restrict__ adam_m, float* __restrict__ adam_v, int N,
+                        const int64_t* __restrict__ idx, int k, const float* __restrict__ gt_depth,
+                        const float* __restrict__ gt_rgb, int W, int H, const float* __restrict__ intr,
+                        const float* __restrict__ pose, const float* __restrict__ opacity_raw, float inv_num_points,
+                        const float* __restrict__ depth_min) {
+#pragma clang fp contract(off)
+    const int j = blockIdx.x * STAGE_BLOCK + threadIdx.x;
+    if (j >= k) return;
+    const Cam c = cam_from_pose(intr, pose);
+    const int P = W * H;
+    const int64_t p64 = idx[j];
+    const int p = (int)(p64 < 0 ? 0 : (p64 >= P ? P - 1 : p64));
+    const int py = p / W, px = p - py * W;
+    const float d = gt_depth[p];
+    float x[3];
+    pix2world(c, (float)px, (float)py, d, x);
+    const float s = fabsf(d / *depth_min * inv_num_points);
+    float col[3];
+#pragma unroll
+    for (int ch = 0; ch < 3; ++ch) {
+        const float g = fminf(fmaxf(gt_rgb[(size_t)p * 3 + ch], 1e-15f), 1.0f);
+        col[ch] = logf(g / (1.0f - g));
+    }
+    const size_t r = (size_t)(N + j) * (ROW / 4);
+    float4* row = reinterpret_cast<float4*>(params) + r;
+    row[0] = make_float4(x[0], x[1], x[2], s);
+    row[1] = make_float4(s, s, 1.f, 0.f);
+    row[2] = make_float4(0.f, 0.f, *opacity_raw, col[0]);
+    row[3] = make_float4(col[1], col[2], 0.f, 0.f);
+    const float4 z4 = make_float4(0.f, 0.f, 0.f, 0.f);
+    float4* m4 = reinterpret_cast<float4*>(adam_m) + r;
+    float4* v4 = reinterpret_cast<float4*>(adam_v) + r;
+#pragma unroll
+    for (int q = 0; q < ROW / 4; ++q) { m4[q] = z4; v4[q] = z4; }
+}
+
+}
+
+using namespace gfl;
+
+extern "C" {
+
+int gfl_stage_end(const float* rec, int n_rendered, const uint8_t* move_mask, int W, int H, const uint8_t* last_still,
+                  int n_last, int n_now, uint8_t* still, uint8_t* tentative, float* uv_out, float* depth_out,
+                  uint8_t* sel_out, gfl_stream_t stream) {
+    if (W < 2 || H < 2 || (size_t)W * H > ((size_t)1 << 30)) return GFL_ERR_INVALID;
+    if (n_rendered < 0 || n_last < 0 || n_now < 0 || n_rendered > n_now || n_last > n_now) return GFL_ERR_INVALID;
+    if (n_last > 0 && !last_still) return GFL_ERR_INVALID;
+    if (n_now == 0) return GFL_OK;
+    if (!move_mask || !still || !tentative) return GFL_ERR_INVALID;
+    if (n_rendered > 0 && (!rec || !uv_out || !depth_out || !sel_out || ((uintptr_t)uv_out & 7))) return GFL_ERR_INVALID;
+    stage_end_kernel<<<(n_now + STAGE_BLOCK - 1) / STAGE_BLOCK, STAGE_BLOCK, 0, (hipStream_t)stream>>>(
+        rec, n_rendered, move_mask, W, H, last_still, n_last, n_now, still, tentative, uv_out, depth_out, sel_out);
+    return check_launch();
+}
+
+size_t gfl_stage_begin_workspace_bytes(void) { return (size_t)2 * STAGE_COUNT_BLOCKS * sizeof(int32_t); }
+
+int gfl_stage_begin(const gfl_fit_state* st, const float* last_uv, int n_flow, const float* gt_flow,
+                    const uint8_t* still_mask, int n_lab, const uint8_t* last_still, int n_still, const float* last_xyz,
+                    int xyz_stride, int camera_only, const float* warp_depth, void* workspace, size_t workspace_bytes,
+                    gfl_stream_t stream) {
+    if (!st || st->W < 2 || st->H < 2 || (size_t)st->W * st->H > ((size_t)1 << 30)) return GFL_ERR_INVALID;
+    if (st->N < 0 || st->cap <= 0 || st->N > st->cap) return GFL_ERR_INVALID;
+    if (!st->params || !st->adam_m || !st->adam_v || !st->pose || !st->intr || !st->pose_m || !st->pose_v || !st->depth_ab ||
+        !st->depth_ab_m || !st->depth_ab_v || !st->step)
+        return GFL_ERR_INVALID;
+    if (n_flow < 0 || n_lab < 0 || n_still < 0 || n_flow > st->N || n_lab > st->N || n_still > st->N) return GFL_ERR_INVALID;
+    const bool flow = st->flow_target || st->flow_w, still = st->still_target || st->still_w, warp = warp_depth != nullptr;
+    if (flow && (!st->flow_target || !st->flow_w || !gt_flow || (n_flow > 0 && !last_uv))) return GFL_ERR_INVALID;
+    if (still && (!st->still_target || !st->still_w || (n_still > 0 && (!last_still || !last_xyz || xyz_stride < 3))))
+        return GFL_ERR_INVALID;
+    if (warp && (!gt_flow || n_still > n_flow || (n_still > 0 && (!last_still || !last_uv)))) return GFL_ERR_INVALID;
+    if (n_lab > 0 && !still_mask) return GFL_ERR_INVALID;
+    if (((uintptr_t)last_uv & 7) || ((uintptr_t)gt_flow & 7) || ((uintptr_t)st->flow_target & 7)) return GFL_ERR_INVALID;
+    if (!flow) n_flow = warp ? n_flow : 0;
+    if (!still && !warp) n_still = 0;
+    const bool count = flow || still || warp;
+    if (count && (!workspace || workspace_bytes < gfl_stage_begin_workspace_bytes())) return GFL_ERR_WORKSPACE;
+    hipStream_t s = (hipStream_t)stream;
+    BeginArgs a;
+    a.last_uv = last_uv; a.n_flow = n_flow; a.gt_flow = gt_flow;
+    a.still_mask = still_mask; a.n_lab = n_lab;
+    a.last_still = last_still; a.n_still = n_still;
+    a.last_xyz = last_xyz; a.xyz_stride = xyz_stride;
+    a.warp_depth = warp_depth;
+    a.camera_only = camera_only; a.W = st->W; a.H = st->H; a.N = st->N; a.cap = st->cap;
+    a.params = st->params; a.adam_m = st->adam_m; a.adam_v = st->adam_v;
+    a.intr = st->intr; a.pose = st->pose;
+    a.pose_m = st->pose_m; a.pose_v = st->pose_v;
+    a.depth_ab = st->depth_ab; a.depth_ab_m = st->depth_ab_m; a.depth_ab_v = st->depth_ab_v;
+    a.step = st->step;
+    a.flow_target = const_cast<float*>(st->flow_target); a.flow_w = const_cast<float*>(st->flow_w);
+    a.still_target = const_cast<float*>(st->still_target); a.still_w = const_cast<float*>(st->still_w);
+    a.row_flags = const_cast<uint8_t*>(st->row_flags);
+    a.partial = (int32_t*)workspace;
+    const int rows = max(n_flow, n_still);
+    a.count_blocks = min(max((rows + STAGE_BLOCK - 1) / STAGE_BLOCK, 1), STAGE_COUNT_BLOCKS);
+    if (count) stage_count_warp_kernel<<<a.count_blocks, STAGE_BLOCK, 0, s>>>(a);
+    stage_tables_kernel<<<(st->cap + STAGE_BLOCK - 1) / STAGE_BLOCK, STAGE_BLOCK, 0, s>>>(a);
+    return check_launch();
+}
+
+int gfl_densify_append(float* params, float* adam_m, float* adam_v, int N, int cap, const int64_t* idx, int k,
+                       const float* gt_depth, const float* gt_rgb, int W, int H, const float* intr, const float* pose,
+                       const float* opacity_raw, float inv_num_points, float* depth_min, gfl_stream_t stream) {
+    if (W < 2 || H < 2 || (size_t)W * H > ((size_t)1 << 30)) return GFL_ERR_INVALID;
+    if (N < 0 || k < 0 || cap <= 0 || (long long)N + k > cap) return GFL_ERR_INVALID;
+    if (k == 0) return GFL_OK;
+    if (!params || !adam_m || !adam_v || !idx || !gt_depth || !gt_rgb || !intr || !pose || !opacity_raw || !depth_min)
+        return GFL_ERR_INVALID;
+    hipStream_t s = (hipStream_t)stream;
+    densify_min_kernel<<<1, MIN_BLOCK, 0, s>>>(idx, k, gt_depth, W * H, depth_min);
+    densify_rows_kernel<<<(k + STAGE_BLOCK - 1) / STAGE_BLOCK, STAGE_BLOCK, 0, s>>>(
+        params, adam_m, adam_v, N, idx, k, gt_depth, gt_rgb, W, H, intr, pose, opacity_raw, inv_num_points, depth_min);
+    return check_launch();
+}
+
+}
diff --git a/gflow_amd/fit_video.py b/gflow_amd/fit_video.py
--- a/gflow_amd/fit_video.py
+++ b/gflow_amd/fit_video.py
@@ -294,7 +294,7 @@
             xyz_now = tr.get_attribute("xyz")[traj_index_t].detach().float().clone()
             extr_now = tr.get_extr().detach().clone()
             if tr.engine_current:
-                rgb_u8 = tr._render_scene_fused()[0].clone()
+                rgb_u8 = tr._render_scene_fused(images=1)[0].clone()
                 final.append(tr._aux)
             else:
                 from . import render as render_mod
diff --git a/gflow_amd/fused.py b/gflow_amd/fused.py
--- a/gflow_amd/fused.py
+++ b/gflow_amd/fused.py
@@ -26,6 +26,7 @@
                 ("workspace", _P), ("workspace_bytes", ctypes.c_size_t), ("cu_count", _I), ("flags", _I)]
 
 GFL_FIT_DETERMINISTIC = 1
+SNAP_RGB, SNAP_DEPTH, SNAP_CENTER, SNAP_ALL = 1, 2, 4, 7
 
 
 class FitHyper(ctypes.Structure):
@@ -50,6 +51,10 @@
     lib.gfl_fit_iterations.argtypes = [ctypes.POINTER(FitState), ctypes.POINTER(FitHyper), ctypes.c_int, ctypes.c_int, _P]
     lib.gfl_fit_snapshot.restype = ctypes.c_int
     lib.gfl_fit_snapshot.argtypes = [ctypes.POINTER(FitState), ctypes.POINTER(FitHyper), _P, _P, _P, ctypes.c_size_t, _P]
+    lib.gfl_fit_snapshot_images.restype = ctypes.c_int
+    lib.gfl_fit_snapshot_images.argtypes = [ctypes.POINTER(FitState), ctypes.POINTER(FitHyper), _P, _P, _P, ctypes.c_size_t, _I, _P]
+    lib.gfl_stage_begin.restype = ctypes.c_int
+    lib.gfl_stage_begin.argtypes = [ctypes.POINTER(FitState), _P, _I, _P, _P, _I, _P, _I, _P, _I, _I, _P, _P, ctypes.c_size_t, _P]
     lib.gfl_fit_iteration_snapshot.restype = ctypes.c_int
     lib.gfl_fit_iteration_snapshot.argtypes = [ctypes.POINTER(FitState), ctypes.POINTER(FitHyper), _P, _P, _P]
     lib.gfl_render_bwd.restype = ctypes.c_int
@@ -126,6 +131,7 @@
         self._pend_event = self._pend_host = self._ovf_event = self._ovf_host = None
         self._snap_ring = self._snap_ring_done = None
         self._snap_out = self._snap_ws = self._capture_stream = None
+        self._tables = self._stage_ws = self._depth_min = None
         self._launched = False
         self._reserved_N = -1
         self.busy = False
@@ -256,17 +262,84 @@
         self.row_flags = pad(row_flags, 0, torch.uint8)
         self._state = None
 
+    def stage_begin(self, last_uv=None, gt_flow=None, flow_term=False, last_still=None, last_xyz=None, still_term=False,
+                    labels=None, camera_only=False, warp_depth=None):
+        f32c = lambda t: None if t is None else t.detach().to(self.dev).float().contiguous()
+        last_uv, gt_flow, warp_depth = f32c(last_uv), f32c(gt_flow), f32c(warp_depth)
+        if flow_term and (last_uv is None or gt_flow is None):
+            raise ValueError("FitEngine.stage_begin: the flow term needs last_uv and gt_flow")
+        if still_term and (last_still is None or last_xyz is None):
+            raise ValueError("FitEngine.stage_begin: the still term needs last_still and last_xyz")
+        if warp_depth is not None and (last_still is None or last_uv is None or gt_flow is None):
+            raise ValueError("FitEngine.stage_begin: the warp needs last_still, last_uv and gt_flow")
+        if gt_flow is not None and tuple(gt_flow.shape) != (self.H, self.W, 2):
+            raise ValueError(f"FitEngine.stage_begin: gt_flow is {tuple(gt_flow.shape)}, not {(self.H, self.W, 2)}")
+        if warp_depth is not None:
+            warp_depth = warp_depth.reshape(self.H, self.W)
+        labels = None if labels is None else L.mask_u8(labels)
+        last_still = None if last_still is None else L.mask_u8(last_still)
+        n_still, xyz_stride = 0, 3
+        if last_still is not None and (still_term or warp_depth is not None):
+            n_still = last_still.shape[0]
+        if still_term:
+            last_xyz = last_xyz.detach()
+            if last_xyz.dtype != torch.float32 or last_xyz.dim() != 2 or last_xyz.stride(1) != 1 or last_xyz.shape[1] != 3:
+                last_xyz = last_xyz.float().reshape(-1, 3).contiguous()
+            if last_xyz.shape[0] < n_still:
+                raise ValueError("FitEngine.stage_begin: last_xyz has fewer rows than last_still")
+            xyz_stride = last_xyz.stride(0)
+        tb = self._tables
+        if tb is None or tb["flow_w"].shape[0] != self.cap:
+            e = lambda *shape, dtype=torch.float32: torch.empty(*shape, dtype=dtype, device=self.dev)
+            tb = self._tables = {"flow_target": e(self.cap, 2), "flow_w": e(self.cap), "still_target": e(self.cap, 3),
+                                 "still_w": e(self.cap), "row_flags": e(self.cap, dtype=torch.uint8)}
+        if self._stage_ws is None:
+            self._stage_ws = torch.empty(int(self.lib.gfl_stage_begin_workspace_bytes()), dtype=torch.uint8, device=self.dev)
+        self.flow_target, self.flow_w = (tb["flow_target"], tb["flow_w"]) if flow_term else (None, None)
+        self.still_target, self.still_w = (tb["still_target"], tb["still_w"]) if still_term else (None, None)
+        self.row_flags = tb["row_flags"] if labels is not None else None
+        self._state = None
+        self._reserved_N = -1
+        n_flow = last_uv.shape[0] if last_uv is not None and (flow_term or warp_depth is not None) else 0
+        L.check(self.lib.gfl_stage_begin(ctypes.byref(self._struct()), L.ptr(last_uv), n_flow, L.ptr(gt_flow), L.ptr(labels),
+                                         0 if labels is None else labels.shape[0], L.ptr(last_still), n_still,
+                                         L.ptr(last_xyz) if still_term else None, int(xyz_stride), int(bool(camera_only)),
+                                         L.ptr(warp_depth), L.ptr(self._stage_ws), self._stage_ws.numel(), L.stream()),
+                "stage begin")
+
+    def append_rows(self, idx, gt_depth, gt_rgb, intr, pose, opacity_raw, inv_num_points):
+        k = int(idx.shape[0])
+        if k == 0:
+            return
+        if idx.dtype != torch.int64 or not idx.is_contiguous():
+            idx = idx.long().contiguous()
+        self.ensure_capacity(self.N + k)
+        f32c = lambda t: t.detach().to(self.dev).float().contiguous()
+        gt_depth, gt_rgb, intr, pose, opacity_raw = (f32c(t) for t in (gt_depth, gt_rgb, intr, pose, opacity_raw))
+        if gt_depth.numel() != self.H * self.W or tuple(gt_rgb.shape) != (self.H, self.W, 3):
+            raise ValueError("FitEngine.append_rows: gt_depth / gt_rgb do not have the engine's image size")
+        if self._depth_min is None:
+            self._depth_min = torch.empty(1, dtype=torch.float32, device=self.dev)
+        L.check(self.lib.gfl_densify_append(L.ptr(self.params), L.ptr(self.adam_m), L.ptr(self.adam_v), self.N, self.cap,
+                                            L.ptr(idx), k, L.ptr(gt_depth), L.ptr(gt_rgb), self.W, self.H, L.ptr(intr),
+                                            L.ptr(pose), L.ptr(opacity_raw), float(inv_num_points), L.ptr(self._depth_min),
+                                            L.stream()), "densify append")
+
+    def _struct(self):
+        s = FitState()
+        s.N, s.cap, s.W, s.H, s.K_cap = self.N, self.cap, self.W, self.H, self.K_cap
+        for name, ctype in FitState._fields_:
+            if ctype is _P:
+                t = getattr(self, {"depth_ab_m": "ab_m", "depth_ab_v": "ab_v"}.get(name, name))
+                setattr(s, name, None if t is None else t.data_ptr())
+        s.workspace_bytes = self.workspace.numel()
+        s.cu_count = self.cu_count
+        s.flags = GFL_FIT_DETERMINISTIC if self._deterministic else 0
+        return s
+
     def state(self):
         if self._state is None:
-            s = FitState()
-            s.N, s.cap, s.W, s.H, s.K_cap = self.N, self.cap, self.W, self.H, self.K_cap
-            for name, ctype in FitState._fields_:
-                if ctype is _P:
-                    t = getattr(self, {"depth_ab_m": "ab_m", "depth_ab_v": "ab_v"}.get(name, name))
-                    setattr(s, name, None if t is None else t.data_ptr())
-            s.workspace_bytes = self.workspace.numel()
-            s.cu_count = self.cu_count
-            s.flags = GFL_FIT_DETERMINISTIC if self._deterministic else 0
+            s = self._struct()
             if self.gt_rgb is not None and self.foot_flags is None:
                 L.check(self.lib.gfl_fit_prepare_targets(ctypes.byref(s), L.stream()), "fit prepare targets")
                 s.gt_cached = 1
@@ -371,15 +444,19 @@
         self._launched = True
         return self._snap_out if snapshot else None
 
-    def snapshot(self, out=None):
+    def snapshot(self, out=None, images=SNAP_ALL):
         from .color import lut
-        need = self.lib.gfl_fit_snapshot_workspace_bytes(self.N, self.W, self.H)
-        if self._snap_ws is None or self._snap_ws.numel() < need:
-            self._snap_ws = torch.empty(int(need * 1.5), dtype=torch.uint8, device=self.dev)
+        ws = None
+        if images & (SNAP_DEPTH | SNAP_CENTER):
+            need = self.lib.gfl_fit_snapshot_workspace_bytes(self.N, self.W, self.H)
+            if self._snap_ws is None or self._snap_ws.numel() < need:
+                self._snap_ws = torch.empty(int(need * 1.5), dtype=torch.uint8, device=self.dev)
+            ws = self._snap_ws
         if out is None:
             out = torch.empty(3, self.H, self.W, 3, dtype=torch.uint8, device=self.dev)
-        L.check(self.lib.gfl_fit_snapshot(ctypes.byref(self.state()), ctypes.byref(self.hp), L.ptr(lut("turbo", self.dev)),
-                                          L.ptr(out), L.ptr(self._snap_ws), self._snap_ws.numel(), L.stream()), "snapshot")
+        L.check(self.lib.gfl_fit_snapshot_images(ctypes.byref(self.state()), ctypes.byref(self.hp),
+                                                 L.ptr(lut("turbo", self.dev)) if images & SNAP_DEPTH else None, L.ptr(out),
+                                                 L.ptr(ws), 0 if ws is None else ws.numel(), int(images), L.stream()), "snapshot")
         return out
 
     _STATE_TENSORS = ("step", "pose", "pose_m", "pose_v", "depth_ab", "ab_m", "ab_v")
diff --git a/gflow_amd/stage.py b/gflow_amd/stage.py
--- a/gflow_amd/stage.py
+++ b/gflow_amd/stage.py
@@ -119,6 +119,7 @@
         self.iteration = 0
         self.move_mask, self.camera_only = p.move_mask, p.camera_only
         self.uv = self.depth = self.last_render = None
+        self.rec = None
         self.yielding = False
 
     @property
@@ -224,14 +225,12 @@
         eng = self.eng = tr._pack_to_engine()
         super().__init__(tr, p, RingSink(eng, p, tr.H, tr.W, tr.device))
         eng.drop_pending()
-        eng.pose.copy_(tr.pose.detach())
+        if tr.pose is not eng.pose:
+            eng.pose.copy_(tr.pose.detach())
         eng.invalidate_regions()
         tr.pose = eng.pose
-        eng.depth_ab.zero_()
-        eng.depth_ab[0:1].fill_(1.0)
         tr.depth_ab = eng.depth_ab
         eng.intr.copy_(tr.intr)
-        eng.reset_optimizer()
         hp = eng.hp
         hp.bg = tr.bg
         hp.lambda_rgb = p.lambda_rgb if p.lambda_rgb > 0 else 0.0
@@ -243,7 +242,7 @@
         hp.freeze_all_splats = 1 if p.camera_only else 0
         hp.step_camera = 1
         hp.lambda_flow = hp.lambda_still = 0.0
-        self._set_regularisers()
+        self._begin()
         move_mask, camera_only = p.move_mask, p.camera_only
         eng.set_targets(tr.gt_image, tr.gt_depth if p.lambda_depth > 0 else None,
                         (~move_mask) if (camera_only and move_mask is not None) else None)
@@ -253,34 +252,24 @@
                                    ~tr.still_mask_tentative)
         self.unchecked = 0
 
-    def _set_regularisers(self):
-        tr, p, eng, dev = self.tr, self.plan, self.eng, self.tr.device
-        n, hp = eng.N, eng.hp
-        flow_target = flow_w = still_target = still_w = row_flags = None
-        if tr.has_still:
-            row_flags = torch.zeros(n, dtype=torch.uint8, device=dev)
-            row_flags[:tr.still_mask.shape[0]] = tr.still_mask.to(torch.uint8) | 2
-        still = tr._still_selection(p.lambda_still)
-        if still is not None:
-            m, last_xyz = still
-            still_target = torch.zeros(n, 3, device=dev)
-            still_target[:m.shape[0]] = last_xyz
-            still_w = torch.zeros(n, device=dev)
-            still_w[:m.shape[0]] = m.float() / m.sum().clamp(min=1)
+    def _begin(self):
+        tr, p, eng, hp = self.tr, self.plan, self.eng, self.eng.hp
+        still_term = bool(p.lambda_still and tr.has_still)
+        flow_term = tr._has_flow_term(p.lambda_flow)
+        warp = bool(p.warp)
+        if still_term:
             hp.lambda_still = p.lambda_still
-        flow = tr._flow_selection(p.lambda_flow, p.camera_only)
-        if flow is not None:
-            and_mask, gt_f = flow
-            flow_target = torch.zeros(n, 2, device=dev)
-            flow_target[:tr.last_num] = tr.last_uv + gt_f
-            flow_w = torch.zeros(n, device=dev)
-            flow_w[:tr.last_num] = and_mask.float() / (2.0 * and_mask.sum().clamp(min=1))
+        if flow_term:
             hp.lambda_flow = p.lambda_flow
-        eng.set_regularisers(flow_target, flow_w, still_target, still_w, row_flags)
+        eng.stage_begin(last_uv=tr.last_uv if flow_term or warp else None, gt_flow=tr.gt_flow if flow_term or warp else None,
+                        flow_term=flow_term, last_still=tr.last_still_mask if still_term or warp else None,
+                        last_xyz=tr.last_xyz if still_term else None, still_term=still_term,
+                        labels=tr.still_mask if tr.has_still else None, camera_only=p.camera_only,
+                        warp_depth=tr.gt_depth if warp else None)
 
     def note_forward(self, n_rendered, rec=None):
         rec = self.eng.rec if rec is None else rec
-        self.uv, self.depth, self.last_render = rec[:n_rendered, 0:2], rec[:n_rendered, 9:10], self.eng.render
+        self.uv, self.depth, self.last_render, self.rec = rec[:n_rendered, 0:2], rec[:n_rendered, 9:10], self.eng.render, rec
 
     def settle(self, last=None):
         while True:
diff --git a/gflow_amd/trainer.py b/gflow_amd/trainer.py
--- a/gflow_amd/trainer.py
+++ b/gflow_amd/trainer.py
@@ -90,6 +90,7 @@
         self.traj_xyz = self.traj_scale = self.traj_rotate = self.traj_opacity = self.traj_rgb = self.last_traj_group = None
         self._engine_live = False
         self._aux = self._snap_aux = self._snap_stream = self._snap_done = None
+        self._new_opacity_raw = None
 
     @property
     def later_frame(self):
@@ -245,9 +246,10 @@
                      mask_count=None):
         if move_mask is not None:
             move_mask = move_mask.to(self.device).bool()
-        if not camera_only and self.has_still:
+        warp = not camera_only and self.has_still
+        if warp and not self.fused:
             self._warp_moving()
-        plan = StagePlan(iterations=iterations, lr=lr, lr_camera=lr_camera, lambda_rgb=lambda_rgb, lambda_depth=lambda_depth,
+        plan = StagePlan(warp=warp and self.fused, iterations=iterations, lr=lr, lr_camera=lr_camera, lambda_rgb=lambda_rgb, lambda_depth=lambda_depth,
                          lambda_flow=lambda_flow, lambda_var=lambda_var, lambda_still=lambda_still, lambda_scale=lambda_scale,
                          move_mask=move_mask, densify_interval=densify_interval, densify_times=densify_times, mask=mask,
                          camera_only=camera_only, densify_occ_percent=densify_occ_percent, densify_err_thre=densify_err_thre,
@@ -287,8 +289,11 @@
         m = self.last_still_mask
         return m, self.last_xyz[:m.shape[0]]
 
+    def _has_flow_term(self, lambda_flow):
+        return bool(lambda_flow and self.gt_flow is not None and self.last_uv is not None)
+
     def _flow_selection(self, lambda_flow, camera_only):
-        if not (lambda_flow and self.gt_flow is not None and self.last_uv is not None):
+        if not self._has_flow_term(lambda_flow):
             return None
         W, H = self.W, self.H
         and_mask = self._stage_rows(geometry.within(self.last_uv, W, H), camera_only)
@@ -338,9 +343,11 @@
             move_mask = move_mask.to(self.device).bool()
 
         self._project_appended(st)
-        uv_d, depth_d = st.uv.clone(), st.depth.clone()
         if not st.camera_only:
-            self._relabel_after_stage(uv_d, depth_d, move_mask, move_seg)
+            if self.fused and self.engine is not None:
+                self._relabel_after_stage(st.uv, st.depth, move_mask, move_seg, rec=st.rec)
+            else:
+                self._relabel_after_stage(st.uv.clone(), st.depth.clone(), move_mask, move_seg)
         parts, parts_block = (None, None, None, None), None
         if self.has_still and render_parts:
             parts, parts_block = self._render_parts(st.sink)
@@ -361,33 +368,40 @@
         with torch.no_grad():
             if self.fused and self.engine is not None:
                 self.engine.forward()
-                st.uv, st.depth, st.last_render = self.engine.uv, self.engine.depth, self.engine.render
+                st.uv, st.depth, st.last_render, st.rec = self.engine.uv, self.engine.depth, self.engine.render, self.engine.rec
             else:
                 st.uv, st.depth, st.last_render, _ = self._render_rgbd(want_extras=False)
             self.rasterisations_done += 1
 
-    def _relabel_after_stage(self, uv_d, depth_d, move_mask, move_seg):
+    def _relabel_after_stage(self, uv_d, depth_d, move_mask, move_seg, rec=None):
         W, H, dev = self.W, self.H, self.device
+        n_now = self.current_pts_num()
+        if rec is not None:
+            self.still_mask, self.still_mask_tentative, uv_d, depth_d, moving_inside = L.stage_end(
+                rec, uv_d.shape[0], move_mask, self.last_still_mask, n_now)
+            return self._after_relabel(uv_d, depth_d, move_seg, lambda: moving_inside)
         within = geometry.within(uv_d, W, H)
         yx = uv_d.long()
         labels = ~move_mask[yx[:, 1].clamp(0, H - 1), yx[:, 0].clamp(0, W - 1)]
-        n_now = self.current_pts_num()
         still = torch.ones(n_now, dtype=torch.bool, device=dev)
         still[:uv_d.shape[0]] = torch.where(within, labels, still[:uv_d.shape[0]])
         self.still_mask = still
         self.still_mask_tentative = still.clone()
         if self.last_still_mask is not None:
             self.still_mask[:self.last_still_mask.shape[0]] = self.last_still_mask
+        self._after_relabel(uv_d, depth_d, move_seg, lambda: within & ~self.still_mask[:uv_d.shape[0]])
+
+    def _after_relabel(self, uv_d, depth_d, move_seg, moving_inside):
+        W, H = self.W, self.H
         if move_seg:
             from .hull import FastConcaveHull2D
             from scipy.ndimage import minimum_filter
-            sel = within & ~self.still_mask[:uv_d.shape[0]]
-            pts = uv_d[sel].cpu().numpy()
+            pts = uv_d[moving_inside()].cpu().numpy()
             if pts.shape[0] > 5:
                 self.move_seg = (FastConcaveHull2D(pts).mask(W, H) * 255).astype(np.uint8)
                 self.move_seg_erode = minimum_filter(self.move_seg, size=20, mode="constant", cval=255)
         if self.seg_recorder is not None:
-            self.seg_recorder.record(uv_d, within & ~self.still_mask[:uv_d.shape[0]])
+            self.seg_recorder.record(uv_d, moving_inside())
         if self.mask_prompt_pts is not None:
             from .hull import FastConcaveHull2D
             m = self.mask_prompt_pts
@@ -453,9 +467,9 @@
         aux.hp.bg = self.bg
         return aux
 
-    def _render_scene_fused(self):
+    def _render_scene_fused(self, images=7):
         aux = self._aux_forward()
-        out = aux.snapshot()
+        out = aux.snapshot(images=images)
         aux.watch_overflow()
         return out
 
@@ -467,15 +481,16 @@
 
     def _render_parts_fused(self):
         eng, aux, n = self.engine, self._aux_engine(), self.engine.N
-        out = []
+        from .fused import SNAP_CENTER, SNAP_RGB
+        out = torch.empty(2, 3, self.H, self.W, 3, dtype=torch.uint8, device=self.device)
         hidden = torch.full((), -1000.0, device=self.device)
-        for sel in (self.still_mask, ~self.still_mask):
+        for j, sel in enumerate((self.still_mask, ~self.still_mask)):
             aux.params[:n].copy_(eng.params[:n])
             aux.params[:n, 10] = torch.where(sel, eng.params[:n, 10], hidden)
             aux.forward()
-            out.append(aux.snapshot())
+            aux.snapshot(out=out[j], images=SNAP_RGB | SNAP_CENTER)
         aux.watch_overflow()
-        return torch.stack(out)
+        return out
 
     def densify_weights(self, error_map, error_threshold=1e-3, mask=None):
         dev = self.device
@@ -521,8 +536,20 @@
         if densify_num > 0:
             idx = self.sample_pixels(err, densify_num)
             self.last_densify_idx = idx
-            self.densification_postfix(*self.new_splats_at(idx // W, idx % W))
+            if self.engine_live:
+                self._append_in_engine(idx)
+            else:
+                self.densification_postfix(*self.new_splats_at(idx // W, idx % W))
         return num_before, self.current_pts_num()
+
+    def _append_in_engine(self, idx):
+        eng = self.engine
+        if self._new_opacity_raw is None:
+            self._new_opacity_raw = (torch.logit(0.99 * torch.ones(1, 1, device=self.device)) / 10.0).reshape(1)
+        n0, k = eng.N, idx.shape[0]
+        eng.append_rows(idx, self.gt_depth, self.gt_image, self.intr, self.pose, self._new_opacity_raw, 1.0 / self.num_points)
+        eng.set_count(n0 + k)
+        self._attributes = eng.views()
 
     def sample_pixels(self, weights, count):
         from .sampling import cdf_device
diff --git a/include/gflow_hip.h b/include/gflow_hip.h
--- a/include/gflow_hip.h
+++ b/include/gflow_hip.h
@@ -194,6 +194,12 @@
 size_t gfl_fit_snapshot_workspace_bytes(int N, int W, int H);
 int gfl_fit_snapshot(const gfl_fit_state* st, const gfl_fit_hyper* hp, const float* lut, uint8_t* out_u8, void* workspace,
                      size_t workspace_bytes, gfl_stream_t stream);
+#define GFL_SNAP_RGB 1
+#define GFL_SNAP_DEPTH 2
+#define GFL_SNAP_CENTER 4
+#define GFL_SNAP_ALL 7
+int gfl_fit_snapshot_images(const gfl_fit_state* st, const gfl_fit_hyper* hp, const float* lut, uint8_t* out_u8, void* workspace,
+                            size_t workspace_bytes, int images, gfl_stream_t stream);
 int gfl_fit_iteration_snapshot(const gfl_fit_state* st, const gfl_fit_hyper* hp, const float* lut, uint8_t* out_u8,
                                gfl_stream_t stream);
 int gfl_fit_snapshot_stage(const gfl_fit_state* src, const gfl_fit_state* dst, gfl_stream_t stream);
@@ -258,6 +264,18 @@
 int gfl_flow_occlusion(const float* fwd, const float* bwd, int n_pairs, int W, int H, float alpha, float beta,
                        float* diff_fwd, float* diff_bwd, uint8_t* occ_fwd, uint8_t* occ_bwd, gfl_stream_t stream);
 
+int gfl_stage_end(const float* rec, int n_rendered, const uint8_t* move_mask, int W, int H, const uint8_t* last_still,
+                  int n_last, int n_now, uint8_t* still, uint8_t* tentative, float* uv_out, float* depth_out,
+                  uint8_t* sel_out, gfl_stream_t stream);
+size_t gfl_stage_begin_workspace_bytes(void);
+int gfl_stage_begin(const gfl_fit_state* st, const float* last_uv, int n_flow, const float* gt_flow,
+                    const uint8_t* still_mask, int n_lab, const uint8_t* last_still, int n_still, const float* last_xyz,
+                    int xyz_stride, int camera_only, const float* warp_depth, void* workspace, size_t workspace_bytes,
+                    gfl_stream_t stream);
+int gfl_densify_append(float* params, float* adam_m, float* adam_v, int N, int cap, const int64_t* idx, int k,
+                       const float* gt_depth, const float* gt_rgb, int W, int H, const float* intr, const float* pose,
+                       const float* opacity_raw, float inv_num_points, float* depth_min, gfl_stream_t stream);
+
 int gfl_abi_sizes(int* sizeof_fit_state, int* sizeof_fit_hyper);
 
 #define GFL_PROFILE_STAGES 9
```

Result: no change. 10.45 (median of 3 runs) (+1.8%).
